# shanice-l/UNOPose

Measured on AMD Instinct MI355X. Metric: (query,ref) pairs/sec forward, higher is better.
Workload: dtype bf16; 1 GPU; UNOPose.forward, batch 32 pairs/GPU, 2048 query pts, 5000->2048 reference pts, 196 coarse pts, 518x518 crops, DINOv2 ViT-B/14 reg4, random-init (trained-like) weights

## Files before the change

### include/unopose_hip.h

```cpp
#ifndef UNOPOSE_HIP_H
#define UNOPOSE_HIP_H

#include <stdint.h>

#ifdef __cplusplus
extern "C" {
#endif

#define UNOPOSE_OK 0
#define UNOPOSE_EINVAL 1
#define UNOPOSE_ELAUNCH 2
#define UNOPOSE_ENOMEM 3

typedef void *unopose_stream_t;

int unopose_abi_version(void);
const char *unopose_last_error(void);


int unopose_furthest_point_sampling(const float *xyz, int B, int N, int M,
                                    int32_t *idx, unopose_stream_t stream);

int unopose_gather_points(const float *points, const int32_t *idx, int B, int C,
                          int N, int M, float *out, unopose_stream_t stream);
// ... 45 lines not shown
int unopose_pe_image_bytes(void);
int unopose_pe_pack_weights(const float *w1, const float *b1, const float *w2, const float *b2,
                            const float *w3, const float *b3, void *image, unopose_stream_t stream);

int unopose_pe_geometry(const float *xyz, int B, int N, float radius, int nsample, float radius2, int nsample2,
                        const int *cand_in, const int *cand_cnt_in, int cand_stride, void *lists, int *counts,
                        float *frames, int *cand_out, void *lists2, int *counts2, float *frames2,
                        unopose_stream_t stream);
int unopose_pe_mlp_max_packed(const float *xyz, int B, int N, float radius, int nsample, const void *image,
                              const void *lists, const int *counts, const float *frames, void *out, int out_ld,
                              int out_split, unopose_stream_t stream);

int unopose_geo_embedding(const float *points, int B, int n, const void *wd_hi,
                          const void *wd_lo, const void *wa_hi, const void *wa_lo,
                          const float *bias_sum, const float *div_term,
                          float sigma_d, float factor_a, int reduce_mean, int split,
                          int out_bf16, int32_t *knn_ws, void *out,
                          unopose_stream_t stream);

int unopose_geo_embedding_table(const float *points, int B, int n, const float *tab_d, int rows_d, const float *tab_a, int rows_a,
                                const float *bias_sum, const float *w_d, const float *div_term, int hinv, int npoint, float sigma_d,
                                float factor_a, int reduce_mean, int out_bf16, int32_t *knn_ws, void *out,
                                unopose_stream_t stream);

int unopose_geo_embedding_train_workgroups(int B, int n);
int unopose_geo_embedding_train_forward(const float *points, int B, int n, const float *tab_d, int rows_d, const float *tab_a, int rows_a,
                                        const float *bias_sum, const float *w_d, const float *div_term, int hinv, float sigma_d, float factor_a,
                                        int reduce_mean, int32_t *knn, float *out, void *amax, unopose_stream_t stream);
int unopose_geo_embedding_train_backward(const float *points, const int32_t *knn, int B, int n, int rows_d, int rows_a, int hinv, float sigma_d,
                                         float factor_a, int reduce_mean, const float *dE, const void *amax, float *ws, float *full_d,
                                         int *past_table, unopose_stream_t stream);

int unopose_pe_group_mlp_max(const float *xyz, int B, int N, float radius, int nsample,
                             const float *w1, const float *b1, const float *w2,
                             const float *b2, const float *w3, const float *b3,
                             int bf16x3, float *out, unopose_stream_t stream);

int unopose_softmax_stats(const float *x, int B, int R, int C, float *stats_ws, unopose_stream_t stream);
int unopose_infonce_grad(const float *x, int B, int R, int C, const float *stats_ws, const long long *label1,
                         const long long *label2, const float *g, float *grad, unopose_stream_t stream);

int unopose_bn_train_chunk(void);
int unopose_bn_relu_train_forward(const float *x, int B, int C, long L, const float *gamma, const float *beta, float eps, float momentum,
                                  float *running_mean, float *running_var, float *workspace, float *mean, float *rstd, float *y,
                                  unopose_stream_t stream);
int unopose_bn_relu_train_backward(const float *x, const float *dy, int B, int C, long L, const float *gamma, const float *beta,
                                   const float *mean, const float *rstd, float *workspace, float *dgamma, float *dbeta, float *dx,
                                   unopose_stream_t stream);

int unopose_bn_relu_maxpool_train_forward(const float *x, int B, int C, int N, int S, const float *gamma, const float *beta, float eps,
                                          float momentum, float *running_mean, float *running_var, float *workspace, float *mean, float *rstd,
                                          float *out, int32_t *idx, unopose_stream_t stream);
int unopose_bn_relu_maxpool_train_backward(const float *x, const float *g, const int32_t *idx, int B, int C, int N, int S, const float *gamma,
                                           const float *beta, const float *mean, const float *rstd, float *workspace, float *dgamma, float *dbeta,
                                           float *dx, unopose_stream_t stream);

int unopose_saliency_train_forward(const float *atten, const float *s1, const float *s2, int B, int n1, int n2, float *m1, float *m2, float *rmax,
                                   float *rsum, float *cmax, float *csum, unopose_stream_t stream);
int unopose_saliency_train_backward(const float *atten, const float *s1, const float *s2, const float *m1, const float *m2, const float *rmax,
                                    const float *rsum, const float *cmax, const float *csum, const float *g1, const float *g2, int B, int n1, int n2,
                                    float *d_atten, float *ds1, float *ds2, unopose_stream_t stream);

int unopose_nearest_partner(const float *a, const float *b, int B, int n, int m, int over_b, float thr, float *dmin, int32_t *arg,
                            uint8_t *any_close, unopose_stream_t stream);

int unopose_conv1x1_train_wgrad_blocks(void);
int unopose_conv1x1_train_forward(const float *x, int B, int cin, long L, const float *w, int cout, float *y, unopose_stream_t stream);
int unopose_conv1x1_train_wgrad(const float *dy, const float *x, int B, int cout, int cin, long L, float *workspace, float *dw,
                                unopose_stream_t stream);

int unopose_linear_wgrad_f32_splits(long rows, int N, int K);
int unopose_linear_wgrad_f32(const float *g, const float *x, long rows, int N, int K, float *workspace, float *dw, unopose_stream_t stream);
int unopose_assign_labels(const float *atten, int B, int R, int C, const float *score1,
                          const float *score2, float *stats_ws, float *w1, float *w2,
                          unopose_stream_t stream);

int unopose_fine_correspondences(const float *atten, int B, int R, int C, const float *score1,
                                 const float *score2, const float *stats_ws, const float *w1,
                                 const float *w2, const float *pts2, float *weight, float *pred,
                                 unopose_stream_t stream);

int unopose_upproj_plan(const long long *choose, int B2, int Np, int H, int W, int side, int tok_offset, int tok_stride,
                        int cap_rows, int *ws, int *row_list, int *cellmap, int *tile_info, unopose_stream_t stream);

int unopose_linear_bf16_ld(const void *A, int lda, const void *W, int ldw, const float *bias, void *C, int ldc, long M, int N, int K,
                           int epilogue, unopose_stream_t stream);

int unopose_linear_add_layernorm_bf16(const void *A, const void *W, const float *bias, const void *resid, const float *ln_w,
                                      const float *ln_b, float eps, void *C, long M, int K, unopose_stream_t stream);

int unopose_linear_bf16_kv_vt(const void *A, const void *W, const float *bias, void *C, void *vt, long M, int N, int K, int tokens, int key_pad,
                              unopose_stream_t stream);

int unopose_linear_bf16_gather(const void *A, long M, int K, const void *W, int N, const float *bias, const int *row_list,
                               const int *tile_info, int max_tiles, void *C, unopose_stream_t stream);

int unopose_bilinear_sample_compact(const void *Cc, const int *cellmap, const long long *choose, int B2, int side, int Np,
                                    int H, int W, void *out, int out_bf16, unopose_stream_t stream);

int unopose_fine_assign(const void *f1, const void *f2, int B, int R, int C, int D, float shift, const float *score1,
                        const float *score2, const float *pts2, float *ws, float *w1, float *w2, float *weight,
                        float *pred, unopose_stream_t stream);

int unopose_min_dist(const float *p, const float *q, int B, int N, int M, const float *R,
                     const float *t, int cand_per_b, float *out, unopose_stream_t stream);

int unopose_coarse_hypotheses(const float *atten, int B, int R, int C, const float *score1,
                              const float *score2, const float *stats_ws, const float *w1,
                              const float *w2, const float *rand, int nprop, const float *pts1,
                              const float *pts2, float *cdf_ws, float *Rout, float *tout,
                              float *dis, unopose_stream_t stream);

int unopose_coarse_scores(const float *pts1, const float *pts2, int B, int n1, int n2,
                          const float *Rall, const float *tall, int nprop, const int64_t *top,
                          int ncand, const float *w1, float *score, unopose_stream_t stream);

int unopose_topk_smallest(const float *x, int B, int n, int k, int64_t *idx, unopose_stream_t stream);
int unopose_coarse_pick(const float *score, const int64_t *top, int B, int ncand, const float *Rall, const float *tall, int nprop,
                        float *R, float *t, float *best_score, unopose_stream_t stream);

int unopose_token_attention(const void *q, int ldq, const void *k, int ldk, const void *vt,
                            const void *qp, int ldqp, const void *E, int B, int n, int m,
                            float scale, void *out, unopose_stream_t stream);
int unopose_token_attention_key_pad(void);

int unopose_token_attention_f32(const float *q, int ldq, const float *k, int ldk, const float *vt,
                                const float *qp, int ldqp, const float *E, int B, int n, int m,
                                float scale, float *out, unopose_stream_t stream);
int unopose_vit_attention_f32(const float *qkv, int B, int T, int H, float *out, unopose_stream_t stream);
int unopose_token_attention_f32_train(const float *q, int ldq, const float *k, int ldk, const float *vt,
                                      const float *qp, int ldqp, const float *E, int B, int n, int m,
                                      float scale, float *out, float *P, unopose_stream_t stream);
int unopose_token_attention_f32_backward(const float *dout, const float *q, int ldq, const float *v, int ldv,
                                         const float *kt, const float *qp, int ldqp, const float *E, const float *P,
                                         int B, int n, int m, float scale, float *dS, float *dq, float *dk, float *dv,
                                         float *dqp, float *dE, unopose_stream_t stream);
int unopose_vit_attention_f32_split(const float *qkv, int B, int T, int H, void *out_split, unopose_stream_t stream);
int unopose_vit_attention_f32_ss(const void *qkv_split, int B, int T, int H, void *out_split, unopose_stream_t stream);

int unopose_vit_attention(const void *qkv, int B, int T, int H, void *out, unopose_stream_t stream);
int unopose_vit_attention_route(int T, int H);

int unopose_add_layernorm(const void *a, int a_bf16, const void *b, int b_bf16, const float *w,
                          const float *bias, long rows, int C, float eps, void *out, int out_bf16,
                          unopose_stream_t stream);

int unopose_add_layernorm_strided(const void *a, int a_bf16, const void *b, int b_bf16, const float *w,
                                  const float *bias, long rows, int C, float eps, void *out, int out_bf16,
                                  long ld_out, unopose_stream_t stream);

int unopose_add_layernorm_train(const void *a, int a_bf16, const void *b, int b_bf16, const float *w,
                                const float *bias, long rows, int C, float eps, float *y, float *s, float *mean,
                                float *rstd, unopose_stream_t stream);
int unopose_add_layernorm_backward_slabs(long rows, int C);
int unopose_add_layernorm_backward(const float *dy, const float *s, const float *mean, const float *rstd,
                                   const float *w, long rows, int C, float *dx, float *dw, float *db,
                                   float *partials, int partial_slabs, unopose_stream_t stream);

int unopose_bilinear_sample(const void *z, int z_bf16, const long long *choose, int B, int side, int Np,
                            int H, int W, float *out, unopose_stream_t stream);

int unopose_bilinear_sample_tokens(const void *z, int z_bf16, const long long *choose, int B, int side, int Np,
                                   int H, int W, int tok_offset, int tok_stride, float *out,
                                   unopose_stream_t stream);

int unopose_scale_residual_layernorm(float *x, const void *y_bf16, const float *gamma, const float *w,
                                     const float *bias, long rows, int C, float eps, void *out_bf16,
                                     unopose_stream_t stream);
int unopose_scale_residual_layernorm_f32(float *x, const float *y, const float *gamma, const float *w, const float *bias, long rows,
                                         int C, float eps, void *out_split, long out_ld_bytes, unopose_stream_t stream);

int unopose_scale_residual(float *x, const void *y_bf16, const float *gamma, long rows, int C,
                           unopose_stream_t stream);

int unopose_linear_attention(const void *x, const float *inv_softplus_scale, const void *kvt,
                             const float *ksum, int B, int N, int focus, int mode, void *out,
                             unopose_stream_t stream);
int unopose_linear_attention_kv_state(const void *ykv, const float *inv_softplus_scale, int B, int J, int rows_per_pair,
                                      int first_row, int focus, void *kvt, float *ksum, unopose_stream_t stream);
int unopose_linear_attention_f32(const float *x, const float *inv_softplus_scale, const float *kvt,
                                 const float *ksum, int B, int N, int focus, int mode, float *out,
                                 unopose_stream_t stream);

int unopose_render_depth(const float *verts, int V, const int *faces, int F, const float *Rt, const float *K4, int P, int H, int W,
                         float *depth, unopose_stream_t stream);

int unopose_render_color(const float *verts, int V, const int *faces, int F, const float *colors, float surf_r, float surf_g, float surf_b,
                         float ambient, const float *Rt, const float *K4, int P, int H, int W, void *keys, float *depth, void *rgb,
                         unopose_stream_t stream);

int unopose_render_shaded(const float *verts, int V, const int *faces, int F, const float *normals, const float *colors, const float *uv,
                          const float *texture, int Ht, int Wt, float surf_r, float surf_g, float surf_b, float ambient, int phong, int ssaa,
                          const float *Rt, const float *K4, int P, int H, int W, void *keys, void *rgb, unopose_stream_t stream);

int unopose_vis_workspace_ints(void);
int unopose_vis_compose(const void *rgbs, const float *depths, int P, int H, int W, const void *photo, int resolve_visib, int *boxes,
                        void *ren_rgb, float *ren_depth, void *vis_rgb, unopose_stream_t stream);
int unopose_vis_depth_diff(const float *ren_depth, const float *depth, int H, int W, float delta, void *workspace, void *image, double *stats,
                           unopose_stream_t stream);

int unopose_patchify_bf16(const float *rgb_a, int na, const float *rgb_b, int nb, int S, int Kp, void *out,
                          unopose_stream_t stream);
int unopose_vit_tokens_layernorm(const void *patch, const float *pos, const float *prefix, int npre, int P, int nimg, int C,
                                 const float *ln_w, const float *ln_b, float eps, float *x, void *n1, float *row_mean, unopose_stream_t stream);
int unopose_patchify_split(const float *rgb_a, int na, const float *rgb_b, int nb, int S, int Kp, void *out, unopose_stream_t stream);
int unopose_vit_tokens_layernorm_f32(const float *patch, const float *pos, const float *prefix, int npre, int P, int nimg, int C,
                                     const float *ln_w, const float *ln_b, float eps, float *x, void *n1_split, unopose_stream_t stream);
int unopose_row_dot(const void *x, int x_bf16, const float *w, float b, long rows, int C, void *out, int out_bf16,
                    unopose_stream_t stream);
int unopose_normalize_rows_bf16(const void *x, int x_bf16, long rows, int C, float temp, void *out, int out_f32,
                                unopose_stream_t stream);
int unopose_gather_rows(const void *feats, int B, int N, int row_bytes, const void *idx, int idx_is_i64, int J, int off,
                        const void *alt, long alt_stride_bytes, int prepend, void *out, unopose_stream_t stream);
int unopose_transpose_pad_bf16(const void *v, long ld, int B, int m, int C, int pad, void *vt, unopose_stream_t stream);
int unopose_transpose_pad_f32(const float *v, long ld, int B, int m, int C, int pad, float *vt, unopose_stream_t stream);

int unopose_cloud_radius(const float *pts, int B, int N, float *radius, unopose_stream_t stream);
int unopose_scale_by_radius(const float *x, int B, int n, const float *radius, float eps, int multiply, float *out, unopose_stream_t stream);
int unopose_overlap_scores(const void *scores, int x_bf16, int B, int n_tot, int n1, int halves, float *out, unopose_stream_t stream);
int unopose_nan_to_num_multi(const void *ptrs_dev, const void *sizes_dev, int n_tensors, long max_size, float nan_value, float posinf_value,
                             float neginf_value, unopose_stream_t stream);
int unopose_copy_rows(const void *src, long src_stride_bytes, void *dst, long dst_stride_bytes, int rows, int row_bytes,
                      unopose_stream_t stream);
int unopose_rigid_rows_bf16(const float *p, int B, int N, const float *t, const float *R, void *out, unopose_stream_t stream);
int unopose_token_sum_bf16(const void *x, int B, int J, int C, float *out, unopose_stream_t stream);
int unopose_pose_score(const float *dis, const float *w, int B, int N, float thr, float *out, unopose_stream_t stream);

int unopose_linear_bf16(const void *A, const void *W, const float *bias, void *C, long M, int N, int K,
                        int epilogue, unopose_stream_t stream);
int unopose_gemm_bf16_tile(void);

int unopose_linear_bf16_residual(const void *A, const void *W, const float *bias, float *xres, void *xb, float *stats, const float *prev,
                                 int prev_nparts, long M, int N, int K, unopose_stream_t stream);
int unopose_linear_bf16_lnfold(const void *A, const void *W, const float *dvec, const float *cvec, const float *stats, int nparts, float eps,
                               void *C, long M, int N, int K, int gelu, unopose_stream_t stream);
int unopose_gemm_fold_stagger(int eighth_ticks_per_ktile);

int unopose_bmm_f32(const float *A, long sab, long sah, long sai, long sak, const float *Bm, long sbb, long sbh, long sbj, long sbk,
                    float *C, int bo, int bi, int n, int m, int K, float alpha, unopose_stream_t stream);

int unopose_split_bf16x2(const float *X, long M, int K, void *Xs, unopose_stream_t stream);
int unopose_linear_f32x3(const void *As, const void *Ws, const float *bias, float *C, void *Cs, long M, int N, int K,
                         int epilogue, unopose_stream_t stream);
int unopose_linear_f32x3_bf16(const void *As, const void *Ws, const float *bias, const void *resid, void *Cb, long M, int N, int K,
                              unopose_stream_t stream);

int unopose_prep_desc_ints(void);
int unopose_prep_crop_resize(const void *img, int H, int W, int C, const int *desc, const int *taps, const void *masks, const float *lut,
                             int D, int S, int bgr, int use_mask, float *out, unopose_stream_t stream);
int unopose_prep_compact_lift(const double *depth, int H, int W, const int *desc, const void *masks, const int *row_base, double fx,
                              double fy, double cx, double cy, int D, int max_h, int *pix, double *cloud, double *row_sums,
                              unopose_stream_t stream);
int unopose_prep_distances(const int *desc, const double *cloud, const double *row_sums, int D, int max_n, double *dist,
                           unopose_stream_t stream);
int unopose_prep_gather(const int *sel, const int *index, const int *pix, const double *cloud, int P, int n, int S, float *pts, void *choose,
                        unopose_stream_t stream);

int unopose_rle_desc_ints(void);
int unopose_rle_stats_ints(void);
int unopose_rle_parse(const void *bytes, const int *lists, const int *desc, int D, int H, int W, int *starts, int *stats,
                      unopose_stream_t stream);
int unopose_rle_fill(const int *desc, const int *starts, const double *depth, int D, int H, int W, void *masks, int *stats,
                     unopose_stream_t stream);
int unopose_rle_column_scan(const void *masks, int D, int H, int W, int *col_count, int *totals, unopose_stream_t stream);
int unopose_rle_compact(const void *masks, const int *col_count, const void *off, int D, int H, int W, int *pos, unopose_stream_t stream);
int unopose_rle_diff(const int *pos, const void *off, int D, int max_n, int H, int W, int *counts, unopose_stream_t stream);
int unopose_window_masks(const void *masks, const int *desc, int K, int max_h, int H, int W, void *packed, int *row_counts,
                         unopose_stream_t stream);

int unopose_vsd_count_ints(void);
int unopose_vsd_counts(const float *test, int n_test, const float *gt, int n_gt, const float *est, int n_est, const int *index,
                       const double *pairs, const double *taus, int T, int P, int H, int W, int *counts, unopose_stream_t stream);
int unopose_pose_errors(const double *pts, int n, const double *syms, int S, const double *est, const double *gt, const double *K, int P,
                        double *mssd, double *mspd, unopose_stream_t stream);

int unopose_adi_tile_points(void);
int unopose_adi_slab_points(void);
int unopose_pose_metrics(const double *pts, int n, const double *syms, int S, const double *est, const double *gt, const double *K, int P,
                         int proj_sym, double *out, unopose_stream_t stream);
int unopose_adi(const double *pts, int n, const double *est, const double *gt, int P, double *workspace, double *adi,
                unopose_stream_t stream);

int unopose_gt_visibility_ints(void);
int unopose_gt_visibility(const float *canvas, int n_canvas, const float *test, int n_test, const int *index, const double *params, int G,
                          int H, int W, int *out, void *mask, void *mask_visib, unopose_stream_t stream);

int unopose_pts_extent_tile_points(void);
int unopose_pts_extent_doubles(void);
int unopose_pts_extent(const double *pts, const long long *offsets, const long long *offsets_dev, int M, int prune, double *kept,
                       long long *kept_count, double *out, unopose_stream_t stream);

int unopose_ref_select_query_tile(void);
int unopose_ref_select_entry_tile(void);
int unopose_ref_select_slab(int Q, int C, int S);
int unopose_ref_select(const double *Rq, const long long *q_scene, const unsigned long long *q_key, int Q, const double *Rc,
                       const long long *c_scene, const unsigned long long *c_key, int C, const double *syms, int S, double trace_min,
                       unsigned long long seed, int cross_scene, int slab, long long *workspace, long long *out, unopose_stream_t stream);

int unopose_adam_table_ints(int what);
int unopose_adam_prepare(const void *grads_dev, const void *chunks_dev, long n_chunks, int n_tensors, double *partials, unopose_stream_t stream);
int unopose_adam_finalise(const double *partials, long n_chunks, int n_tensors, const void *state_dev, const void *finite, double max_norm, double lr,
                          double beta1, double beta2, float *block, unopose_stream_t stream);
int unopose_adam_update(const void *grads_dev, const void *state_dev, const void *chunks_dev, long n_chunks, int n_tensors, const float *block,
                        double beta1, double beta2, double eps, double weight_decay, unopose_stream_t stream);

int unopose_coloraug_ints(int what);
int unopose_coloraug_luma_sum(const void *src, int H, int W, const int *desc, const int *ops, int n_crops, int max_pixels, int pos, void *sums,
                              unopose_stream_t stream);
int unopose_coloraug_step(const void *src, void *dst, int H, int W, const int *desc, const int *ops, const void *grids, const float *noise,
                          const void *sums, int n_crops, int max_pixels, int pos, unopose_stream_t stream);
int unopose_coloraug_blur_lines(const void *src, void *dst, int H, int W, const int *desc, const int *ops, int n_crops, int max_across,
                                int max_line, int pos, int axis, unopose_stream_t stream);

#ifdef __cplusplus
}
#endif
#endif
```

### unopose_amd/_lib.py

```python
import ctypes
import os

import torch

_HERE = os.path.dirname(os.path.abspath(__file__))
SO_PATH = os.environ.get("UNOPOSE_LIB") or os.path.join(_HERE, "libunopose_hip.so")

_lib = None

_P = ctypes.c_void_p
_I = ctypes.c_int
_F = ctypes.c_float
_L = ctypes.c_long
_D = ctypes.c_double

SIGNATURES = {
    "unopose_furthest_point_sampling": [_P, _I, _I, _I, _P, _P],
    "unopose_gather_points": [_P, _P, _I, _I, _I, _I, _P, _P],
    "unopose_gather_points_grad": [_P, _P, _I, _I, _I, _I, _P, _P],
    "unopose_ball_query": [_P, _P, _I, _I, _I, _F, _I, _P, _P],
    "unopose_group_points": [_P, _P, _I, _I, _I, _I, _I, _P, _P],
    "unopose_group_points_grad": [_P, _P, _I, _I, _I, _I, _I, _P, _P],
    "unopose_three_nn": [_P, _P, _I, _I, _I, _P, _P, _P],
    "unopose_three_interpolate": [_P, _P, _P, _I, _I, _I, _I, _P, _P],
    "unopose_three_interpolate_grad": [_P, _P, _P, _I, _I, _I, _I, _P, _P],
    "unopose_lrf_global": [_P, _I, _I, _I, _P, _P],
    "unopose_query_lrf_group": [_P, _I, _I, _F, _I, _P, _P],
    "unopose_lrf_group_idx": [_P, _P, _P, _I, _I, _F, _I, _P, _P],
    "unopose_weighted_procrustes": [_P, _P, _P, _I, _I, _F, _F, _P, _P, _P],
    "unopose_assign_labels": [_P, _I, _I, _I, _P, _P, _P, _P, _P, _P],
    "unopose_linear_bf16_ld": [_P, _I, _P, _I, _P, _P, _I, ctypes.c_long, _I, _I, _I, _P],
    "unopose_scale_residual_layernorm_f32": [_P, _P, _P, _P, _P, ctypes.c_long, _I, _F, _P, _L, _P],
    "unopose_gather_rows": [_P, _I, _I, _I, _P, _I, _I, _I, _P, _L, _I, _P, _P],
    "unopose_softmax_stats": [_P, _I, _I, _I, _P, _P],
    "unopose_infonce_grad": [_P, _I, _I, _I, _P, _P, _P, _P, _P, _P],
    "unopose_fine_correspondences": [_P, _I, _I, _I, _P, _P, _P, _P, _P, _P, _P, _P, _P],
    "unopose_upproj_plan": [_P, _I, _I, _I, _I, _I, _I, _I, _I, _P, _P, _P, _P, _P],
    "unopose_linear_add_layernorm_bf16": [_P, _P, _P, _P, _P, _P, _F, _P, ctypes.c_long, _I, _P],
    "unopose_linear_bf16_kv_vt": [_P, _P, _P, _P, _P, ctypes.c_long, _I, _I, _I, _I, _P],
    "unopose_linear_bf16_gather": [_P, ctypes.c_long, _I, _P, _I, _P, _P, _P, _I, _P, _P],
    "unopose_bilinear_sample_compact": [_P, _P, _P, _I, _I, _I, _I, _I, _P, _I, _P],
    "unopose_fine_assign": [_P, _P, _I, _I, _I, _I, _F, _P, _P, _P, _P, _P, _P, _P, _P, _P],
    "unopose_min_dist": [_P, _P, _I, _I, _I, _P, _P, _I, _P, _P],
    "unopose_coarse_hypotheses": [_P, _I, _I, _I, _P, _P, _P, _P, _P, _P, _I, _P, _P, _P, _P, _P, _P, _P],
    "unopose_coarse_scores": [_P, _P, _I, _I, _I, _P, _P, _I, _P, _I, _P, _P, _P],
    "unopose_topk_smallest": [_P, _I, _I, _I, _P, _P],
    "unopose_coarse_pick": [_P, _P, _I, _I, _P, _P, _I, _P, _P, _P, _P],
    "unopose_token_attention": [_P, _I, _P, _I, _P, _P, _I, _P, _I, _I, _I, _F, _P, _P],
    "unopose_token_attention_key_pad": [],
    "unopose_token_attention_f32": [_P, _I, _P, _I, _P, _P, _I, _P, _I, _I, _I, _F, _P, _P],
    "unopose_token_attention_f32_train": [_P, _I, _P, _I, _P, _P, _I, _P, _I, _I, _I, _F, _P, _P, _P],
    "unopose_token_attention_f32_backward": [_P, _P, _I, _P, _I, _P, _P, _I, _P, _P, _I, _I, _I, _F, _P, _P, _P, _P, _P, _P, _P],
    "unopose_vit_attention_f32": [_P, _I, _I, _I, _P, _P],
    "unopose_vit_attention_f32_split": [_P, _I, _I, _I, _P, _P],
    "unopose_vit_attention_f32_ss": [_P, _I, _I, _I, _P, _P],
    "unopose_bn_train_chunk": [],
    "unopose_bn_relu_train_forward": [_P, _I, _I, ctypes.c_long, _P, _P, _F, _F, _P, _P, _P, _P, _P, _P, _P],
    "unopose_bn_relu_train_backward": [_P, _P, _I, _I, ctypes.c_long, _P, _P, _P, _P, _P, _P, _P, _P, _P],
    "unopose_bn_relu_maxpool_train_forward": [_P, _I, _I, _I, _I, _P, _P, _F, _F, _P, _P, _P, _P, _P, _P, _P, _P],
    "unopose_bn_relu_maxpool_train_backward": [_P, _P, _P, _I, _I, _I, _I, _P, _P, _P, _P, _P, _P, _P, _P, _P],
    "unopose_nearest_partner": [_P, _P, _I, _I, _I, _I, _F, _P, _P, _P, _P],
    "unopose_saliency_train_forward": [_P, _P, _P, _I, _I, _I, _P, _P, _P, _P, _P, _P, _P],
    "unopose_saliency_train_backward": [_P, _P, _P, _P, _P, _P, _P, _P, _P, _P, _P, _I, _I, _I, _P, _P, _P, _P],
    "unopose_conv1x1_train_wgrad_blocks": [],
    "unopose_conv1x1_train_forward": [_P, _I, _I, ctypes.c_long, _P, _I, _P, _P],
    "unopose_conv1x1_train_wgrad": [_P, _P, _I, _I, _I, ctypes.c_long, _P, _P, _P],
    "unopose_linear_wgrad_f32_splits": [ctypes.c_long, _I, _I],
    "unopose_linear_wgrad_f32": [_P, _P, ctypes.c_long, _I, _I, _P, _P, _P],
    "unopose_vit_attention": [_P, _I, _I, _I, _P, _P],
    "unopose_vit_attention_route": [_I, _I],
    "unopose_add_layernorm": [_P, _I, _P, _I, _P, _P, ctypes.c_long, _I, _F, _P, _I, _P],
    "unopose_add_layernorm_strided": [_P, _I, _P, _I, _P, _P, ctypes.c_long, _I, _F, _P, _I, ctypes.c_long, _P],
    "unopose_add_layernorm_train": [_P, _I, _P, _I, _P, _P, _L, _I, _F, _P, _P, _P, _P, _P],
    "unopose_add_layernorm_backward_slabs": [_L, _I],
    "unopose_add_layernorm_backward": [_P, _P, _P, _P, _P, _L, _I, _P, _P, _P, _P, _I, _P],
    "unopose_bilinear_sample": [_P, _I, _P, _I, _I, _I, _I, _I, _P, _P],
    "unopose_bilinear_sample_tokens": [_P, _I, _P, _I, _I, _I, _I, _I, _I, _I, _P, _P],
    "unopose_scale_residual_layernorm": [_P, _P, _P, _P, _P, ctypes.c_long, _I, _F, _P, _P],
    "unopose_scale_residual": [_P, _P, _P, ctypes.c_long, _I, _P],
    "unopose_linear_attention": [_P, _P, _P, _P, _I, _I, _I, _I, _P, _P],
    "unopose_linear_attention_f32": [_P, _P, _P, _P, _I, _I, _I, _I, _P, _P],
    "unopose_linear_attention_kv_state": [_P, _P, _I, _I, _I, _I, _I, _P, _P, _P],
    "unopose_linear_bf16": [_P, _P, _P, _P, ctypes.c_long, _I, _I, _I, _P],
    "unopose_gemm_bf16_tile": [],
    "unopose_gemm_fold_stagger": [_I],
    "unopose_linear_bf16_residual": [_P, _P, _P, _P, _P, _P, _P, _I, ctypes.c_long, _I, _I, _P],
    "unopose_linear_bf16_lnfold": [_P, _P, _P, _P, _P, _I, _F, _P, ctypes.c_long, _I, _I, _I, _P],
    "unopose_patchify_bf16": [_P, _I, _P, _I, _I, _I, _P, _P],
    "unopose_patchify_split": [_P, _I, _P, _I, _I, _I, _P, _P],
    "unopose_vit_tokens_layernorm": [_P, _P, _P, _I, _I, _I, _I, _P, _P, _F, _P, _P, _P, _P],
    "unopose_vit_tokens_layernorm_f32": [_P, _P, _P, _I, _I, _I, _I, _P, _P, _F, _P, _P, _P],
    "unopose_row_dot": [_P, _I, _P, _F, ctypes.c_long, _I, _P, _I, _P],
    "unopose_normalize_rows_bf16": [_P, _I, ctypes.c_long, _I, _F, _P, _I, _P],
    "unopose_transpose_pad_bf16": [_P, ctypes.c_long, _I, _I, _I, _I, _P, _P],
    "unopose_transpose_pad_f32": [_P, _L, _I, _I, _I, _I, _P, _P],
    "unopose_cloud_radius": [_P, _I, _I, _P, _P],
    "unopose_scale_by_radius": [_P, _I, _I, _P, _F, _I, _P, _P],
    "unopose_overlap_scores": [_P, _I, _I, _I, _I, _I, _P, _P],
    "unopose_copy_rows": [_P, _L, _P, _L, _I, _I, _P],
    "unopose_nan_to_num_multi": [_P, _P, _I, _L, _F, _F, _F, _P],
    "unopose_rigid_rows_bf16": [_P, _I, _I, _P, _P, _P, _P],
    "unopose_token_sum_bf16": [_P, _I, _I, _I, _P, _P],
    "unopose_pose_score": [_P, _P, _I, _I, _F, _P, _P],
    "unopose_render_depth": [_P, _I, _P, _I, _P, _P, _I, _I, _I, _P, _P],
    "unopose_render_color": [_P, _I, _P, _I, _P, _F, _F, _F, _F, _P, _P, _I, _I, _I, _P, _P, _P, _P],
    "unopose_render_shaded": [_P, _I, _P, _I, _P, _P, _P, _P, _I, _I, _F, _F, _F, _F, _I, _I, _P, _P, _I, _I, _I, _P, _P, _P],
    "unopose_vis_workspace_ints": [],
    "unopose_vis_compose": [_P, _P, _I, _I, _I, _P, _I, _P, _P, _P, _P, _P],
    "unopose_vis_depth_diff": [_P, _P, _I, _I, _F, _P, _P, _P, _P],
    "unopose_bmm_f32": [_P, ctypes.c_long, ctypes.c_long, ctypes.c_long, ctypes.c_long, _P, ctypes.c_long, ctypes.c_long, ctypes.c_long, ctypes.c_long, _P, _I, _I, _I, _I, _I, _F, _P],
    "unopose_split_bf16x2": [_P, ctypes.c_long, _I, _P, _P],
    "unopose_linear_f32x3": [_P, _P, _P, _P, _P, ctypes.c_long, _I, _I, _I, _P],
    "unopose_pe_image_bytes": [],
    "unopose_pe_pack_weights": [_P, _P, _P, _P, _P, _P, _P, _P],
    "unopose_pe_geometry": [_P, _I, _I, _F, _I, _F, _I, _P, _P, _I, _P, _P, _P, _P, _P, _P, _P, _P],
    "unopose_pe_mlp_max_packed": [_P, _I, _I, _F, _I, _P, _P, _P, _P, _P, _I, _I, _P],
    "unopose_linear_f32x3_bf16": [_P, _P, _P, _P, _P, ctypes.c_long, _I, _I, _P],
    "unopose_pe_group_mlp_max": [_P, _I, _I, _F, _I, _P, _P, _P, _P, _P, _P, _I, _P, _P],
    "unopose_geo_embedding": [_P, _I, _I, _P, _P, _P, _P, _P, _P, _F, _F, _I, _I, _I, _P, _P, _P],
    "unopose_geo_embedding_train_workgroups": [_I, _I],
    "unopose_geo_embedding_train_forward": [_P, _I, _I, _P, _I, _P, _I, _P, _P, _P, _I, _F, _F, _I, _P, _P, _P, _P],
    "unopose_geo_embedding_train_backward": [_P, _P, _I, _I, _I, _I, _I, _F, _F, _I, _P, _P, _P, _P, _P, _P],
    "unopose_geo_embedding_table": [_P, _I, _I, _P, _I, _P, _I, _P, _P, _P, _I, _I, _F, _F, _I, _I, _P, _P, _P],
    "unopose_prep_desc_ints": [],
    "unopose_prep_crop_resize": [_P, _I, _I, _I, _P, _P, _P, _P, _I, _I, _I, _I, _P, _P],
    "unopose_prep_compact_lift": [_P, _I, _I, _P, _P, _P, _D, _D, _D, _D, _I, _I, _P, _P, _P, _P],
    "unopose_prep_distances": [_P, _P, _P, _I, _I, _P, _P],
    "unopose_prep_gather": [_P, _P, _P, _P, _I, _I, _I, _P, _P, _P],
    "unopose_rle_desc_ints": [],
    "unopose_rle_stats_ints": [],
    "unopose_rle_parse": [_P, _P, _P, _I, _I, _I, _P, _P, _P],
    "unopose_rle_fill": [_P, _P, _P, _I, _I, _I, _P, _P, _P],
    "unopose_rle_column_scan": [_P, _I, _I, _I, _P, _P, _P],
    "unopose_rle_compact": [_P, _P, _P, _I, _I, _I, _P, _P],
    "unopose_rle_diff": [_P, _P, _I, _I, _I, _I, _P, _P],
    "unopose_window_masks": [_P, _P, _I, _I, _I, _I, _P, _P, _P],
    "unopose_vsd_count_ints": [],
    "unopose_vsd_counts": [_P, _I, _P, _I, _P, _I, _P, _P, _P, _I, _I, _I, _I, _P, _P],
    "unopose_pose_errors": [_P, _I, _P, _I, _P, _P, _P, _I, _P, _P, _P],
    "unopose_adi_tile_points": [],
    "unopose_adi_slab_points": [],
    "unopose_pose_metrics": [_P, _I, _P, _I, _P, _P, _P, _I, _I, _P, _P],
    "unopose_adi": [_P, _I, _P, _P, _I, _P, _P, _P],
    "unopose_gt_visibility_ints": [],
    "unopose_gt_visibility": [_P, _I, _P, _I, _P, _P, _I, _I, _I, _P, _P, _P, _P],
    "unopose_pts_extent_tile_points": [],
    "unopose_pts_extent_doubles": [],
    "unopose_pts_extent": [_P, _P, _P, _I, _I, _P, _P, _P, _P],
    "unopose_ref_select_query_tile": [],
    "unopose_ref_select_entry_tile": [],
    "unopose_ref_select_slab": [_I, _I, _I],
    "unopose_ref_select": [_P, _P, _P, _I, _P, _P, _P, _I, _P, _I, _D, ctypes.c_ulonglong, _I, _I, _P, _P, _P],
    "unopose_adam_table_ints": [_I],
    "unopose_adam_prepare": [_P, _P, _L, _I, _P, _P],
    "unopose_adam_finalise": [_P, _L, _I, _P, _P, _D, _D, _D, _D, _P, _P],
    "unopose_adam_update": [_P, _P, _P, _L, _I, _P, _D, _D, _D, _D, _P],
    "unopose_coloraug_ints": [_I],
    "unopose_coloraug_luma_sum": [_P, _I, _I, _P, _P, _I, _I, _I, _P, _P],
    "unopose_coloraug_step": [_P, _P, _I, _I, _P, _P, _P, _P, _P, _I, _I, _I, _P],
    "unopose_coloraug_blur_lines": [_P, _P, _I, _I, _P, _P, _I, _I, _I, _I, _I, _P],
}


def lib():
    global _lib
    if _lib is None:
        if not os.path.exists(SO_PATH):
            raise RuntimeError(
                f"{SO_PATH} is missing: the HIP extension has not been built "
                "(run `python -m unopose_amd.build`). There is no CPU fallback."
# ... 68 lines not shown
```

### unopose_amd/csrc/fused.hip

```cpp
#include <algorithm>

#include "common.h"

namespace unopose {

template <bool IN_BF16>
__device__ __forceinline__ float fu_load(const void *p, size_t i) {
  return IN_BF16 ? bf2f(reinterpret_cast<const u16 *>(p)[i]) : reinterpret_cast<const float *>(p)[i];
}

template <bool A_BF16, bool B_BF16, bool HAS_B, bool OUT_BF16>
__global__ __launch_bounds__(256) void add_layernorm_kernel(const void *__restrict__ a, const void *__restrict__ b,
                                                            const float *__restrict__ w,
                                                            const float *__restrict__ bias, long rows, int C,
                                                            float eps, void *__restrict__ out, long ldo) {
  const long r = (long)blockIdx.x * 4 + (threadIdx.x >> 6);
  if (r >= rows) return;
  const int lane = threadIdx.x & 63;
  float v[16];
  float s = 0.f;
#pragma unroll
  for (int i = 0; i < 16; ++i) {
    const int c = i * 64 + lane;
    float x = 0.f;
    if (c < C) {
      x = fu_load<A_BF16>(a, (size_t)r * C + c);
      if (HAS_B) x += fu_load<B_BF16>(b, (size_t)r * C + c);
    }
    v[i] = x;
    s += x;
  }
  const float mean = wave_sum_f32(s) / (float)C;
  float q = 0.f;
#pragma unroll
  for (int i = 0; i < 16; ++i) {
    const int c = i * 64 + lane;
    const float d = c < C ? v[i] - mean : 0.f;
    q += d * d;
  }
  const float rstd = rsqrtf(wave_sum_f32(q) / (float)C + eps);
#pragma unroll
  for (int i = 0; i < 16; ++i) {
    const int c = i * 64 + lane;
    if (c < C) {
      const float y = (v[i] - mean) * rstd * w[c] + bias[c];
      if (OUT_BF16)
        reinterpret_cast<u16 *>(out)[(size_t)r * ldo + c] = f2bf(y);
      else
        reinterpret_cast<float *>(out)[(size_t)r * ldo + c] = y;
    }
  }
}

template <bool BF>
__device__ __forceinline__ float4 fu_load4(const void *p, size_t i) {
  if (BF) {
    const uint2 r = *reinterpret_cast<const uint2 *>(reinterpret_cast<const u16 *>(p) + i);
    return make_float4(bf2f((u16)(r.x & 0xFFFF)), bf2f((u16)(r.x >> 16)), bf2f((u16)(r.y & 0xFFFF)), bf2f((u16)(r.y >> 16)));
  }
  return *reinterpret_cast<const float4 *>(reinterpret_cast<const float *>(p) + i);
}
template <bool A_BF16, bool B_BF16, bool HAS_B, bool OUT_BF16>
__global__ __launch_bounds__(256) void add_layernorm_vec4_kernel(const void *__restrict__ a, const void *__restrict__ b,
                                                                 const float *__restrict__ w, const float *__restrict__ bias, long rows,
                                                                 int C, float eps, void *__restrict__ out, long ldo) {
  const long r = (long)blockIdx.x * 4 + (threadIdx.x >> 6);
  if (r >= rows) return;
  const int lane = threadIdx.x & 63;
  float4 v[4];
  float s = 0.f;
#pragma unroll
  for (int i = 0; i < 4; ++i) {
    const int c = (i * 64 + lane) * 4;
    float4 x = make_float4(0.f, 0.f, 0.f, 0.f);
    if (c < C) {
      x = fu_load4<A_BF16>(a, (size_t)r * C + c);
      if (HAS_B) {
        const float4 y = fu_load4<B_BF16>(b, (size_t)r * C + c);
        x.x += y.x;
        x.y += y.y;
        x.z += y.z;
        x.w += y.w;
      }
    }
    v[i] = x;
    s += (x.x + x.y) + (x.z + x.w);
  }
  const float mean = wave_sum_f32(s) / (float)C;
  float q = 0.f;
#pragma unroll
  for (int i = 0; i < 4; ++i) {
    if ((i * 64 + lane) * 4 < C) {
      const float d0 = v[i].x - mean, d1 = v[i].y - mean, d2 = v[i].z - mean, d3 = v[i].w - mean;
      q += (d0 * d0 + d1 * d1) + (d2 * d2 + d3 * d3);
    }
  }
  const float rstd = rsqrtf(wave_sum_f32(q) / (float)C + eps);
#pragma unroll
  for (int i = 0; i < 4; ++i) {
    const int c = (i * 64 + lane) * 4;
    if (c < C) {
      const float4 wv = *reinterpret_cast<const float4 *>(w + c), bv = *reinterpret_cast<const float4 *>(bias + c);
      const float y0 = (v[i].x - mean) * rstd * wv.x + bv.x, y1 = (v[i].y - mean) * rstd * wv.y + bv.y;
      const float y2 = (v[i].z - mean) * rstd * wv.z + bv.z, y3 = (v[i].w - mean) * rstd * wv.w + bv.w;
      if (OUT_BF16) {
        uint2 o;
        o.x = (uint32_t)f2bf(y0) | ((uint32_t)f2bf(y1) << 16);
        o.y = (uint32_t)f2bf(y2) | ((uint32_t)f2bf(y3) << 16);
        *reinterpret_cast<uint2 *>(reinterpret_cast<u16 *>(out) + (size_t)r * ldo + c) = o;
      } else {
        *reinterpret_cast<float4 *>(reinterpret_cast<float *>(out) + (size_t)r * ldo + c) = make_float4(y0, y1, y2, y3);
      }
    }
  }
}

__global__ __launch_bounds__(256) void scale_residual_layernorm_kernel(float *__restrict__ x, const u16 *__restrict__ y,
                                                                       const float *__restrict__ gamma,
                                                                       const float *__restrict__ w,
                                                                       const float *__restrict__ bias, long rows,
                                                                       int C, float eps, u16 *__restrict__ out) {
  const long r = (long)blockIdx.x * 4 + (threadIdx.x >> 6);
  if (r >= rows) return;
  const int lane = threadIdx.x & 63;
  float v[16];
  float s = 0.f;
#pragma unroll
  for (int i = 0; i < 4; ++i) {
    const int c = (i * 64 + lane) * 4;
    float4 xv = make_float4(0.f, 0.f, 0.f, 0.f);
    if (c < C) {
      xv = *reinterpret_cast<const float4 *>(x + (size_t)r * C + c);
      const uint2 yv = *reinterpret_cast<const uint2 *>(y + (size_t)r * C + c);
      const float4 g = *reinterpret_cast<const float4 *>(gamma + c);
      xv.x += g.x * bf2f((u16)(yv.x & 0xFFFF));
      xv.y += g.y * bf2f((u16)(yv.x >> 16));
      xv.z += g.z * bf2f((u16)(yv.y & 0xFFFF));
      xv.w += g.w * bf2f((u16)(yv.y >> 16));
      *reinterpret_cast<float4 *>(x + (size_t)r * C + c) = xv;
    }
    v[i * 4 + 0] = xv.x; v[i * 4 + 1] = xv.y; v[i * 4 + 2] = xv.z; v[i * 4 + 3] = xv.w;
    s += (xv.x + xv.y) + (xv.z + xv.w);
  }
  const float mean = wave_sum_f32(s) / (float)C;
  float q = 0.f;
#pragma unroll
  for (int i = 0; i < 4; ++i) {
    const int c = (i * 64 + lane) * 4;
    if (c < C) {
#pragma unroll
      for (int e = 0; e < 4; ++e) {
        const float d = v[i * 4 + e] - mean;
        q += d * d;
      }
    }
  }
  const float rstd = rsqrtf(wave_sum_f32(q) / (float)C + eps);
#pragma unroll
  for (int i = 0; i < 4; ++i) {
    const int c = (i * 64 + lane) * 4;
    if (c < C) {
      const float4 wv = *reinterpret_cast<const float4 *>(w + c), bv = *reinterpret_cast<const float4 *>(bias + c);
      uint2 o;
      o.x = (uint32_t)f2bf((v[i * 4 + 0] - mean) * rstd * wv.x + bv.x) |
            ((uint32_t)f2bf((v[i * 4 + 1] - mean) * rstd * wv.y + bv.y) << 16);
      o.y = (uint32_t)f2bf((v[i * 4 + 2] - mean) * rstd * wv.z + bv.z) |
            ((uint32_t)f2bf((v[i * 4 + 3] - mean) * rstd * wv.w + bv.w) << 16);
      *reinterpret_cast<uint2 *>(out + (size_t)r * C + c) = o;
    }
  }
}

__global__ __launch_bounds__(256) void scale_residual_layernorm_f32_kernel(float *__restrict__ x, const float *__restrict__ y,
                                                                           const float *__restrict__ gamma, const float *__restrict__ w,
                                                                           const float *__restrict__ bias, long rows, int C, float eps,
                                                                           char *__restrict__ out, long out_ld) {
  const long r = (long)blockIdx.x * 4 + (threadIdx.x >> 6);
  if (r >= rows) return;
  const int lane = threadIdx.x & 63;
  float v[16];
  float s = 0.f;
#pragma unroll
  for (int i = 0; i < 4; ++i) {
    const int c = (i * 64 + lane) * 4;
    float4 xv = make_float4(0.f, 0.f, 0.f, 0.f);
    if (c < C) {
      xv = *reinterpret_cast<const float4 *>(x + (size_t)r * C + c);
      if (y) {
        const float4 yv = *reinterpret_cast<const float4 *>(y + (size_t)r * C + c);
        const float4 g = *reinterpret_cast<const float4 *>(gamma + c);
        xv.x += g.x * yv.x; xv.y += g.y * yv.y; xv.z += g.z * yv.z; xv.w += g.w * yv.w;
        *reinterpret_cast<float4 *>(x + (size_t)r * C + c) = xv;
      }
    }
    v[i * 4 + 0] = xv.x; v[i * 4 + 1] = xv.y; v[i * 4 + 2] = xv.z; v[i * 4 + 3] = xv.w;
    s += (xv.x + xv.y) + (xv.z + xv.w);
  }
// ... 54 lines not shown
  const int b = blockIdx.y, lane = threadIdx.x & 63;
  const int p = blockIdx.x * 4 + (threadIdx.x >> 6);
  if (p >= Np) return;
  const long long pix = choose[(size_t)b * Np + p];
  const int hw = 4 * side;
  const BilinearTap tp = bilinear_tap(pix, H, W, hw);
  const int y0 = tp.y0, x0 = tp.x0, y1 = tp.y1, x1 = tp.x1;
  const float ly = tp.ly, lx = tp.lx;
  auto at = [&](int Y, int X) -> size_t {
    return ((((size_t)b * tok_stride + tok_off + (size_t)(Y >> 2) * side + (X >> 2))) * 16 + (Y & 3) * 4 + (X & 3)) * 256;
  };
  const size_t o00 = at(y0, x0), o01 = at(y0, x1), o10 = at(y1, x0), o11 = at(y1, x1);
  float v[4][4];
  const size_t offs[4] = {o00, o01, o10, o11};
#pragma unroll
  for (int k = 0; k < 4; ++k) {
    if (IN_BF16) {
      const uint2 r = *reinterpret_cast<const uint2 *>(reinterpret_cast<const u16 *>(z) + offs[k] + lane * 4);
      v[k][0] = bf2f((u16)(r.x & 0xFFFF)); v[k][1] = bf2f((u16)(r.x >> 16));
      v[k][2] = bf2f((u16)(r.y & 0xFFFF)); v[k][3] = bf2f((u16)(r.y >> 16));
    } else {
      const float4 r = *reinterpret_cast<const float4 *>(reinterpret_cast<const float *>(z) + offs[k] + lane * 4);
      v[k][0] = r.x; v[k][1] = r.y; v[k][2] = r.z; v[k][3] = r.w;
    }
  }
  float4 res;
  float *rp = &res.x;
#pragma unroll
  for (int c = 0; c < 4; ++c) {
    const float top = (1.f - lx) * v[0][c] + lx * v[1][c];
    const float bot = (1.f - lx) * v[2][c] + lx * v[3][c];
    rp[c] = (1.f - ly) * top + ly * bot;
  }
  *reinterpret_cast<float4 *>(out + ((size_t)b * Np + p) * 256 + lane * 4) = res;
}

}

using namespace unopose;

extern "C" {

int unopose_add_layernorm(const void *a, int a_bf16, const void *b, int b_bf16, const float *w, const float *bias,
                          long rows, int C, float eps, void *out, int out_bf16, unopose_stream_t stream) {
  return unopose_add_layernorm_strided(a, a_bf16, b, b_bf16, w, bias, rows, C, eps, out, out_bf16, C, stream);
}

int unopose_add_layernorm_strided(const void *a, int a_bf16, const void *b, int b_bf16, const float *w,
                                  const float *bias, long rows, int C, float eps, void *out, int out_bf16, long ld_out,
                                  unopose_stream_t stream) {
  UNOPOSE_REQUIRE(a && w && bias && out, "add_layernorm: null pointer");
  UNOPOSE_REQUIRE(rows >= 0 && C >= 1 && C <= 1024 && ld_out >= C, "add_layernorm: C=%d unsupported (<= 1024, ld_out >= C)", C);
  if (rows == 0) return UNOPOSE_OK;
  dim3 grid((unsigned)((rows + 3) / 4));
  hipStream_t s = (hipStream_t)stream;
  const bool vec4 = C % 4 == 0 && ld_out % 4 == 0;
#define UNOPOSE_LN(AB, BB, HB, OB)                                                                                               \
  do {                                                                                                                           \
    if (vec4)                                                                                                                    \
      hipLaunchKernelGGL((add_layernorm_vec4_kernel<AB, BB, HB, OB>), grid, dim3(256), 0, s, a, b, w, bias, rows, C, eps, out, ld_out); \
    else                                                                                                                         \
      hipLaunchKernelGGL((add_layernorm_kernel<AB, BB, HB, OB>), grid, dim3(256), 0, s, a, b, w, bias, rows, C, eps, out, ld_out);      \
  } while (0)
  const int key = (a_bf16 ? 8 : 0) | (b ? (b_bf16 ? 4 : 0) | 2 : 0) | (out_bf16 ? 1 : 0);
  switch (key) {
    case 0: UNOPOSE_LN(false, false, false, false); break;
    case 1: UNOPOSE_LN(false, false, false, true); break;
    case 2: UNOPOSE_LN(false, false, true, false); break;
    case 3: UNOPOSE_LN(false, false, true, true); break;
    case 6: UNOPOSE_LN(false, true, true, false); break;
    case 7: UNOPOSE_LN(false, true, true, true); break;
    case 8: UNOPOSE_LN(true, false, false, false); break;
    case 9: UNOPOSE_LN(true, false, false, true); break;
    case 10: UNOPOSE_LN(true, false, true, false); break;
    case 11: UNOPOSE_LN(true, false, true, true); break;
    case 14: UNOPOSE_LN(true, true, true, false); break;
    case 15: UNOPOSE_LN(true, true, true, true); break;
    default: UNOPOSE_REQUIRE(false, "add_layernorm: bad dtype combination");
  }
#undef UNOPOSE_LN
  return check_launch("add_layernorm");
}

int unopose_bilinear_sample(const void *z, int z_bf16, const long long *choose, int B, int side, int Np, int H, int W,
                            float *out, unopose_stream_t stream) {
  return unopose_bilinear_sample_tokens(z, z_bf16, choose, B, side, Np, H, W, 0, side * side, out, stream);
}

int unopose_bilinear_sample_tokens(const void *z, int z_bf16, const long long *choose, int B, int side, int Np, int H,
                                   int W, int tok_offset, int tok_stride, float *out, unopose_stream_t stream) {
  UNOPOSE_REQUIRE(z && choose && out, "bilinear_sample: null pointer");
  UNOPOSE_REQUIRE(B >= 0 && side >= 1 && Np >= 0 && H >= 1 && W >= 1 && B <= 65535 && tok_offset >= 0 &&
                      tok_stride >= tok_offset + side * side,
                  "bilinear_sample: bad sizes");
  if (B == 0 || Np == 0) return UNOPOSE_OK;
  dim3 grid(cdiv(Np, 4), B);
  if (z_bf16)
    hipLaunchKernelGGL(bilinear_sample_kernel<true>, grid, dim3(256), 0, (hipStream_t)stream, z, choose, side, Np, H, W,
                       tok_offset, tok_stride, out);
  else
    hipLaunchKernelGGL(bilinear_sample_kernel<false>, grid, dim3(256), 0, (hipStream_t)stream, z, choose, side, Np, H,
                       W, tok_offset, tok_stride, out);
  return check_launch("bilinear_sample");
}

int unopose_scale_residual_layernorm(float *x, const void *y_bf16, const float *gamma, const float *w, const float *bias,
                                     long rows, int C, float eps, void *out_bf16, unopose_stream_t stream) {
  UNOPOSE_REQUIRE(x && y_bf16 && gamma && w && bias && out_bf16, "scale_residual_layernorm: null pointer");
  UNOPOSE_REQUIRE(rows >= 0 && C >= 4 && C % 4 == 0 && C <= 1024, "scale_residual_layernorm: C must be a multiple of 4, <= 1024");
  if (rows == 0) return UNOPOSE_OK;
  hipLaunchKernelGGL(scale_residual_layernorm_kernel, dim3((unsigned)((rows + 3) / 4)), dim3(256), 0,
                     (hipStream_t)stream, x, (const u16 *)y_bf16, gamma, w, bias, rows, C, eps, (u16 *)out_bf16);
  return check_launch("scale_residual_layernorm");
}

int unopose_scale_residual_layernorm_f32(float *x, const float *y, const float *gamma, const float *w, const float *bias, long rows, int C, float eps,
                                         void *out_split, long out_ld_bytes, unopose_stream_t stream) {
  UNOPOSE_REQUIRE(x && (y || out_split) && (!y || gamma) && (!out_split || (w && bias)), "scale_residual_layernorm_f32: null pointer");
  UNOPOSE_REQUIRE(rows >= 0 && C >= 32 && C % 32 == 0 && C <= 1024, "scale_residual_layernorm_f32: C must be a multiple of 32, <= 1024");
  UNOPOSE_REQUIRE(out_ld_bytes == 0 || (out_ld_bytes >= (long)C * 4 && out_ld_bytes % 128 == 0), "scale_residual_layernorm_f32: output rows must be >= 4 C bytes apart, whole 128-byte lines (got %ld)", out_ld_bytes);
  if (rows == 0) return UNOPOSE_OK;
  hipLaunchKernelGGL(scale_residual_layernorm_f32_kernel, dim3((unsigned)((rows + 3) / 4)), dim3(256), 0, (hipStream_t)stream, x, y, gamma, w,
                     bias, rows, C, eps, (char *)out_split, out_ld_bytes ? out_ld_bytes : (long)C * 4);
  return check_launch("scale_residual_layernorm_f32");
}

int unopose_scale_residual(float *x, const void *y_bf16, const float *gamma, long rows, int C,
                           unopose_stream_t stream) {
  UNOPOSE_REQUIRE(x && y_bf16 && gamma, "scale_residual: null pointer");
  UNOPOSE_REQUIRE(rows >= 0 && C >= 4 && C % 4 == 0, "scale_residual: C must be a multiple of 4");
  if (rows == 0) return UNOPOSE_OK;
  const long n4 = rows * C / 4;
  const unsigned blocks = (unsigned)std::min<long>((n4 + 255) / 256, 4096);
  hipLaunchKernelGGL(scale_residual_kernel, dim3(blocks), dim3(256), 0, (hipStream_t)stream, x, (const u16 *)y_bf16,
                     gamma, n4, C);
  return check_launch("scale_residual");
}

}
```

### unopose_amd/csrc/gemm.hip

```cpp
#include <mutex>

#include "gemm_kernel.h"

using namespace unopose;

static inline int use_nt_store(long M, int N) { return (size_t)M * N * 2 > (32u << 20) ? 1 : 0; }

namespace unopose {
int gemm_small_tiles_limit() {
  return gemm_cu_count() * 5 / 8;
}
}
static int small_tiles_limit() { return unopose::gemm_small_tiles_limit(); }

namespace unopose {
int *gemm_sched_slot(hipStream_t stream) {
  hipStreamCaptureStatus cap = hipStreamCaptureStatusNone;
  if (hipStreamIsCapturing(stream, &cap) != hipSuccess || cap != hipStreamCaptureStatusNone) return nullptr;
  static std::mutex mu;
  static int *ring[64] = {nullptr};
  static unsigned next_slot[64] = {0};
  int dev = 0;
  if (hipGetDevice(&dev) != hipSuccess || dev < 0 || dev >= 64) return nullptr;
  std::lock_guard<std::mutex> lock(mu);
// ... 30 lines not shown
}

extern "C" {

int unopose_gemm_bf16_tile(void) { return GEMM_BM; }

int unopose_linear_bf16(const void *A, const void *W, const float *bias, void *C, long M, int N, int K, int epilogue,
                        unopose_stream_t stream) {
  UNOPOSE_REQUIRE(A && W && bias && C, "linear_bf16: null pointer");
  UNOPOSE_REQUIRE(M >= 1 && M < (1L << 31) && N >= GEMM_BN && N % GEMM_BN == 0 && K >= GEMM_BK && K % GEMM_BK == 0,
                  "linear_bf16: needs N %% 256 == 0 and K %% 64 == 0 (got M=%ld N=%d K=%d)", M, N, K);
  UNOPOSE_REQUIRE((size_t)M * K * 2 < (1UL << 32) && (size_t)N * K * 2 < (1UL << 32) && (size_t)M * N * 2 < (1UL << 32), "linear_bf16: operand larger than 4 GiB");
  UNOPOSE_REQUIRE(epilogue >= 0 && epilogue <= 2, "linear_bf16: epilogue must be 0 (bias), 1 (bias + GELU) or 2 (bias + ReLU)");
  return linear_bf16_dispatch(A, K, W, K, bias, C, N, M, N, K, epilogue, (hipStream_t)stream, "linear_bf16");
}

int unopose_linear_bf16_ld(const void *A, int lda, const void *W, int ldw, const float *bias, void *C, int ldc, long M, int N, int K,
                           int epilogue, unopose_stream_t stream) {
  UNOPOSE_REQUIRE(A && W && bias && C, "linear_bf16_ld: null pointer");
  UNOPOSE_REQUIRE(M >= 1 && M < (1L << 31) && N >= GEMM_BN && N % GEMM_BN == 0 && K >= GEMM_BK && K % GEMM_BK == 0,
                  "linear_bf16_ld: needs N %% 256 == 0 and K %% 64 == 0 (got M=%ld N=%d K=%d)", M, N, K);
  UNOPOSE_REQUIRE(lda >= K && ldw >= K && ldc >= N && lda % 8 == 0 && ldw % 8 == 0 && ldc % 8 == 0,
                  "linear_bf16_ld: row strides must cover the rows and be multiples of 8 elements (lda=%d ldw=%d ldc=%d)", lda, ldw, ldc);
  UNOPOSE_REQUIRE((size_t)M * lda * 2 < (1UL << 32) && (size_t)N * ldw * 2 < (1UL << 32) && (size_t)M * ldc * 2 < (1UL << 32), "linear_bf16_ld: operand larger than 4 GiB");
  UNOPOSE_REQUIRE(epilogue >= 0 && epilogue <= 2, "linear_bf16_ld: epilogue must be 0 (bias), 1 (bias + GELU) or 2 (bias + ReLU)");
  return linear_bf16_dispatch(A, lda, W, ldw, bias, C, ldc, M, N, K, epilogue, (hipStream_t)stream, "linear_bf16_ld");
}

int unopose_linear_add_layernorm_bf16(const void *A, const void *W, const float *bias, const void *resid, const float *ln_w,
                                      const float *ln_b, float eps, void *C, long M, int K, unopose_stream_t stream) {
  UNOPOSE_REQUIRE(A && W && bias && resid && ln_w && ln_b && C, "linear_add_layernorm_bf16: null pointer");
  UNOPOSE_REQUIRE(M >= 1 && M < (1L << 31) && K >= GEMM_BK && K % GEMM_BK == 0, "linear_add_layernorm_bf16: needs K %% 64 == 0 (got M=%ld K=%d)", M, K);
  UNOPOSE_REQUIRE((size_t)M * K * 2 < (1UL << 32), "linear_add_layernorm_bf16: operand larger than 4 GiB");
  const int tiles = cdiv(M, GEMM_BM);
  if (tiles < small_tiles_limit()) return gemm_small_linear_ln(A, W, bias, resid, ln_w, ln_b, eps, C, M, K, (hipStream_t)stream);
  const int n_cu = gemm_cu_count();
  const int grid = tiles >= n_cu ? n_cu : ((tiles + 7) & ~7);
  hipLaunchKernelGGL((gemm256_kernel<3, false>), dim3(grid), dim3(512), 0, (hipStream_t)stream, (const u16 *)A, (const u16 *)W, bias,
                     (u16 *)C, (int)M, GEMM_BN, K, 1, tiles, use_nt_store(M, GEMM_BN), (const int *)nullptr, (const int *)nullptr,
                     (const u16 *)resid, ln_w, ln_b, eps);
  return check_launch("linear_add_layernorm_bf16");
}

int unopose_linear_bf16_kv_vt(const void *A, const void *W, const float *bias, void *C, void *vt, long M, int N, int K, int tokens, int key_pad,
                               unopose_stream_t stream) {
  UNOPOSE_REQUIRE(A && W && bias && C && vt, "linear_bf16_kv_vt: null pointer");
  UNOPOSE_REQUIRE(M >= 1 && M < (1L << 31) && N >= 256 && N % 128 == 0 && K >= GEMM_BK && K % GEMM_BK == 0,
                  "linear_bf16_kv_vt: needs N %% 128 == 0 (>= 256) and K %% 64 == 0 (got M=%ld N=%d K=%d)", M, N, K);
  UNOPOSE_REQUIRE(tokens >= 1 && key_pad >= tokens && M % tokens == 0 && key_pad - tokens <= 64, "linear_bf16_kv_vt: M must be whole clouds of `tokens` rows, key_pad in [tokens, tokens + 64] (got %ld, %d, %d)", M, tokens, key_pad);
  UNOPOSE_REQUIRE((size_t)M * K * 2 < (1UL << 32) && (size_t)N * K * 2 < (1UL << 32) && (size_t)M * N * 2 < (1UL << 32), "linear_bf16_kv_vt: operand larger than 4 GiB");
  return gemm_small_linear_vt(A, W, bias, C, vt, M, N, K, tokens, key_pad, (hipStream_t)stream);
}

int unopose_linear_bf16_gather(const void *A, long M, int K, const void *W, int N, const float *bias, const int *row_list,
                               const int *tile_info, int max_tiles, void *C, unopose_stream_t stream) {
  UNOPOSE_REQUIRE(A && W && bias && C && row_list && tile_info, "linear_bf16_gather: null pointer");
  UNOPOSE_REQUIRE(M >= 1 && M < (1L << 31) && N >= GEMM_BN && N % GEMM_BN == 0 && N / GEMM_BN <= 64 && K >= GEMM_BK && K % GEMM_BK == 0,
                  "linear_bf16_gather: needs N %% 256 == 0 and K %% 64 == 0 (got M=%ld N=%d K=%d)", M, N, K);
  UNOPOSE_REQUIRE((size_t)M * K * 2 < (1UL << 32) && (size_t)N * K * 2 < (1UL << 32), "linear_bf16_gather: operand larger than 4 GiB");
  UNOPOSE_REQUIRE(max_tiles >= 0, "linear_bf16_gather: bad tile capacity");
  if (max_tiles == 0) return UNOPOSE_OK;
  const int n_cu = gemm_cu_count();
  const int grid = max_tiles >= n_cu ? n_cu : ((max_tiles + 7) & ~7);
  hipLaunchKernelGGL((gemm256_kernel<0, true>), dim3(grid), dim3(512), 0, (hipStream_t)stream, (const u16 *)A, (const u16 *)W, bias,
                     (u16 *)C, (int)M, N, K, 1, 0, 0, row_list, tile_info);
  return check_launch("linear_bf16_gather");
}

static int fold_launch_shape(long M, int N, int *grid, int *tiles, int *tiles_n) {
  *tiles_n = N / GEMM_BN;
  *tiles = cdiv(M, GEMM_BM) * *tiles_n;
  const int n_cu = gemm_cu_count();
  *grid = *tiles >= n_cu ? n_cu : ((*tiles + 7) & ~7);
  return use_nt_store(M, N);
}

static int g_fold_stagger = 8 * 105;
int unopose_gemm_fold_stagger(int eighth_ticks_per_ktile) {
  const int was = g_fold_stagger;
  if (eighth_ticks_per_ktile >= 0) g_fold_stagger = eighth_ticks_per_ktile;
  return was;
}

int unopose_linear_bf16_residual(const void *A, const void *W, const float *bias, float *xres, void *xb, float *stats, const float *prev,
                                 int prev_nparts, long M, int N, int K, unopose_stream_t stream) {
  UNOPOSE_REQUIRE(A && W && bias && xres && xb && stats, "linear_bf16_residual: null pointer");
  UNOPOSE_REQUIRE(prev != stats && (prev_nparts == 0 || (prev && prev_nparts * GEMM_BN == N && prev_nparts <= GEMM_LNF_MAXPARTS)),
                  "linear_bf16_residual: prev must be another buffer with 0 or N / 256 <= %d partials per row (got prev_nparts=%d N=%d)",
                  GEMM_LNF_MAXPARTS, prev_nparts, N);
  UNOPOSE_REQUIRE(M >= 1 && M < (1L << 31) && N >= GEMM_BN && N % GEMM_BN == 0 && K >= GEMM_BK && K % GEMM_BK == 0,
                  "linear_bf16_residual: needs N %% 256 == 0 and K %% 64 == 0 (got M=%ld N=%d K=%d)", M, N, K);
  UNOPOSE_REQUIRE((size_t)M * K * 2 < (1UL << 32) && (size_t)N * K * 2 < (1UL << 32) && (size_t)M * N * 4 < (1UL << 31), "linear_bf16_residual: operand too large for 32-bit buffer offsets");
  int grid, tiles, tiles_n;
  const int nt = fold_launch_shape(M, N, &grid, &tiles, &tiles_n);
  hipStream_t s = (hipStream_t)stream;
  int *const sched = tiles > grid ? gemm_sched_slot(s) : nullptr;
  hipLaunchKernelGGL((gemm256_kernel<5>), dim3(grid), dim3(512), 0, s, (const u16 *)A, (const u16 *)W, bias, (u16 *)xb, (int)M, N, K, tiles_n, tiles, nt,
                     (const int *)nullptr, (const int *)nullptr, (const u16 *)nullptr, (const float *)nullptr, (const float *)nullptr, 0.f, 0, 0, 0, sched,
                     (void *)xres, (const float *)nullptr, (float2 *)stats, prev_nparts, tiles > grid ? g_fold_stagger * (K / GEMM_BK) / 8 : 0, prev);
  return check_launch("linear_bf16_residual");
}

int unopose_linear_bf16_lnfold(const void *A, const void *W, const float *dvec, const float *cvec, const float *stats, int nparts, float eps, void *C,
                               long M, int N, int K, int gelu, unopose_stream_t stream) {
  UNOPOSE_REQUIRE(A && W && dvec && cvec && stats && C, "linear_bf16_lnfold: null pointer");
  UNOPOSE_REQUIRE(M >= 1 && M < (1L << 31) && N >= GEMM_BN && N % GEMM_BN == 0 && K >= GEMM_BK && K % GEMM_BK == 0,
                  "linear_bf16_lnfold: needs N %% 256 == 0 and K %% 64 == 0 (got M=%ld N=%d K=%d)", M, N, K);
  UNOPOSE_REQUIRE(nparts >= 1 && nparts <= GEMM_LNF_MAXPARTS && nparts * GEMM_BN == K, "linear_bf16_lnfold: needs nparts = K / 256 <= %d (got nparts=%d K=%d)", GEMM_LNF_MAXPARTS, nparts, K);
  UNOPOSE_REQUIRE((size_t)M * K * 2 < (1UL << 32) && (size_t)N * K * 2 < (1UL << 32) && (size_t)M * N * 2 < (1UL << 32), "linear_bf16_lnfold: operand larger than 4 GiB");
  int grid, tiles, tiles_n;
  const int nt = fold_launch_shape(M, N, &grid, &tiles, &tiles_n);
  hipStream_t s = (hipStream_t)stream;
  int *const sched = tiles > grid ? gemm_sched_slot(s) : nullptr;
#define UNOPOSE_LNF_LAUNCH(E)                                                                                                                      \
  hipLaunchKernelGGL((gemm256_kernel<E>), dim3(grid), dim3(512), 0, s, (const u16 *)A, (const u16 *)W, dvec, (u16 *)C, (int)M, N, K, tiles_n, tiles, nt, \
                     (const int *)nullptr, (const int *)nullptr, (const u16 *)nullptr, (const float *)nullptr, (const float *)nullptr, eps, 0, 0, 0, sched, \
                     (void *)nullptr, cvec, (float2 *)stats, nparts)
  if (gelu)
    UNOPOSE_LNF_LAUNCH(7);
  else
    UNOPOSE_LNF_LAUNCH(6);
#undef UNOPOSE_LNF_LAUNCH
  return check_launch("linear_bf16_lnfold");
}

}
```

### unopose_amd/csrc/gemm_kernel.h

```cpp
#pragma once
#include "gemm_common.h"

namespace unopose {

constexpr int GEMM_XPOL = 2;
#define GEMM_BK 64
constexpr int GEMM_ROTX = 5, GEMM_ROTS = 3;

#define GEMM_WAIT_VM(n) asm volatile("s_waitcnt vmcnt(" #n ")" ::: "memory")
#define GEMM_WAIT_VM_(n) GEMM_WAIT_VM(n)

#define GEMM_LDS_BIAS (2 * GEMM_BUFBYTES)
#define GEMM_LDS_MBOX (GEMM_LDS_BIAS + 2048)
#define GEMM_LDS_LNW (GEMM_LDS_MBOX + 16)
#define GEMM_LDS_LNB (GEMM_LDS_LNW + 1024)
#define GEMM_LDS_LNPART (GEMM_LDS_LNB + 1024)
#define GEMM_LDS_STATS GEMM_LDS_LNPART
#define GEMM_LNF_MAXPARTS 4
#define GEMM_LDS_SHIFT (GEMM_LDS_LNPART + 8192)

struct AccTile {
  static constexpr int RB = 16;
  static constexpr int NRB = 128 / RB;
  static constexpr int NP = 64 / RB;
  static constexpr int NCG = 16 / NP;
  static constexpr int NKS = 8 / NP;
  typedef f32x4 frag;
  static __device__ __forceinline__ int row(int lane) { return lane & (RB - 1); }
  static __device__ __forceinline__ int part(int lane) { return (lane / RB) & (NP - 1); }
  static __device__ __forceinline__ int col0(int cg, int pt) { return cg * (4 * NP) + 4 * pt; }
  static __device__ __forceinline__ f32x4 get(const frag (&acc)[NCG][NRB], int rb, int cg) { return acc[cg][rb]; }
  static __device__ __forceinline__ void set(frag (&acc)[NCG][NRB], int rb, int cg, f32x4 v) { acc[cg][rb] = v; }
  static __device__ __forceinline__ uint32_t frag_off(int ks, int lane) {
    const int r = row(lane), c = NP * ks + part(lane);
    return (uint32_t)((r >> 3) * 1024 + (r & 7) * 128 + ((c ^ ((r >> 1) & 7)) << 4));
  }
  static __device__ __forceinline__ frag mfma(bf16x8 w, bf16x8 a, frag c) { return __builtin_amdgcn_mfma_f32_16x16x32_bf16(w, a, c, 0, 0, 0); }
};

template <int EPI, bool GATHER = false, bool F32 = false>
__global__ __launch_bounds__(512, 1) __attribute__((amdgpu_num_vgpr(127))) void gemm256_kernel(const void *__restrict__ Av, const void *__restrict__ Wv,
                                                           const float *__restrict__ bias, void *__restrict__ Cv, int M,
                                                           int N, int K, int tiles_n, int tiles_arg, int nt_store,
                                                           const int *__restrict__ row_list = nullptr,
                                                           const int *__restrict__ tile_info = nullptr,
                                                           const u16 *__restrict__ resid = nullptr, const float *__restrict__ ln_w = nullptr,
                                                           const float *__restrict__ ln_b = nullptr, float ln_eps = 0.f, int lda = 0,
                                                           int ldw = 0, int ldc = 0, int *__restrict__ sched = nullptr,
                                                           void *__restrict__ C2v = nullptr, const float *__restrict__ aux_vec = nullptr,
                                                           float2 *__restrict__ stats = nullptr, int nparts = 0, int stagger = 0,
                                                           const float *__restrict__ fold_prev = nullptr) {
  static_assert(!(F32 && (EPI == 3 || GATHER)), "the fp32-class form has no LayerNorm epilogue / gathered rows");
  static_assert(!((F32 || GATHER) && EPI >= 5), "the residual / LayerNorm-fold epilogues belong to the dense bf16 form");
  constexpr bool LNF = EPI == 6 || EPI == 7;
  static_assert(F32 || EPI != 4, "EPI 4 (bf16 + residual out of fp32-class operands) is an F32 epilogue");
  constexpr int ESZ = F32 ? 4 : 2;
  constexpr int KT = F32 ? 32 : 64;
  using T = AccTile;
  using frag = T::frag;
  const char *A = reinterpret_cast<const char *>(Av), *W = reinterpret_cast<const char *>(Wv);
  const int LDA = lda ? lda : K, LDW = ldw ? ldw : K, LDC = ldc ? ldc : N;
  const int tiles = GATHER ? __builtin_amdgcn_readfirstlane(tile_info[0]) : tiles_arg;
  __shared__ __attribute__((aligned(1024))) char smem[GEMM_LDS_BIAS + 2048 + 16 + (EPI == 3 ? 2048 + 8192 : EPI == 5 ? 2048 + 8192 + 4096 : LNF ? 2048 + 2 * 8192 : 0)];
  float *const lnw_lds = reinterpret_cast<float *>(smem + GEMM_LDS_LNW), *const lnb_lds = reinterpret_cast<float *>(smem + GEMM_LDS_LNB);
  float2 *const ln_part = reinterpret_cast<float2 *>(smem + GEMM_LDS_LNPART);
  if (EPI == 3 && threadIdx.x < GEMM_BN) {
    lnw_lds[threadIdx.x] = ln_w[threadIdx.x];
    lnb_lds[threadIdx.x] = ln_b[threadIdx.x];
  }
  const int tid = threadIdx.x, lane = tid & 63, wave = __builtin_amdgcn_readfirstlane(tid >> 6);
  const int wm = wave >> 2, wn = wave & 3;
  const int lane_ = lane;
  const int xcd = blockIdx.x & 7, slot = blockIdx.x >> 3, nslots = gridDim.x >> 3;
  const int tiles_m = tiles / tiles_n, per_group = GEMM_GM * tiles_n;
  int cw = (size_t)N * K * ESZ > (size_t)(4u << 20) ? (2400 * 1024) / (GEMM_BN * K * ESZ) : 0;
  if (cw < 3) cw = 0;
  const bool colwalk = cw > 0 && !GATHER && tiles_n > cw && ((tiles_m & 7) == 0 || tiles_m >= 512);
  const int rq = tiles_m >> 3, rr = tiles_m & 7;
  const int rows_x = rq + (xcd < rr ? 1 : 0), row_base = xcd < rr ? xcd * (rq + 1) : rr * (rq + 1) + (xcd - rr) * rq;
  const int cq = tiles >> 3, cr = tiles & 7;
  const int chunk_base = xcd < cr ? xcd * (cq + 1) : cr * (cq + 1) + (xcd - cr) * cq;
  const int chunk_len = colwalk ? rows_x * tiles_n : cq + (xcd < cr ? 1 : 0);
  const __amdgpu_buffer_rsrc_t a_rs = __builtin_amdgcn_make_buffer_rsrc((void *)A, 0, (int)((size_t)M * LDA * ESZ), 0x00020000);
  const __amdgpu_buffer_rsrc_t w_rs = __builtin_amdgcn_make_buffer_rsrc((void *)W, 0, (int)((size_t)N * LDW * ESZ), 0x00020000);
  const __amdgpu_buffer_rsrc_t c_rs = __builtin_amdgcn_make_buffer_rsrc(Cv, 0, GATHER ? 0x7fffffff : (int)((size_t)M * LDC * 2), 0x00020000);
  const __amdgpu_buffer_rsrc_t b_rs = __builtin_amdgcn_make_buffer_rsrc((void *)bias, 0, N * 4, 0x00020000);
  const int nk = K / KT;

  uint32_t fr_off[T::NKS];
#pragma unroll
  for (int ks = 0; ks < T::NKS; ++ks) fr_off[ks] = T::frag_off(ks, lane);
  constexpr int ABH = 64 / T::RB, BBH = 32 / T::RB, BLKB = T::RB * GEMM_ROWB;
  const uint32_t a_base = (uint32_t)(wm * 16384);
  const uint32_t w_base = (uint32_t)(GEMM_OPBYTES + wn * 8192);
  const uint32_t a_dst = (uint32_t)((wave >> 2) * 16384 + (wave & 3) * 2048);
  const uint32_t w_dst = (uint32_t)(GEMM_OPBYTES + (wave >> 1) * 8192 + (wave & 1) * 2048);

  struct TileP {
    int m0, n0, rot;
    uint32_t a_off[4], w_off[2];
  };
  auto tile_params = [&](int ti, int step, TileP &p) {
    const int t = chunk_base + ti;
    int tn, tm;
    if (GATHER) {
      tm = t;
      tn = 0;
      const int ng = N / GEMM_BN;
      for (int g = 1; g < ng; ++g) tn += t >= tile_info[1 + g] ? 1 : 0;
      tn = __builtin_amdgcn_readfirstlane(tn);
    } else if (colwalk) {
      const int per_block = rows_x * cw;
      const int cb = ti / per_block, v = ti - cb * per_block;
      const int cwb = min(cw, tiles_n - cb * cw);
      const int g = v / (GEMM_GM * cwb), w = v - g * GEMM_GM * cwb;
      const int gm = min(GEMM_GM, rows_x - g * GEMM_GM);
      const int tl = w / gm;
      tn = cb * cw + tl;
      tm = row_base + g * GEMM_GM + (w - tl * gm);
    } else {
      const int mg = t / per_group, rr = t - mg * per_group;
      const int gm = min(GEMM_GM, tiles_m - mg * GEMM_GM);
      tn = rr / gm;
      tm = mg * GEMM_GM + (rr - tn * gm);
    }
    p.m0 = __builtin_amdgcn_readfirstlane(tm * GEMM_BM);
    p.n0 = __builtin_amdgcn_readfirstlane(tn * GEMM_BN);
#pragma unroll
    for (int j = 0; j < 4; ++j) {
      const int row = (wave >> 2) * 128 + (j >> 1) * 64 + (wave & 3) * 16 + (j & 1) * 8 + (lane >> 3);
      const int c = (lane & 7) ^ ((row >> 1) & 7);
      int arow = p.m0 + row;
      if (GATHER) arow = max(row_list[p.m0 + row], 0);
      p.a_off[j] = (uint32_t)((size_t)arow * LDA * ESZ + c * 16);
    }
#pragma unroll
    for (int i = 0; i < 2; ++i) {
      const int row = (wave >> 1) * 64 + (wave & 1) * 16 + i * 8 + (lane >> 3);
      const int c = (lane & 7) ^ ((row >> 1) & 7);
      p.w_off[i] = (uint32_t)((size_t)(p.n0 + row) * LDW * ESZ + c * 16);
    }
    const int skew = ((tm & 3) + tn) % GEMM_SKEW;
    p.rot = __builtin_amdgcn_readfirstlane((xcd * GEMM_ROTX + step * GEMM_ROTS + skew) % nk);
  };
  const uint32_t lds0 = (uint32_t)(uintptr_t)(__attribute__((address_space(3))) char *)smem;
// ... 232 lines not shown
        for (int cg = 0; cg < T::NCG; ++cg) {
          const int nl = T::col0(cg, pt);
          const f32x4 bv = *reinterpret_cast<const f32x4 *>(bias_lds + wn * 64 + nl);
          const uint2 r = *reinterpret_cast<const uint2 *>(rp + nl);
          f32x4 v = T::get(acc, rb, cg);
          v[0] = v[0] + bv[0] + __uint_as_float(r.x << 16);
          v[1] = v[1] + bv[1] + __uint_as_float(r.x & 0xffff0000u);
          v[2] = v[2] + bv[2] + __uint_as_float(r.y << 16);
          v[3] = v[3] + bv[3] + __uint_as_float(r.y & 0xffff0000u);
          T::set(acc, rb, cg, v);
          a1 += (v[0] + v[1]) + (v[2] + v[3]);
          a2 += (v[0] * v[0] + v[1] * v[1]) + (v[2] * v[2] + v[3] * v[3]);
        }
#pragma unroll
        for (int d = T::RB; d < 64; d <<= 1) {
          a1 += __shfl_xor(a1, d);
          a2 += __shfl_xor(a2, d);
        }
        if (pt == 0) ln_part[(wm * 128 + rb * T::RB + row) * 4 + wn] = make_float2(a1, a2);
      }
      __syncthreads();
#pragma unroll
      for (int rb = 0; rb < T::NRB; ++rb) {
        const float2 *pp = ln_part + (wm * 128 + rb * T::RB + row) * 4;
        const float t1 = (pp[0].x + pp[1].x) + (pp[2].x + pp[3].x), t2 = (pp[0].y + pp[1].y) + (pp[2].y + pp[3].y);
        const float mean = t1 * (1.f / GEMM_BN);
        const float rstd = rsqrtf(fmaxf(t2 * (1.f / GEMM_BN) - mean * mean, 0.f) + ln_eps);
#pragma unroll
        for (int cg = 0; cg < T::NCG; ++cg) {
          const int nl = wn * 64 + T::col0(cg, pt);
          const f32x4 gw = *reinterpret_cast<const f32x4 *>(lnw_lds + nl), gb = *reinterpret_cast<const f32x4 *>(lnb_lds + nl);
          f32x4 v = T::get(acc, rb, cg);
#pragma unroll
          for (int e = 0; e < 4; ++e) v[e] = (v[e] - mean) * rstd * gw[e] + gb[e];
          T::set(acc, rb, cg, v);
        }
      }
    }
    if constexpr (LNF) {
      int lane = lane_;
      asm volatile("" : "+v"(lane));
      const int row = T::row(lane), pt = T::part(lane);
      const float *c_lds = reinterpret_cast<const float *>(smem + GEMM_LDS_LNW + bsel * 1024);
      const float inv_k = 1.f / (float)K;
      float rs[T::NRB], nm[T::NRB];
#pragma unroll
      for (int rb = 0; rb < T::NRB; ++rb) {
        const float2 *sp = reinterpret_cast<const float2 *>(smem + GEMM_LDS_STATS + bsel * 8192) + (wm * 128 + rb * T::RB + row) * nparts;
        float t1 = 0.f, t2 = 0.f;
#pragma unroll
        for (int i = 0; i < GEMM_LNF_MAXPARTS; ++i)
          if (i < nparts) {
            const float2 q = sp[i];
            t1 += q.x;
            t2 += q.y;
          }
        const float mean = t1 * inv_k;
        rs[rb] = rsqrtf(fmaxf(t2 * inv_k - mean * mean, 0.f) + ln_eps);
        nm[rb] = -mean * rs[rb];
      }
#pragma unroll
      for (int cg = 0; cg < T::NCG; ++cg) {
        const int nl = wn * 64 + T::col0(cg, pt);
        const f32x4 cv = *reinterpret_cast<const f32x4 *>(c_lds + nl), dv = *reinterpret_cast<const f32x4 *>(bias_lds + nl);
#pragma unroll
        for (int rb = 0; rb < T::NRB; ++rb) {
          f32x4 v = T::get(acc, rb, cg);
#pragma unroll
          for (int e = 0; e < 4; ++e) v[e] = fmaf(rs[rb], v[e], fmaf(nm[rb], cv[e], dv[e]));
          T::set(acc, rb, cg, v);
        }
      }
    }
    if constexpr (EPI == 5) {
      int lane = lane_;
      asm volatile("" : "+v"(lane));
      const int arow = T::row(lane), pt = T::part(lane);
      char *cw = smem + par + (wave < 4 ? 8192 + (wave & 1) * 4096 + (wave >> 1) * 16384 : GEMM_OPBYTES + 4096 + (wave - 4) * 8192);
      const __amdgpu_buffer_rsrc_t x_rs = __builtin_amdgcn_make_buffer_rsrc(C2v, 0, (int)((size_t)M * N * 4), 0x00020000);
      const int r4 = lane >> 4, q = lane & 15;
      const uint32_t x_v0 = (uint32_t)((((size_t)m0 + wm * 128 + r4) * N + n0 + wn * 64 + q * 4) * 4);
      const uint32_t c_v0 = (uint32_t)((((size_t)m0 + wm * 128 + r4) * LDC + n0 + wn * 64 + q * 4) * 2);
      const uint32_t x_rowb = (uint32_t)(N * 4), c_rowb = (uint32_t)(LDC * 2);
      const int rows_p = tiles_m * GEMM_BM;
      float sv[2] = {0.f, 0.f};
      if (fold_prev != nullptr) {
        float pv[2][GEMM_LNF_MAXPARTS + 1];
#pragma unroll
        for (int j = 0; j < 2; ++j) {
          const size_t m = (size_t)m0 + wm * 128 + j * 64 + lane, sh_at = (size_t)rows_p * 2 * nparts + m;
#pragma unroll
          for (int i = 0; i < GEMM_LNF_MAXPARTS; ++i) pv[j][i] = fold_prev[i < nparts ? m * 2 * nparts + 2 * i : sh_at];
          pv[j][GEMM_LNF_MAXPARTS] = fold_prev[sh_at];
        }
#pragma unroll
        for (int j = 0; j < 2; ++j) {
          float t = 0.f;
#pragma unroll
          for (int i = 0; i < GEMM_LNF_MAXPARTS; ++i) t += i < nparts ? pv[j][i] : 0.f;
          sv[j] = m0 + wm * 128 + j * 64 + lane < M ? pv[j][GEMM_LNF_MAXPARTS] + t * (1.f / (float)N) : 0.f;
        }
      }
      constexpr int PF = 3;
      f32x4 rv[PF][4];
      auto load_round = [&](int r, f32x4(&dst)[4]) {
#pragma unroll
        for (int it = 0; it < 4; ++it) {
          dst[it] = __builtin_bit_cast(f32x4, __builtin_amdgcn_raw_buffer_load_b128(x_rs, x_v0 + (uint32_t)(r * 16 + it * 4) * x_rowb, 0, GEMM_XPOL));
        }
      };
#pragma unroll
      for (int r = 0; r < PF; ++r) load_round(r, rv[r]);
      float *const sh_lds = reinterpret_cast<float *>(smem + GEMM_LDS_SHIFT + wave * 512);
#pragma unroll
      for (int r = 0; r < 8; ++r) {
        static_assert(T::RB == 16, "a staging round of the residual epilogue is one row block");
#pragma unroll
        for (int cg = 0; cg < T::NCG; ++cg) {
          const int s16 = (T::col0(cg, pt) >> 2) ^ arow;
          *reinterpret_cast<f32x4 *>(cw + arow * 256 + s16 * 16) = T::get(acc, r, cg);
        }
        if (r == 0) {
#pragma unroll
          for (int j = 0; j < 2; ++j) {
            sh_lds[j * 64 + lane] = sv[j];
            if (wn == 0) reinterpret_cast<float *>(stats)[(size_t)rows_p * 2 * tiles_n + m0 + wm * 128 + j * 64 + lane] = sv[j];
          }
        }
        __builtin_amdgcn_fence(__ATOMIC_RELEASE, "wavefront");
        __builtin_amdgcn_wave_barrier();
        __builtin_amdgcn_fence(__ATOMIC_ACQUIRE, "wavefront");
#pragma unroll
        for (int it = 0; it < 4; ++it) {
          const int row = it * 4 + r4;
          const f32x4 a = *reinterpret_cast<const f32x4 *>(cw + row * 256 + ((q ^ row) << 4));
          const f32x4 o = rv[r % PF][it];
          f32x4 v;
#pragma unroll
          for (int e = 0; e < 4; ++e) v[e] = a[e] + o[e];
          __builtin_amdgcn_raw_buffer_store_b128(__builtin_bit_cast(u32x4, v), x_rs, x_v0 + (uint32_t)(r * 16 + it * 4) * x_rowb, 0, GEMM_XPOL);
          const float s = sh_lds[row + r * 16];
#pragma unroll
          for (int e = 0; e < 4; ++e) v[e] = v[e] - s;
          typedef unsigned int u32x2 __attribute__((ext_vector_type(2)));
          const u32x2 pk = {cvt_pk_bf16_f32(v[0], v[1]), cvt_pk_bf16_f32(v[2], v[3])};
          if (nt_store)
            __builtin_amdgcn_raw_buffer_store_b64(pk, c_rs, c_v0 + (uint32_t)(r * 16 + it * 4) * c_rowb, 0, 2);
          else
            __builtin_amdgcn_raw_buffer_store_b64(pk, c_rs, c_v0 + (uint32_t)(r * 16 + it * 4) * c_rowb, 0, 0);
          float a1 = (v[0] + v[1]) + (v[2] + v[3]), a2 = (v[0] * v[0] + v[1] * v[1]) + (v[2] * v[2] + v[3] * v[3]);
          a1 += dpp_f32<0x111, 0xF>(a1, 0.f);
          a2 += dpp_f32<0x111, 0xF>(a2, 0.f);
          a1 += dpp_f32<0x112, 0xF>(a1, 0.f);
          a2 += dpp_f32<0x112, 0xF>(a2, 0.f);
          a1 += dpp_f32<0x114, 0xF>(a1, 0.f);
          a2 += dpp_f32<0x114, 0xF>(a2, 0.f);
          a1 += dpp_f32<0x118, 0xF>(a1, 0.f);
          a2 += dpp_f32<0x118, 0xF>(a2, 0.f);
          if (q == 15) ln_part[(wm * 128 + r * 16 + row) * 4 + wn] = make_float2(a1, a2);
        }
        __builtin_amdgcn_fence(__ATOMIC_RELEASE, "wavefront");
        __builtin_amdgcn_wave_barrier();
        __builtin_amdgcn_fence(__ATOMIC_ACQUIRE, "wavefront");
        if (r + PF < 8) load_round(r + PF, rv[r % PF]);
      }
      asm volatile("s_waitcnt lgkmcnt(0)" ::: "memory");
      __builtin_amdgcn_s_barrier();
// ... 214 lines not shown
```

### unopose_amd/csrc/upproj.hip

```cpp
#include <algorithm>

#include "common.h"

namespace unopose {

__global__ __launch_bounds__(256) void upproj_clear_kernel(int *__restrict__ flags, long nflags, int *__restrict__ row_list, long nrows) {
  const long n = nflags + nrows, step = (long)gridDim.x * 256;
  for (long i = (long)blockIdx.x * 256 + threadIdx.x; i < n; i += step) {
    if (i < nflags) flags[i] = 0;
    else row_list[i - nflags] = -1;
  }
}

__global__ __launch_bounds__(256) void upproj_mark_kernel(const long long *__restrict__ choose, int Np, int H, int W, int side,
                                                          int *__restrict__ flags) {
  const int b = blockIdx.y, p = blockIdx.x * 256 + threadIdx.x;
  if (p >= Np) return;
  const int hw = 4 * side;
  const BilinearTap t = bilinear_tap(choose[(size_t)b * Np + p], H, W, hw);
  int *f = flags + (size_t)b * hw * hw;
  f[t.y0 * hw + t.x0] = 1;
  f[t.y0 * hw + t.x1] = 1;
  f[t.y1 * hw + t.x0] = 1;
  f[t.y1 * hw + t.x1] = 1;
}

__device__ __forceinline__ int up_cell(int t, int s, int side) {
  const int ty = t / side, tx = t - ty * side;
  return (4 * ty + (s >> 2)) * (4 * side) + 4 * tx + (s & 3);
}

__global__ __launch_bounds__(256) void upproj_count_kernel(const int *__restrict__ flags, int side, int B2, int *__restrict__ counts) {
  __shared__ int cnt[16];
  const int b = blockIdx.x, hw = 4 * side;
  if (threadIdx.x < 16) cnt[threadIdx.x] = 0;
  __syncthreads();
  const int *f = flags + (size_t)b * hw * hw;
  int local[16];
#pragma unroll
  for (int s = 0; s < 16; ++s) local[s] = 0;
  for (int t = threadIdx.x; t < side * side; t += 256) {
#pragma unroll
    for (int s = 0; s < 16; ++s) local[s] += f[up_cell(t, s, side)];
  }
#pragma unroll
  for (int s = 0; s < 16; ++s) {
    const int v = (int)wave_sum_f32((float)local[s]);
    if ((threadIdx.x & 63) == 0) atomicAdd(&cnt[s], v);
  }
  __syncthreads();
  if (threadIdx.x < 16) counts[threadIdx.x * B2 + b] = cnt[threadIdx.x];
}

__global__ __launch_bounds__(64) void upproj_offsets_kernel(const int *__restrict__ counts, int B2, int *__restrict__ offsets,
                                                            int *__restrict__ tile_info) {
  __shared__ int total[16], start[17];
  const int s = threadIdx.x;
  if (s < 16) {
    int t = 0;
    for (int b = 0; b < B2; ++b) t += counts[s * B2 + b];
    total[s] = t;
  }
  __syncthreads();
  if (s == 0) {
    int run = 0;
    for (int g = 0; g < 16; ++g) {
      start[g] = run;
      run += (total[g] + 255) & ~255;
    }
    start[16] = run;
    tile_info[0] = run >> 8;
    for (int g = 0; g <= 16; ++g) tile_info[1 + g] = start[g] >> 8;
  }
  __syncthreads();
  if (s < 16) {
    int run = start[s];
    for (int b = 0; b < B2; ++b) {
      offsets[s * B2 + b] = run;
      run += counts[s * B2 + b];
    }
  }
}

__global__ __launch_bounds__(512) void upproj_fill_kernel(const int *__restrict__ flags, const int *__restrict__ offsets, int side, int B2, int tok_offset,
                                                          int tok_stride, int *__restrict__ row_list, int *__restrict__ cellmap) {
  const int b = blockIdx.x, lane = threadIdx.x & 63, wave = threadIdx.x >> 6, hw = 4 * side;
  const int *f = flags + (size_t)b * hw * hw;
  int *cm = cellmap + (size_t)b * hw * hw;
  for (int s = wave * 2; s < wave * 2 + 2; ++s) {
    int base = offsets[s * B2 + b];
    for (int t0 = 0; t0 < side * side; t0 += 64) {
      const int t = t0 + lane;
      const int cell = t < side * side ? up_cell(t, s, side) : 0;
      const bool on = t < side * side && f[cell] != 0;
      const unsigned long long m = __ballot(on);
      if (on) {
        const int r = base + __popcll(m & ((1ull << lane) - 1ull));
        row_list[r] = b * tok_stride + tok_offset + t;
        cm[cell] = r;
      }
      base += __popcll(m);
    }
  }
}

template <bool OUT_BF16>
__global__ __launch_bounds__(256) void bilinear_sample_compact_kernel(const u16 *__restrict__ Cc, const int *__restrict__ cellmap,
                                                                      const long long *__restrict__ choose, int side, int Np, int H,
                                                                      int W, void *__restrict__ outv) {
  const int b = blockIdx.y, lane = threadIdx.x & 63;
  const int p = blockIdx.x * 4 + (threadIdx.x >> 6);
  if (p >= Np) return;
  const int hw = 4 * side;
  const BilinearTap tp = bilinear_tap(choose[(size_t)b * Np + p], H, W, hw);
  const int *cm = cellmap + (size_t)b * hw * hw;
  const int rows[4] = {cm[tp.y0 * hw + tp.x0], cm[tp.y0 * hw + tp.x1], cm[tp.y1 * hw + tp.x0], cm[tp.y1 * hw + tp.x1]};
  float v[4][4];
#pragma unroll
  for (int k = 0; k < 4; ++k) {
    const uint2 r = *reinterpret_cast<const uint2 *>(Cc + (size_t)rows[k] * 256 + lane * 4);
    v[k][0] = bf2f((u16)(r.x & 0xFFFF));
    v[k][1] = bf2f((u16)(r.x >> 16));
    v[k][2] = bf2f((u16)(r.y & 0xFFFF));
    v[k][3] = bf2f((u16)(r.y >> 16));
  }
  const float ly = tp.ly, lx = tp.lx;
  float4 res;
  float *rp = &res.x;
#pragma unroll
  for (int c = 0; c < 4; ++c) {
    const float top = (1.f - lx) * v[0][c] + lx * v[1][c];
    const float bot = (1.f - lx) * v[2][c] + lx * v[3][c];
    rp[c] = (1.f - ly) * top + ly * bot;
  }
  if (OUT_BF16)
    *reinterpret_cast<uint2 *>(reinterpret_cast<u16 *>(outv) + ((size_t)b * Np + p) * 256 + lane * 4) =
        make_uint2(cvt_pk_bf16_f32(res.x, res.y), cvt_pk_bf16_f32(res.z, res.w));
  else
    *reinterpret_cast<float4 *>(reinterpret_cast<float *>(outv) + ((size_t)b * Np + p) * 256 + lane * 4) = res;
}

}

using namespace unopose;

extern "C" {

int unopose_upproj_plan(const long long *choose, int B2, int Np, int H, int W, int side, int tok_offset, int tok_stride, int cap_rows,
                        int *ws, int *row_list, int *cellmap, int *tile_info, unopose_stream_t stream) {
  UNOPOSE_REQUIRE(choose && ws && row_list && cellmap && tile_info, "upproj_plan: null pointer");
  UNOPOSE_REQUIRE(B2 >= 1 && B2 <= 65535 && Np >= 1 && H >= 1 && W >= 1 && side >= 1 && side <= 256 && tok_offset >= 0 &&
                      tok_stride >= tok_offset + side * side && cap_rows >= 0 && cap_rows % 256 == 0,
                  "upproj_plan: bad sizes");
  UNOPOSE_REQUIRE((long)B2 * tok_stride < (1L << 31), "upproj_plan: too many activation rows");
  {
    const long per_crop = std::min<long>(4L * Np, 16L * side * side);
    UNOPOSE_REQUIRE(cap_rows >= B2 * per_crop + 16 * 256, "upproj_plan: cap_rows %d below the worst case %ld (B2 * min(4 Np, cells) + 16 * 256)",
                    cap_rows, B2 * per_crop + 16 * 256);
  }
  hipStream_t s = (hipStream_t)stream;
  const size_t cells = (size_t)B2 * 16 * side * side;
  int *flags = ws, *counts = ws + cells, *offsets = counts + 16 * B2;
  hipLaunchKernelGGL(upproj_clear_kernel, dim3((unsigned)std::min<long>(((long)cells + cap_rows + 255) / 256, 2048)), dim3(256), 0, s, flags, (long)cells,
                     row_list, (long)cap_rows);
  hipLaunchKernelGGL(upproj_mark_kernel, dim3(cdiv(Np, 256), B2), dim3(256), 0, s, choose, Np, H, W, side, flags);
  hipLaunchKernelGGL(upproj_count_kernel, dim3(B2), dim3(256), 0, s, flags, side, B2, counts);
  hipLaunchKernelGGL(upproj_offsets_kernel, dim3(1), dim3(64), 0, s, counts, B2, offsets, tile_info);
  hipLaunchKernelGGL(upproj_fill_kernel, dim3(B2), dim3(512), 0, s, flags, offsets, side, B2, tok_offset, tok_stride, row_list,
                     cellmap);
  return check_launch("upproj_plan");
}

int unopose_bilinear_sample_compact(const void *Cc, const int *cellmap, const long long *choose, int B2, int side, int Np, int H, int W,
                                    void *out, int out_bf16, unopose_stream_t stream) {
  UNOPOSE_REQUIRE(Cc && cellmap && choose && out, "bilinear_sample_compact: null pointer");
  UNOPOSE_REQUIRE(B2 >= 0 && B2 <= 65535 && side >= 1 && Np >= 0 && H >= 1 && W >= 1, "bilinear_sample_compact: bad sizes");
  if (B2 == 0 || Np == 0) return UNOPOSE_OK;
  if (out_bf16)
    hipLaunchKernelGGL(bilinear_sample_compact_kernel<true>, dim3(cdiv(Np, 4), B2), dim3(256), 0, (hipStream_t)stream, (const u16 *)Cc, cellmap,
                       choose, side, Np, H, W, out);
  else
    hipLaunchKernelGGL(bilinear_sample_compact_kernel<false>, dim3(cdiv(Np, 4), B2), dim3(256), 0, (hipStream_t)stream, (const u16 *)Cc, cellmap,
                       choose, side, Np, H, W, out);
  return check_launch("bilinear_sample_compact");
}

}
```

### unopose_amd/csrc/vit_attn.hip

```cpp
#include "common.h"
#include "gemm_common.h"

namespace unopose {

typedef __bf16 bf16x4 __attribute__((ext_vector_type(4)));

constexpr int VA_CHUNK = 128;
constexpr int VA_LDK = 64 + 8;
constexpr int VA_VSUB = 128 * 16 + 64;
typedef short s16x4 __attribute__((ext_vector_type(4)));


constexpr float VA_DEFER = 8.f;
constexpr int VA_BUF = VA_CHUNK * VA_LDK + 4 * VA_VSUB;

template <int QB, int NBUF, int NW>
__global__ __launch_bounds__(NW * 64) __attribute__((amdgpu_waves_per_eu(QB == 1 ? 3 : 2, QB == 1 ? 4 : 2))) void vit_attn_kernel(const u16 *__restrict__ qkv, int T, int H, int BH, int nq,
                                                       float scale_log2e, u16 *__restrict__ out) {
  extern __shared__ __attribute__((aligned(16))) u16 smem[];
  u16 (*Ot)[32][72] = reinterpret_cast<u16 (*)[32][72]>(smem);
  static_assert(NW * 32 * 72 <= NBUF * VA_BUF, "output staging must fit the chunk buffers");
  constexpr int NT = NW * 64;
  const int xcd = blockIdx.x & 7, slot = blockIdx.x >> 3;
  const int bh = (slot / nq) * 8 + xcd, qblk = slot % nq;
// ... 134 lines not shown
      }
    }
  };

  auto chunk_compute = [&](int c0, const u16 *buf) {
    const int nk = min(VA_CHUNK, T - c0);
    int kt = 0;
    for (; kt + 32 <= nk; kt += 32) {
      f32x16 s[QB];
      qk_tile(buf, kt, s);
      softmax_pv_tile(buf, kt, s);
    }
    if (kt < nk) {
      f32x16 s[QB];
      qk_tile(buf, kt, s);
#pragma unroll
      for (int qb = 0; qb < QB; ++qb)
#pragma unroll
        for (int r = 0; r < 16; ++r)
          if (c0 + kt + (r & 3) + 8 * (r >> 2) + 4 * hb >= T) s[qb][r] = -3e38f;
      softmax_pv_tile(buf, kt, s);
    }
  };

  const int nchunks = (T + VA_CHUNK - 1) / VA_CHUNK;
  if (NBUF == 1) {
    chunk_load(0);
    for (int c = 0; c < nchunks; ++c) {
      __syncthreads();
      chunk_store(c * VA_CHUNK, smem);
      if (c + 1 < nchunks) chunk_load((c + 1) * VA_CHUNK);
      __syncthreads();
      if (active) chunk_compute(c * VA_CHUNK, smem);
    }
  } else {
    chunk_load(0);
    chunk_store(0, smem);
    if (nchunks > 1) chunk_load(VA_CHUNK);
    __syncthreads();
    for (int c = 0; c < nchunks; ++c) {
      if (active) chunk_compute(c * VA_CHUNK, smem + (c & 1) * VA_BUF);
      if (c + 1 < nchunks) {
        chunk_store((c + 1) * VA_CHUNK, smem + ((c + 1) & 1) * VA_BUF);
        if (c + 2 < nchunks) chunk_load((c + 2) * VA_CHUNK);
      }
      __syncthreads();
    }
  }
  __syncthreads();
  if (!active) return;
#pragma unroll
  for (int qb = 0; qb < QB; ++qb) {
    const float inv = 1.f / l_run[qb];
#pragma unroll
    for (int t = 0; t < 2; ++t)
#pragma unroll
      for (int r = 0; r < 16; ++r) {
        const int c = t * 32 + (r & 3) + 8 * (r >> 2) + 4 * hb;
        Ot[wave][col][c] = f2bf(o[qb][t][r] * inv);
      }
    __builtin_amdgcn_fence(__ATOMIC_RELEASE, "wavefront");
    __builtin_amdgcn_wave_barrier();
    __builtin_amdgcn_fence(__ATOMIC_ACQUIRE, "wavefront");
#pragma unroll
    for (int it = 0; it < 4; ++it) {
      const int row = it * 8 + (lane >> 3), seg = lane & 7;
      const int tq = q0 + qb * 32 + row;
      if (tq < T) {
        const uint4 v = *reinterpret_cast<const uint4 *>(&Ot[wave][row][seg * 8]);
        *reinterpret_cast<uint4 *>(out + ((size_t)b * T + tq) * (H * 64) + h * 64 + seg * 8) = v;
      }
    }
    __builtin_amdgcn_fence(__ATOMIC_RELEASE, "wavefront");
    __builtin_amdgcn_wave_barrier();
    __builtin_amdgcn_fence(__ATOMIC_ACQUIRE, "wavefront");
  }
}


constexpr int VD_KBYTES = VA_CHUNK * 128;
constexpr int VD_VSUBB = 128 * 32 + 128;
constexpr int VD_BUFB = VD_KBYTES + 4 * VD_VSUBB;

template <int NW>
__global__ __launch_bounds__(NW * 64, 2) void vit_attn_kernel_dma(const u16 *__restrict__ qkv, int T, int H, int BH, int nq, float scale_log2e,
                                                               u16 *__restrict__ out) {
  constexpr int QB = 2, NBUF = 2, NPC = 32 / NW;
  extern __shared__ __attribute__((aligned(1024))) char smemd[];
  u16 (*Ot)[32][72] = reinterpret_cast<u16 (*)[32][72]>(smemd);
  static_assert(NW * 32 * 72 * 2 <= NBUF * VD_BUFB, "output staging must fit the chunk buffers");
  const int xcd = blockIdx.x & 7, slot = blockIdx.x >> 3;
  const int bh = (slot / nq) * 8 + xcd, qblk = slot % nq;
  if (bh >= BH) return;
  const int b = bh / H, h = bh % H;
  const int tid = threadIdx.x, lane = tid & 63, wave = __builtin_amdgcn_readfirstlane(tid >> 6);
  const int q0 = (qblk * NW + wave) * (32 * QB);
  const bool active = q0 < T;
  const int col = lane & 31, hb = lane >> 5;
  const int C3 = 3 * H * 64;
  const u16 *base = qkv + (size_t)b * T * C3;
  const uint32_t lds0 = (uint32_t)(uintptr_t)(__attribute__((address_space(3))) char *)smemd;
  const __amdgpu_buffer_rsrc_t rs = __builtin_amdgcn_make_buffer_rsrc((void *)base, 0, (int)((size_t)T * C3 * 2), 0x00020000);
  uint32_t kvo[NPC / 2], vvo[NPC / 2], kdst[NPC / 2], vdst[NPC / 2];
#pragma unroll
  for (int i = 0; i < NPC / 2; ++i) {
    const int p = (NPC / 2) * wave + i;
    const int krow = 8 * p + (lane >> 3), gch = (lane & 7) ^ ((krow >> 1) & 7);
    kvo[i] = (uint32_t)(krow * C3 * 2 + (H * 64 + h * 64) * 2 + gch * 16);
    kdst[i] = (uint32_t)(p * 1024);
    const int sub = p >> 2, vkey = 32 * (p & 3) + (lane >> 1);
    vvo[i] = (uint32_t)(vkey * C3 * 2 + (2 * H * 64 + h * 64 + sub * 16 + (lane & 1) * 8) * 2);
    vdst[i] = (uint32_t)(VD_KBYTES + sub * VD_VSUBB + (p & 3) * 1024);
  }
  auto issue_chunk = [&](int c, int bslot) {
    const uint32_t b0 = lds0 + bslot * VD_BUFB, ro = (uint32_t)(c * VA_CHUNK) * (uint32_t)(C3 * 2);
#pragma unroll
    for (int i = 0; i < NPC / 2; ++i) gemm_dma16(b0 + kdst[i], kvo[i] + ro, rs, 0);
#pragma unroll
    for (int i = 0; i < NPC / 2; ++i) gemm_dma16(b0 + vdst[i], vvo[i] + ro, rs, 0);
  };
  const int nchunks = (T + VA_CHUNK - 1) / VA_CHUNK;
  issue_chunk(0, 0);

  bf16x8 qf[QB][4];
#pragma unroll
  for (int qb = 0; qb < QB; ++qb) {
    const int tq = min(q0 + qb * 32 + col, T - 1);
    const u16 *qp = base + (size_t)tq * C3 + h * 64 + hb * 8;
#pragma unroll
    for (int ks = 0; ks < 4; ++ks) qf[qb][ks] = *reinterpret_cast<const bf16x8 *>(qp + ks * 16);
  }
#pragma unroll
  for (int qb = 0; qb < QB; ++qb)
#pragma unroll
    for (int ks = 0; ks < 4; ++ks) asm volatile("" : "+v"(qf[qb][ks]));
  f32x16 o[QB][2];
  float m_run[QB], l_run[QB];
#pragma unroll
  for (int qb = 0; qb < QB; ++qb) {
    m_run[qb] = -3e38f;
    l_run[qb] = 0.f;
#pragma unroll
    for (int t = 0; t < 2; ++t)
#pragma unroll
      for (int r = 0; r < 16; ++r) o[qb][t][r] = 0.f;
  }
  uint32_t koff[4];
#pragma unroll
  for (int ks = 0; ks < 4; ++ks) koff[ks] = (uint32_t)(col * 128 + (((2 * ks + hb) ^ ((col >> 1) & 7)) << 4));
  const uint32_t vlane_off = (uint32_t)(VD_KBYTES + ((lane >> 4) & 1) * VD_VSUBB + (4 * hb + ((lane & 15) >> 2)) * 32 + (lane & 3) * 8);

  auto tile = [&](const char *buf, int c0, int kt, bool partial) {
    f32x16 s[QB];
#pragma unroll
    for (int qb = 0; qb < QB; ++qb)
#pragma unroll
      for (int r = 0; r < 16; ++r) s[qb][r] = 0.f;
#pragma unroll
    for (int ks = 0; ks < 4; ++ks) {
      const bf16x8 kf = *reinterpret_cast<const bf16x8 *>(buf + kt * 128 + koff[ks]);
#pragma unroll
      for (int qb = 0; qb < QB; ++qb) s[qb] = __builtin_amdgcn_mfma_f32_32x32x16_bf16(kf, qf[qb][ks], s[qb], 0, 0, 0);
    }
    if (partial) {
#pragma unroll
      for (int qb = 0; qb < QB; ++qb)
#pragma unroll
        for (int r = 0; r < 16; ++r)
          if (c0 + kt + (r & 3) + 8 * (r >> 2) + 4 * hb >= T) s[qb][r] = -3e38f;
    }
    const char *vlane = buf + vlane_off;
    union PF { bf16x8 v; uint32_t w[4]; } pf[QB][2];
    float alpha[QB];
    bool moved = false;
#pragma unroll
    for (int qb = 0; qb < QB; ++qb) {
      float mx = s[qb][0];
#pragma unroll
      for (int r = 1; r < 16; ++r) mx = fmaxf(mx, s[qb][r]);
      const auto sm = __builtin_amdgcn_permlane32_swap(__float_as_uint(mx), __float_as_uint(mx), false, false);
      mx = fmaxf(__uint_as_float(sm[0]), __uint_as_float(sm[1])) * scale_log2e;
      const bool grow = mx > m_run[qb] + VA_DEFER;
      const float m_use = grow ? mx : m_run[qb];
      alpha[qb] = __builtin_amdgcn_exp2f(m_run[qb] - m_use);
      m_run[qb] = m_use;
      moved |= grow;
      float ls = 0.f;
#pragma unroll
      for (int r = 0; r < 16; ++r) {
        s[qb][r] = __builtin_amdgcn_exp2f(fmaf(s[qb][r], scale_log2e, -m_use));
        ls += s[qb][r];
      }
      const auto sw = __builtin_amdgcn_permlane32_swap(__float_as_uint(ls), __float_as_uint(ls), false, false);
      l_run[qb] = fmaf(l_run[qb], alpha[qb], __uint_as_float(sw[0]) + __uint_as_float(sw[1]));
#pragma unroll
      for (int s2 = 0; s2 < 2; ++s2)
#pragma unroll
        for (int e = 0; e < 4; ++e) pf[qb][s2].w[e] = cvt_pk_bf16_f32(s[qb][s2 * 8 + 2 * e], s[qb][s2 * 8 + 2 * e + 1]);
    }
    auto v_frag = [&](int s2, int t) {
      const char *vp = vlane + t * 2 * VD_VSUBB + (kt + s2 * 16) * 32;
      union { bf16x8 v; s16x4 h4[2]; } vf;
      vf.h4[0] = __builtin_amdgcn_ds_read_tr16_b64_v4i16((s16x4 __attribute__((address_space(3))) *)(vp));
      vf.h4[1] = __builtin_amdgcn_ds_read_tr16_b64_v4i16((s16x4 __attribute__((address_space(3))) *)(vp + 8 * 32));
      return vf.v;
    };
#pragma unroll
    for (int s2 = 0; s2 < 2; ++s2)
#pragma unroll
      for (int t = 0; t < 2; ++t) {
        const bf16x8 vf = v_frag(s2, t);
#pragma unroll
        for (int qb = 0; qb < QB; ++qb) o[qb][t] = __builtin_amdgcn_mfma_f32_32x32x16_bf16(vf, pf[qb][s2].v, o[qb][t], 0, 0, 0);
      }
    if (__builtin_expect(__any(moved), 0)) {
#pragma unroll
      for (int t = 0; t < 2; ++t) {
        const bf16x8 v0 = v_frag(0, t), v1 = v_frag(1, t);
#pragma unroll
        for (int qb = 0; qb < QB; ++qb) {
          f32x16 d;
#pragma unroll
          for (int r = 0; r < 16; ++r) d[r] = 0.f;
          d = __builtin_amdgcn_mfma_f32_32x32x16_bf16(v0, pf[qb][0].v, d, 0, 0, 0);
          d = __builtin_amdgcn_mfma_f32_32x32x16_bf16(v1, pf[qb][1].v, d, 0, 0, 0);
#pragma unroll
          for (int r = 0; r < 16; ++r) o[qb][t][r] = fmaf(o[qb][t][r] - d[r], alpha[qb], d[r]);
        }
      }
    }
  };

  asm volatile("s_waitcnt vmcnt(0)" ::: "memory");
  __builtin_amdgcn_s_barrier();
  asm volatile("" ::: "memory");
  for (int c = 0; c < nchunks; ++c) {
    if (c + 1 < nchunks) issue_chunk(c + 1, (c + 1) & 1);
    if (active) {
      const int c0 = c * VA_CHUNK, nk = min(VA_CHUNK, T - c0);
      const char *buf = smemd + (c & 1) * VD_BUFB;
      int kt = 0;
      for (; kt + 32 <= nk; kt += 32) tile(buf, c0, kt, false);
      if (kt < nk) tile(buf, c0, kt, true);
    }
    asm volatile("s_waitcnt vmcnt(0) lgkmcnt(0)" ::: "memory");
    __builtin_amdgcn_s_barrier();
    asm volatile("" ::: "memory");
  }
  if (!active) return;
#pragma unroll
  for (int qb = 0; qb < QB; ++qb) {
    const float inv = 1.f / l_run[qb];
#pragma unroll
    for (int t = 0; t < 2; ++t)
#pragma unroll
      for (int r = 0; r < 16; ++r) Ot[wave][col][t * 32 + (r & 3) + 8 * (r >> 2) + 4 * hb] = f2bf(o[qb][t][r] * inv);
    __builtin_amdgcn_fence(__ATOMIC_RELEASE, "wavefront");
    __builtin_amdgcn_wave_barrier();
    __builtin_amdgcn_fence(__ATOMIC_ACQUIRE, "wavefront");
#pragma unroll
    for (int it = 0; it < 4; ++it) {
      const int row = it * 8 + (lane >> 3), seg = lane & 7;
      const int tq = q0 + qb * 32 + row;
      if (tq < T) {
        const uint4 v = *reinterpret_cast<const uint4 *>(&Ot[wave][row][seg * 8]);
        *reinterpret_cast<uint4 *>(out + ((size_t)b * T + tq) * (H * 64) + h * 64 + seg * 8) = v;
      }
    }
    __builtin_amdgcn_fence(__ATOMIC_RELEASE, "wavefront");
    __builtin_amdgcn_wave_barrier();
    __builtin_amdgcn_fence(__ATOMIC_ACQUIRE, "wavefront");
  }
}

}

using namespace unopose;

static int launch_vit_attn_dma(const void *qkv, int B, int T, int H, void *out, hipStream_t stream) {
  constexpr int NW = 4;
  static bool opt[64];
  const size_t lds = (size_t)2 * VD_BUFB;
  if (lds_optin(opt, reinterpret_cast<const void *>(&vit_attn_kernel_dma<NW>), lds, "vit_attention") != UNOPOSE_OK) return UNOPOSE_ELAUNCH;
  const int BH = B * H, nq = cdiv(T, 32 * NW * 2);
  const long blocks = (long)cdiv(BH, 8) * nq * 8;
  hipLaunchKernelGGL((vit_attn_kernel_dma<NW>), dim3((unsigned)blocks), dim3(NW * 64), lds, stream, (const u16 *)qkv, T, H, BH, nq,
                     0.125f * 1.4426950408889634f, (u16 *)out);
  return check_launch("vit_attention");
}

template <int QB, int NBUF, int NW>
static int launch_vit_attn(const void *qkv, int B, int T, int H, void *out, hipStream_t stream) {
  static bool opt[64];
  const size_t lds = (size_t)NBUF * VA_BUF * sizeof(u16);
  if (lds_optin(opt, reinterpret_cast<const void *>(&vit_attn_kernel<QB, NBUF, NW>), lds, "vit_attention") != UNOPOSE_OK) return UNOPOSE_ELAUNCH;
  const int BH = B * H, nq = cdiv(T, 32 * NW * QB);
  const float scale_log2e = 0.125f * 1.4426950408889634f;
  const long blocks = (long)cdiv(BH, 8) * nq * 8;
  hipLaunchKernelGGL((vit_attn_kernel<QB, NBUF, NW>), dim3((unsigned)blocks), dim3(NW * 64), lds, stream, (const u16 *)qkv, T,
                     H, BH, nq, scale_log2e, (u16 *)out);
  return check_launch("vit_attention");
}

static int vit_attn_route(int T, int H) {
  if (T >= 1024) return (size_t)T * 3 * H * 64 * 2 < (1UL << 31) ? 2 : 3;
  return T >= 512 ? 1 : 0;
}

extern "C" {

int unopose_vit_attention_route(int T, int H) { return vit_attn_route(T, H); }

int unopose_vit_attention(const void *qkv, int B, int T, int H, void *out, unopose_stream_t stream) {
  UNOPOSE_REQUIRE(qkv && out, "vit_attention: null pointer");
  UNOPOSE_REQUIRE(B >= 0 && T >= 1 && H >= 1 && (long)B * H * cdiv(T, 128) < (1L << 31), "vit_attention: bad sizes");
  if (B == 0) return UNOPOSE_OK;
  switch (vit_attn_route(T, H)) {
    case 3: return launch_vit_attn<2, 2, 8>(qkv, B, T, H, out, (hipStream_t)stream);
    case 2: return launch_vit_attn_dma(qkv, B, T, H, out, (hipStream_t)stream);
    case 1: return launch_vit_attn<2, 2, 4>(qkv, B, T, H, out, (hipStream_t)stream);
    default: return launch_vit_attn<1, 1, 4>(qkv, B, T, H, out, (hipStream_t)stream);
  }
}

}
```

### unopose_amd/model/modules.py

```python
import math

import torch
import torch.nn as nn
import torch.nn.functional as F

from .. import ops


class _Attention(nn.Module):
    def __init__(self, dim, heads):
        super().__init__()
        self.heads = heads
        self.qkv = nn.Linear(dim, 3 * dim)
        self.proj = nn.Linear(dim, dim)

    def forward(self, x):
        B, T, C = x.shape
        qkv = ops.linear(x, self.qkv)
        o = ops.vit_attention(qkv, self.heads)
        return ops.linear(o, self.proj)


class _LayerScale(nn.Module):
    def __init__(self, dim):
        super().__init__()
        self.gamma = nn.Parameter(torch.full((dim,), 1e-5))


class _Mlp(nn.Module):
    def __init__(self, dim, ratio=4):
        super().__init__()
        self.fc1 = nn.Linear(dim, ratio * dim)
        self.fc2 = nn.Linear(ratio * dim, dim)

    def forward(self, x):
        return ops.mlp(x, self.fc1, self.fc2)


class _Block(nn.Module):
    def __init__(self, dim, heads):
        super().__init__()
        self.norm1 = nn.LayerNorm(dim, eps=1e-6)
        self.attn = _Attention(dim, heads)
        self.ls1 = _LayerScale(dim)
        self.norm2 = nn.LayerNorm(dim, eps=1e-6)
        self.mlp = _Mlp(dim)
        self.ls2 = _LayerScale(dim)

    def forward_fused(self, x, n1, next_norm):
        y = self.attn(n1)
        n2 = ops.scale_residual_layernorm_(x, y, self.ls1.gamma, self.norm2)
        y = self.mlp(n2)
        if next_norm is None:
            ops.scale_residual_(x, y, self.ls2.gamma)
            return x, None
        return x, ops.scale_residual_layernorm_(x, y, self.ls2.gamma, next_norm)

    def forward_folded(self, x, n1, xb, stats):
        a = self.attn
        qkv = ops.linear(n1, a.qkv) if n1 is not None else ops.linear_lnfold(xb, stats, a.qkv, self.norm1)
        xb, stats = ops.linear_residual_(x, ops.vit_attention(qkv, a.heads), a.proj, self.ls1.gamma, stats)
        h = ops.linear_lnfold(xb, stats, self.mlp.fc1, self.norm2, gelu=True)
        return ops.linear_residual_(x, h, self.mlp.fc2, self.ls2.gamma, stats)

    def forward_fused_f32(self, x, n1s, next_norm):
        B, T, C = x.shape
        rows = B * T
        a, m = self.attn, self.mlp
        cq = ops._f32x3_weights(a.qkv)
        qkv_s = ops.linear_f32x3(n1s, cq[1], cq[2], rows, 3 * C, C, out="split")
        cp = ops._f32x3_weights(a.proj)
        y = ops.linear_f32x3(ops.vit_attention_f32_ss(qkv_s, B, T, a.heads), cp[1], cp[2], rows, C, C).reshape(B, T, C)
        n2s = ops.scale_residual_layernorm_f32_(x, y, self.ls1.gamma, self.norm2)
        c1, c2 = ops._f32x3_weights(m.fc1), ops._f32x3_weights(m.fc2)
        hs = ops.linear_f32x3(n2s, c1[1], c1[2], rows, 4 * C, C, gelu=True, out="split")
        y = ops.linear_f32x3(hs, c2[1], c2[2], rows, C, 4 * C).reshape(B, T, C)
        if next_norm is None:
            return ops.scale_residual_layernorm_f32_(x, y, self.ls2.gamma, None), None
        return x, ops.scale_residual_layernorm_f32_(x, y, self.ls2.gamma, next_norm)

    def forward(self, x):
        if torch.is_autocast_enabled() and x.dtype == torch.float32 and x.is_cuda and not ops.is_differentiable():
            x = x.contiguous()
            y = self.attn(ops.add_layernorm(x, None, self.norm1, torch.bfloat16))
            ops.scale_residual_(x, y, self.ls1.gamma)
            y = self.mlp(ops.add_layernorm(x, None, self.norm2, torch.bfloat16))
            return ops.scale_residual_(x, y, self.ls2.gamma)
        x = x + self.attn(self.norm1(x)) * self.ls1.gamma
        return x + self.mlp(self.norm2(x)) * self.ls2.gamma


class _PatchEmbed(nn.Module):
    def __init__(self, dim, patch):
        super().__init__()
        self.proj = nn.Conv2d(3, dim, patch, patch)


SPARSE_SINGLE_CROP = True
F32_PROLOGUE = True
F32_TAPS_SPLIT = True


class SplitTaps:

    def __init__(self, split, B, T, K):
        self.split, self.B, self.T, self.K = split, B, T, K


class ViT(nn.Module):

    def __init__(self, embed_dim=768, depth=12, num_heads=12, patch_size=14, img_size=224, reg_tokens=4):
        super().__init__()
        self.patch_size, self.depth = patch_size, depth
        self.patch_embed = _PatchEmbed(embed_dim, patch_size)
        self.cls_token = nn.Parameter(torch.zeros(1, 1, embed_dim))
        self.reg_token = nn.Parameter(torch.zeros(1, reg_tokens, embed_dim))
        self.pos_embed = nn.Parameter(torch.zeros(1, (img_size // patch_size) ** 2, embed_dim))
        self.blocks = nn.ModuleList([_Block(embed_dim, num_heads) for _ in range(depth)])
        self.norm = nn.LayerNorm(embed_dim, eps=1e-6)
        self.head = nn.Linear(embed_dim, 1000)

    def forward(self, x, taps_side_by_side=False):
        xa, xb = x if isinstance(x, (tuple, list)) else (x, None)
        if ops.vit_prologue_ok(xa, self) and (xb is None or xb.shape[1:] == xa.shape[1:]):
            x, n1, mean = ops.vit_prologue(xa, xb, self, self.blocks[0].norm1, row_mean=True)
            return self._fused_blocks(x, n1, taps_side_by_side, mean)
        if F32_PROLOGUE and ops.vit_prologue_f32_ok(xa, self) and (xb is None or xb.shape[1:] == xa.shape[1:]):
            x, ns = ops.vit_prologue_f32(xa, xb, self, self.blocks[0].norm1)
            return self._fused_blocks_f32(x, ns, taps_side_by_side)
        x = xa if xb is None else torch.cat([xa, xb], 0)
        B = x.shape[0]
        p = self.patch_size
        gh, gw = x.shape[2] // p, x.shape[3] // p
        patches = x.reshape(B, 3, gh, p, gw, p).permute(0, 2, 4, 1, 3, 5).reshape(B, gh * gw, 3 * p * p)
        x = ops.patch_embed(patches, self.patch_embed.proj)
        x = x + self.pos_embed
        x = torch.cat([self.cls_token.expand(B, -1, -1).to(x.dtype), self.reg_token.expand(B, -1, -1).to(x.dtype), x], 1)
        n = self.depth // 4
        taps = {self.depth - 1, self.depth - n - 1, self.depth - 2 * n - 1, self.depth - 3 * n - 1}
        outs = []
        if x.is_cuda and torch.is_autocast_enabled() and x.dtype == torch.float32 and x.shape[-1] % 4 == 0 \
                and not ops.is_differentiable():
            x = x.contiguous()
            return self._fused_blocks(x, ops.add_layernorm(x, None, self.blocks[0].norm1, torch.bfloat16), taps_side_by_side)
        if ops.vit_f32_fused_ok(x, self):
            x = x.contiguous()
            return self._fused_blocks_f32(x, ops.scale_residual_layernorm_f32_(x, None, None, self.blocks[0].norm1), taps_side_by_side)
        for i, blk in enumerate(self.blocks):
            x = blk(x)
            if i in taps:
                outs.append(ops.add_layernorm(x, None, self.norm)
                            if x.is_cuda and torch.is_autocast_enabled() and not ops.is_differentiable() else self.norm(x))
        return outs

    def _fused_blocks_f32(self, x, ns, taps_side_by_side):
        n = self.depth // 4
        taps = {self.depth - 1, self.depth - n - 1, self.depth - 2 * n - 1, self.depth - 3 * n - 1}
        outs = []
        wide = torch.empty(x.shape[0] * x.shape[1], 2 * 4 * x.shape[2], dtype=torch.bfloat16, device=x.device) if taps_side_by_side and F32_TAPS_SPLIT else None
        for i, blk in enumerate(self.blocks):
            x, ns = blk.forward_fused_f32(x, ns, self.blocks[i + 1].norm1 if i + 1 < len(self.blocks) else None)
            if i in taps:
                if wide is not None:
                    ops.scale_residual_layernorm_f32_(x, None, None, self.norm, wide=wide, block=len(outs))
                    outs.append(None)
                else:
                    outs.append(self.norm(x))
        return SplitTaps(wide, x.shape[0], x.shape[1], 4 * x.shape[2]) if wide is not None else outs


def _vit_fused_blocks(self, x, n1, taps_side_by_side, row_mean=None):
    n = self.depth // 4
    taps = {self.depth - 1, self.depth - n - 1, self.depth - 2 * n - 1, self.depth - 3 * n - 1}
    outs = []
    B, _, D = x.shape
    wide = torch.empty(B, x.shape[1], len(taps) * D, dtype=torch.bfloat16, device=x.device) if taps_side_by_side else None
    fold = ops.ln_fold_ok(B * x.shape[1], D, x.device)
    if fold and row_mean is None:
        row_mean = ops.fold_row_means(x)
    xb, stats = None, row_mean
    for i, blk in enumerate(self.blocks):
        nxt = self.blocks[i + 1].norm1 if i + 1 < len(self.blocks) else None
        if fold:
            xb, stats = blk.forward_folded(x, n1, xb, stats)
            n1 = None
        else:
            x, n1 = blk.forward_fused(x, n1, nxt)
        if i in taps:
            k = len(outs)
            outs.append(ops.add_layernorm(x, None, self.norm, out=None if wide is None else wide[:, :, k * D:(k + 1) * D]))
    return outs if wide is None else wide


ViT._fused_blocks = _vit_fused_blocks


def interpolate_pos_embed(pos_embed_ckpt, new_side):
    P0, C = pos_embed_ckpt.shape[-2:]
    s0 = int(P0 ** 0.5)
    if s0 == new_side:
        return pos_embed_ckpt
    t = pos_embed_ckpt.reshape(-1, s0, s0, C).permute(0, 3, 1, 2)
    t = F.interpolate(t, size=(new_side, new_side), mode="bicubic", align_corners=False)
    return t.permute(0, 2, 3, 1).flatten(1, 2)


class ViT_AE(nn.Module):

    def __init__(self, cfg):
        super().__init__()
        assert cfg.up_type == "linear" and cfg.use_pyramid_feat, "only the configured variant is built"
        assert "reg4" in cfg.vit_type and "patch14" in cfg.vit_type
        dims = {"vit_small": (384, 12, 6), "vit_base": (768, 12, 12), "vit_large": (1024, 24, 16)}
        D, depth, heads = dims[cfg.vit_type[:cfg.vit_type.index("_patch")]]
        assert D == cfg.embed_dim
        self.out_dim = cfg.out_dim
        self.img_size = cfg.get("img_size", 224)
        self.vit = ViT(D, depth, heads, 14, self.img_size)
        self.output_upscaling = nn.Linear(4 * D, 16 * cfg.out_dim, bias=True)
        if cfg.get("pretrained", False):
            self.load_dinov2(cfg.vit_ckpt)

    def load_dinov2(self, path):
        ck = torch.load(path, map_location="cpu")["model"]
        sd = self.vit.state_dict()
        for k in ("head.weight", "head.bias"):
            if k in ck and ck[k].shape != sd[k].shape:
                del ck[k]
        if "pos_embed" in ck:
            ck["pos_embed"] = interpolate_pos_embed(ck["pos_embed"], self.img_size // 14)
        self.vit.load_state_dict(ck, strict=False)

    def lowres_map(self, x):
        B, _, H, W = x.shape
        side = H // 14
        outs = self.vit(x)
        z = torch.cat([o[:, 5:, :] for o in outs], dim=2)
        z = ops.linear(z, self.output_upscaling).reshape(B, side, side, 4, 4, self.out_dim)
        return z.permute(0, 1, 3, 2, 4, 5).reshape(B, 4 * side, 4 * side, self.out_dim), (H, W)

    def upprojected(self, x):
        B, _, H, W = x.shape
        side = H // 14
        outs = self.vit(x)
        z = torch.cat([o[:, 5:, :] for o in outs], dim=2)
        return ops.linear(z, self.output_upscaling).reshape(B, side, side, 4, 4, self.out_dim), (H, W)

    def upprojected_tokens(self, x):
        B, _, H, W = x.shape
        return self.upproject(self.vit(x, taps_side_by_side=True), H, W)

    def upproject(self, outs, H, W):
        if isinstance(outs, SplitTaps):
            lin = self.output_upscaling
            c = ops._f32x3_weights(lin)
            z = ops.linear_f32x3(outs.split, c[1], c[2], outs.B * outs.T, lin.weight.shape[0], outs.K)
            return z.reshape(outs.B, outs.T, 4, 4, self.out_dim), (H, W), outs.T - (H // 14) * (W // 14)
        B = outs.shape[0] if torch.is_tensor(outs) else outs[0].shape[0]
        if torch.is_tensor(outs):
            z = ops.linear(outs, self.output_upscaling)
            return z.reshape(B, outs.shape[1], 4, 4, self.out_dim), (H, W), outs.shape[1] - (H // 14) * (W // 14)
        z = ops.linear(torch.cat([o[:, 5:, :] for o in outs], dim=2), self.output_upscaling)
        return z.reshape(B, -1, 4, 4, self.out_dim), (H, W), 0

    def pixel_features(self, x, choose):
        if x.is_cuda and self.out_dim == 256 and not ops.is_differentiable():
            if SPARSE_SINGLE_CROP and ops.sparse_upproj_ok(x) and x.shape[-1] == x.shape[-2] and x.shape[-1] % 14 == 0:
                sd = x.shape[-1] // 14
                npre = self.vit.cls_token.shape[1] + self.vit.reg_token.shape[1]
                plan = ops.upproj_plan(choose, x.shape[-2], x.shape[-1], sd, npre, npre + sd * sd)
                acts = self.vit(x, taps_side_by_side=True)
                if torch.is_tensor(acts) and acts.shape[1] == plan["tok_stride"]:
                    return ops.sparse_pixel_features(acts, self.output_upscaling, plan)
                z, (H, W), off = self.upproject(acts, x.shape[-2], x.shape[-1])
                return ops.bilinear_sample_native(z, choose, H, W, tok_offset=off)
            z, (H, W), off = self.upprojected_tokens(x)
            return ops.bilinear_sample_native(z, choose, H, W, tok_offset=off)
        low, (H, W) = self.lowres_map(x)
        return ops.bilinear_sample_pixels(low, choose, H, W)


class ViTEncoderOneRef(nn.Module):
    def __init__(self, cfg, npoint=None):
        super().__init__()
        self.npoint = npoint
        self.rgb_net = ViT_AE(cfg)


class SinusoidalPositionalEmbedding(nn.Module):
    def __init__(self, d_model):
        super().__init__()
        self.d_model = d_model
        div = torch.exp(torch.arange(0, d_model, 2).float() * (-math.log(10000.0) / d_model))
        self.register_buffer("div_term", div)


class GeometricStructureEmbedding(nn.Module):

    def __init__(self, cfg):
        super().__init__()
        self.sigma_d, self.sigma_a, self.angle_k = cfg.sigma_d, cfg.sigma_a, cfg.angle_k
        self.factor_a = 180.0 / (self.sigma_a * math.pi)
        self.embedding = SinusoidalPositionalEmbedding(cfg.hidden_dim)
        self.proj_d = nn.Linear(cfg.hidden_dim, cfg.hidden_dim)
        self.proj_a = nn.Linear(cfg.hidden_dim, cfg.hidden_dim)
        self.reduction_a = cfg.reduction_a
        if self.reduction_a not in ("max", "mean"):
            raise ValueError(f"Unsupported reduction mode: {self.reduction_a}.")

    def forward(self, points):
        return ops.geo_embedding(points, self)


class _MHA(nn.Module):
    def __init__(self, d, rpe):
        super().__init__()
        self.proj_q = nn.Linear(d, d)
        self.proj_k = nn.Linear(d, d)
        self.proj_v = nn.Linear(d, d)
        if rpe:
            self.proj_p = nn.Linear(d, d)


class _AttentionLayer(nn.Module):
    def __init__(self, d, rpe):
        super().__init__()
        self.attention = _MHA(d, rpe)
        self.linear = nn.Linear(d, d)
        self.norm = nn.LayerNorm(d)


class _AttentionOutput(nn.Module):
    def __init__(self, d):
        super().__init__()
        self.expand = nn.Linear(d, 2 * d)
        self.squeeze = nn.Linear(2 * d, d)
        self.norm = nn.LayerNorm(d)

    def forward(self, x, out=None):
        if x.is_cuda and not ops.is_differentiable():
            return ops.ffn_add_layernorm(x, self.expand, self.squeeze, self.norm, out=out)
        assert out is None
        return ops.add_layernorm_train(x, ops.linear(ops.linear(x, self.expand, relu=True), self.squeeze), self.norm)


class TransformerLayer(nn.Module):

    def __init__(self, d, rpe, heads=4):
        super().__init__()
        self.heads = heads
        self.attention = _AttentionLayer(d, rpe)
        self.output = _AttentionOutput(d)

    def forward(self, x, mem, embed=None, out=None):
# ... 226 lines not shown
```

### unopose_amd/model/unopose.py

```python

import torch
import torch.nn as nn
import torch.nn.functional as F

from .. import ops
from ..losses import aug_pose_noise, overlap_losses
from .config import to_cfg
from .modules import (GeometricStructureEmbedding, GeometricTransformer, PositionalEncoding,
                      SparseToDenseTransformer, ViTEncoderOneRef, _adjacent)


STACKED_FINE = True
PE_UNDER_COARSE = True
GEOM_UNDER_VIT = 1
LRF_UNDER_VIT = True
_SIDE_STREAMS = {}
COARSE_SLOT = True
TRAIN_PE_UNDER_COARSE = True


def _scores(scores, n1, halves=False):
    return ops.overlap_scores(scores, n1, halves=halves)


# ... 180 lines not shown
            scores = ops.score_head(torch.cat((f1, f2), dim=1), self.score_heads[self.nblock - 1])
            o1, o2 = ops.linear(f1, self.out_proj), ops.linear(f2, self.out_proj)
            if self.taps is None and ops.fine_pose_fused_ok(o1, o2):
                R, t, s = ops.fine_pose_from_features(o1, o2, self.cfg.temp, _scores(scores, n1), p1, p2)
                return self._finish(end_points, R, t, s, radius)
            atten = ops.feature_similarity(o1, o2, self.cfg.temp)
        score = _scores(scores, n1)
        if self.taps is not None:
            self.taps.update(f1=f1, f2=f2, atten=atten, score=score)
        R, t, s = ops.fine_pose(atten, score, p1, p2)
        return self._finish(end_points, R, t, s, radius)

    @staticmethod
    def _finish(end_points, R, t, s, radius):
        end_points["pred_R"] = R
        end_points["pred_t"] = ops.scale_by_radius(t, radius, multiply=True)
        end_points["pred_pose_score"] = s
        return end_points


class UNOPose(nn.Module):
    def __init__(self, cfg):
        super().__init__()
        cfg = to_cfg(cfg)
        self.cfg = cfg
        self.coarse_npoint = cfg.coarse_npoint
        self.fine_npoint = cfg.fine_npoint
        self.use_ref_rad = cfg.get("use_ref_rad", False)
        self.test_coarse_only = cfg.get("test_coarse_only", False)
        self.feature_extraction = ViTEncoderOneRef(cfg.feature_extraction, self.fine_npoint)
        self.geo_embedding = GeometricStructureEmbedding(cfg.geo_embedding)
        self.coarse_point_matching = CoarsePointMatchingOneRef(cfg.coarse_point_matching)
        self.fine_point_matching = FinePointMatchingOneRef(cfg.fine_point_matching)
        self.taps = None
        self.fixed_init = None
        self._zero_rows = {}
        self.internal_overlap = True

    def _features(self, end_points):
        rgb, choose = end_points["rgb"], end_points["rgb_choose"]
        assert choose.size(1) == self.fine_npoint
        net = self.feature_extraction.rgb_net
        dense_pm = end_points["pts"]
        if "dense_po" in end_points and "dense_fo" in end_points:
            dense_fm = net.pixel_features(rgb, choose)
            dense_po, dense_fo = end_points["dense_po"].clone(), end_points["dense_fo"].clone()
            radius = ops.cloud_radius(dense_po)
            dense_pm = ops.scale_by_radius(dense_pm, radius)
            dense_po = ops.scale_by_radius(dense_po, radius)
            return dense_pm, dense_fm, dense_po, dense_fo, radius, None
        if "ref_dense_po" in end_points:
            radius = end_points["ref_radius"]
            dense_pm = ops.scale_by_radius(dense_pm, radius)
            return dense_pm, net.pixel_features(rgb, choose), end_points["ref_dense_po"], end_points["ref_dense_fo"], radius, None
        tem_rgb, tem_choose, tem_pts = end_points["tem1_rgb"], end_points["tem1_choose"], end_points["tem1_pts"]
        radius = ops.cloud_radius(tem_pts)
        dense_pm = ops.scale_by_radius(dense_pm, radius)
        tem_n = ops.scale_by_radius(tem_pts, radius)
        main = torch.cuda.current_stream()
        side = self._side_stream(tem_n.device)
        side.wait_stream(main)
        with torch.cuda.stream(side):
            idx_o = ops.furthest_point_sample(tem_n, self.fine_npoint)
            dense_po = ops.gather_rows(tem_n, idx_o)
            sparse_up = (ops.sparse_upproj_ok(rgb) and idx_o.shape == choose.shape and net.out_dim == 256 and rgb.shape == tem_rgb.shape
                         and tem_choose.dtype == choose.dtype and tem_choose.is_contiguous())
            if sparse_up:
                both_choose = torch.empty(2 * choose.shape[0], choose.shape[1], dtype=choose.dtype, device=choose.device)
                both_choose[:choose.shape[0]].copy_(choose)
                sel_choose = ops.gather_rows(tem_choose.unsqueeze(-1), idx_o, out=both_choose[choose.shape[0]:].unsqueeze(-1)).squeeze(-1)
            else:
                sel_choose = torch.gather(tem_choose, 1, idx_o.long())
            for t in (idx_o, dense_po, sel_choose):
                t.record_stream(main)
            plan = None
            if sparse_up:
                sd = rgb.shape[-1] // 14
                npre = net.vit.cls_token.shape[1] + net.vit.reg_token.shape[1]
                both_choose.record_stream(main)
                plan = ops.upproj_plan(both_choose, rgb.shape[-2], rgb.shape[-1], sd, npre, npre + sd * sd)
                for t in plan.values():
                    if torch.is_tensor(t):
                        t.record_stream(main)
            pre = None
            if GEOM_UNDER_VIT and self.internal_overlap:
                pre = {}
                pre["idx_m"] = ops.furthest_point_sample(dense_pm, self.coarse_npoint)
                pre["idx_o"] = ops.furthest_point_sample(dense_po, self.coarse_npoint)
                pre["sparse_pm"] = ops.gather_rows(dense_pm.float(), pre["idx_m"])
                pre["sparse_po"] = ops.gather_rows(dense_po.float(), pre["idx_o"])
                if GEOM_UNDER_VIT > 1 or LRF_UNDER_VIT:
                    pre["sparse_pm_lrf"] = ops.gather_rows(ops.lrf_global(end_points["pts"], self.use_ref_rad), pre["idx_m"])
                    pre["sparse_po_lrf"] = ops.gather_rows(ops.lrf_global(tem_pts, self.use_ref_rad), pre["idx_o"])
                if GEOM_UNDER_VIT > 1:
                    bg_point = torch.ones(dense_pm.size(0), 1, 3, device=dense_pm.device)
                    pre["geo"] = self.geo_embedding(torch.cat([torch.cat([bg_point, pre["sparse_pm_lrf"]], dim=1),
                                                               torch.cat([bg_point, pre["sparse_po_lrf"]], dim=1)], dim=0))
                for t in pre.values():
                    t.record_stream(main)
        B = rgb.shape[0]
        if plan is not None:
            acts = net.vit((rgb, tem_rgb), taps_side_by_side=True)
            if torch.is_tensor(acts) and acts.shape[1] == plan["tok_stride"]:
                main.wait_stream(side)
                both = ops.sparse_pixel_features(acts, net.output_upscaling, plan)
                return dense_pm, both[:B], dense_po, both[B:], radius, pre
            z, (H, W), off = net.upproject(acts, rgb.shape[-2], rgb.shape[-1])
        else:
            z, (H, W), off = net.upproject(net.vit((rgb, tem_rgb), taps_side_by_side=True), rgb.shape[-2], rgb.shape[-1])
        both = torch.empty(2 * B, choose.shape[1], 256, dtype=torch.float32, device=z.device) \
            if sel_choose.shape == choose.shape else None
        dense_fm = ops.bilinear_sample_native(z[:B], choose, H, W, out=None if both is None else both[:B], tok_offset=off)
        main.wait_stream(side)
        dense_fo = ops.bilinear_sample_native(z[B:], sel_choose, H, W, out=None if both is None else both[B:], tok_offset=off)
        return dense_pm, dense_fm, dense_po, dense_fo, radius, pre

    @torch.no_grad()
    def encode_reference(self, tem1_rgb, tem1_choose, tem1_pts):
        radius = ops.cloud_radius(tem1_pts)
        tem_n = ops.scale_by_radius(tem1_pts, radius)
        idx_o = ops.furthest_point_sample(tem_n, self.fine_npoint)
        sel_choose = torch.gather(tem1_choose, 1, idx_o.long())
        net = self.feature_extraction.rgb_net
        return dict(ref_dense_po=ops.gather_rows(tem_n, idx_o), ref_dense_fo=net.pixel_features(tem1_rgb, sel_choose),
                    ref_radius=radius, ref_lrf=ops.lrf_global(tem1_pts, self.use_ref_rad))

    def _side_stream(self, device):
        cur = torch.cuda.current_stream(device)
        key = (torch.device(device).index if torch.device(device).index is not None else torch.cuda.current_device(), cur.cuda_stream)
        if key not in _SIDE_STREAMS:
            _SIDE_STREAMS[key] = torch.cuda.Stream(device=device)
        return _SIDE_STREAMS[key]

    def _sample_wlrf(self, pts, pts_lrf, feats, npoint):
        idx = ops.furthest_point_sample(pts, npoint)
        return ops.gather_rows(pts.float(), idx), ops.gather_rows(pts_lrf, idx), ops.gather_rows(feats, idx), idx

    def _lowres_train(self, rgb):
        net = self.feature_extraction.rgb_net
        frozen = not any(p.requires_grad for p in net.vit.parameters())
        if frozen:
            with torch.no_grad(), ops.differentiable(False):
                taps = net.vit(rgb)
        else:
            taps = net.vit(rgb)
        B, _, H, W = rgb.shape
        side = H // 14
        z = torch.cat([o[:, 5:, :] for o in taps], dim=2).float()
        z = ops.linear(z, net.output_upscaling).reshape(B, side, side, 4, 4, net.out_dim)
        return z.permute(0, 1, 3, 2, 4, 5).reshape(B, 4 * side, 4 * side, net.out_dim)

    def _pixel_features_train(self, rgb, choose):
        return ops.bilinear_sample_pixels(self._lowres_train(rgb), choose, rgb.shape[-2], rgb.shape[-1])

    def forward_train(self, end_points):
        tem_pts = end_points["tem1_pts"]
        radius = torch.norm(tem_pts - tem_pts.mean(1, keepdim=True), dim=2).max(1)[0]
        scale = radius.reshape(-1, 1, 1) + 1e-6
        dense_pm, tem_n = end_points["pts"] / scale, tem_pts / scale
        main = torch.cuda.current_stream() if dense_pm.is_cuda else None
        side = self._side_stream(dense_pm.device) if main is not None and self.internal_overlap else None
        geo = {}

        def geometry():
            with torch.no_grad():
                geo["idx_o"] = ops.furthest_point_sample(tem_n, self.fine_npoint)
                geo["dense_po"] = ops.gather_rows(tem_n, geo["idx_o"])
                geo["sel_choose"] = torch.gather(end_points["tem1_choose"], 1, geo["idx_o"].long())
                geo["pm_lrf"] = ops.lrf_global(end_points["pts"], self.use_ref_rad)
                geo["po_lrf"] = ops.lrf_global(tem_pts, self.use_ref_rad)
                geo["fps_m"] = ops.furthest_point_sample(dense_pm, self.coarse_npoint)
                geo["fps_o"] = ops.furthest_point_sample(geo["dense_po"], self.coarse_npoint)

        if side is not None:
            side.wait_stream(main)
            with torch.cuda.stream(side):
                geometry()
                for t in geo.values():
                    t.record_stream(main)
            low_m = self._lowres_train(end_points["rgb"])
            low_o = self._lowres_train(end_points["tem1_rgb"])
            main.wait_stream(side)
        else:
            geometry()
            low_m = self._lowres_train(end_points["rgb"])
# ... 146 lines not shown
```

### unopose_amd/ops/__init__.py

```python
import sys
import types

from . import _state
from .common import (
    _c, differentiable, is_differentiable, _fallbacks_seen, note_fallback, _params_key, _SPLIT_MEMO, _MUTATION_EPOCH, note_mutation,
    clear_split_memo, _aligned16, _no_autograd, _f32_path, _own_f32, _own_glue,
)
from .dense import (
    linear_backend, _bf16_weights, linear_bf16_hip, own_gemm_ok, bf16_linear_2d, f32x3_ok, split_f32, _f32x3_weights, linear_f32x3,
    linear_f32x3_bf16, linear_f32_raw, _transposed_weights, _LinearFn, _ZERO_BIAS, _zero_bias, linear_train, _lin, mlp, linear,
    ffn_add_layernorm, linear_add_layernorm, patch_embed, vit_prologue_ok, vit_prologue, vit_prologue_f32_ok, vit_prologue_f32, bmm_nt_f32, score_head, add_layernorm,
    _AddLayerNormFn, add_layernorm_train_ok, add_layernorm_train,
    scale_residual_, scale_residual_layernorm_f32_, vit_f32_fused_ok, scale_residual_layernorm_, ln_fold_ok, _fold_producer_weights,
    _fold_consumer_weights, linear_residual_, linear_lnfold, fold_shift, fold_row_means, _into,
)
from .attention import (
    vit_attention, vit_attention_f32_split, vit_attention_f32_ss, vit_attention_torch, _KEY_PAD, token_attention,
    _token_attention_hip_f32, _attn_weights, _token_attention_hip, token_attention_torch, _key_pad, _transpose_pad_f32, _TokenAttnFn,
    token_attention_train_ok, _token_attention_train, focused_linear_attention,
    _focused_linear_attention_hip_f32, _focused_linear_attention_hip, focused_linear_attention_torch,
)
from .geometry import (
    lrf_global, query_lrf_group, lrf_group_idx, weighted_procrustes, cloud_radius, scale_by_radius, gather_rows, pairwise_distance,
    _bf16_split, _mfma_fragment_order, _GEO_HINV, _GEO_D_RANGE, _GEO_TABLE_UNAVAILABLE, _geo_tables, geo_embedding, geo_embedding_torch,
    pe_group_mlp_max, pe_group_mlp_max_unfused, pe_geometry, pe_mlp_max, _pe_image, furthest_point_sample, _geo_grid, _GeoEmbedFn, geo_embedding_train_ok,
)
from .sampling import (
    bilinear_sample_native, sparse_upproj_ok, upproj_plan, sparse_pixel_features, bilinear_sample_pixels,
)
from .pose import (
    overlap_scores, set_first_rows_, pose_score, rigid_rows, feature_similarity, soft_assignment, coarse_pose_torch, fine_pose_torch, _assign_labels, _check_score_width,
    coarse_pose, fine_pose, fine_pose_fused_ok, normalize_rows_bf16, normalize_rows_f32, fine_pose_from_features,
)
from .prep import (
    PrepPlan, _desc_ints, _tap_table, prep_norm_table, _require, _result, prep_crop_resize, prep_lift, prep_gather,
)
from .augment import AugTables, color_augment, finish_crops
from .rle import pack_segs, rle_decode, rle_encode, window_masks
from .score import vsd_counts, pose_errors, pose_metrics, adi, gt_visibility, pts_extent, ref_select
from .vis import compose_poses
from .train import (
    _InfoNCEFn, infonce_two_way, _BNReLUTrain, bn_relu, _BNReLUMaxPoolTrain, bn_relu_maxpool, _SaliencyFn, saliency_pair,
    nearest_partner, _CONV_FWD_PAIRS, _CONV_WGRAD_PAIRS, _conv1x1_pair_ok, _conv1x1_wgrad_ok, _Conv1x1Fn, conv1x1,
)

_SWITCHES = frozenset(['FORBID_LIBRARY_BF16_GEMM', 'GEO_TABLE', 'GEO_TABLE_F32', 'HIP_GEMM_ALL', 'PIXEL_FEATS_BF16', 'TRAIN_FUSED_SALIENCY', 'TRAIN_OWN_ATTN', 'TRAIN_OWN_CONV', 'TRAIN_OWN_GEMM', 'TRAIN_OWN_GEMM_MIN_FLOP', 'TRAIN_OWN_GEO', 'TRAIN_OWN_LN', 'TRAIN_OWN_WGRAD', 'TRAIN_OWN_WGRAD_MIN_ROWS', 'USE_F32X3', 'USE_FUSED_BN_RELU', 'USE_FUSED_FINE', 'USE_FUSED_INFONCE', 'USE_FUSED_LINEAR_LN', 'USE_HIP_GEMM', 'USE_KV_VT', 'USE_LA_KV_STATE', 'USE_LN_FOLD', 'USE_OWN_TOPK', 'USE_SPARSE_UPPROJ', 'USE_STACKED_OUT', '_DIFF'])


class _OpsModule(types.ModuleType):

    def __getattr__(self, name):
        if name in _SWITCHES:
            return getattr(_state, name)
        raise AttributeError(f"module {self.__name__!r} has no attribute {name!r}")

    def __setattr__(self, name, value):
        if name in _SWITCHES:
            setattr(_state, name, value)
        else:
            super().__setattr__(name, value)

    def __delattr__(self, name):
        if name in _SWITCHES:
            raise AttributeError(f"{name} is a switch of ops._state and cannot be deleted")
        super().__delattr__(name)


sys.modules[__name__].__class__ = _OpsModule
```

### unopose_amd/ops/attention.py

```python
import ctypes

import torch
import torch.nn.functional as F

from .._lib import call, lib, on_device, ptr, stream_ptr
from . import _state as st
from .common import _c, _own_f32, _own_glue, _params_key, note_fallback
from .dense import _lin, bf16_linear_2d, bmm_nt_f32, linear, linear_f32_raw


def vit_attention(qkv, heads):
    if st._DIFF:
        return vit_attention_torch(qkv, heads)
    if qkv.dtype == torch.bfloat16 and qkv.shape[-1] == 3 * heads * 64:
        B, T, C3 = qkv.shape
        qkv = _c(qkv)
        out = torch.empty(B, T, C3 // 3, dtype=torch.bfloat16, device=qkv.device)
        with on_device(qkv.device):
            call("unopose_vit_attention", ptr(qkv), B, T, heads, ptr(out), stream_ptr())
        return out
    if qkv.dtype == torch.float32 and qkv.is_cuda and qkv.shape[-1] == 3 * heads * 64:
        B, T, C3 = qkv.shape
        qkv = _c(qkv)
        out = torch.empty(B, T, C3 // 3, dtype=torch.float32, device=qkv.device)
        with on_device(qkv.device):
            call("unopose_vit_attention_f32", ptr(qkv), B, T, heads, ptr(out), stream_ptr())
        return out
    note_fallback("vit_attention", f"head dim {qkv.shape[-1] // (3 * heads)} / dtype {qkv.dtype} (kernels: head dim 64, bf16 or fp32)")
    return vit_attention_torch(qkv, heads)


def vit_attention_f32_split(qkv, heads):
    B, T, C3 = qkv.shape
    assert qkv.dtype == torch.float32 and qkv.is_cuda and C3 == 3 * heads * 64
    qkv = _c(qkv)
    out = torch.empty(B * T, 2 * (C3 // 3), dtype=torch.bfloat16, device=qkv.device)
    with on_device(qkv.device):
        call("unopose_vit_attention_f32_split", ptr(qkv), B, T, heads, ptr(out), stream_ptr())
    return out


def vit_attention_f32_ss(qkv_split, B, T, heads):
    C3 = qkv_split.shape[-1] // 2
    assert qkv_split.dtype == torch.bfloat16 and qkv_split.is_cuda and qkv_split.is_contiguous() and C3 == 3 * heads * 64
    out = torch.empty(B * T, 2 * (C3 // 3), dtype=torch.bfloat16, device=qkv_split.device)
    with on_device(qkv_split.device):
        call("unopose_vit_attention_f32_ss", ptr(qkv_split), B, T, heads, ptr(out), stream_ptr())
    return out


def vit_attention_torch(qkv, heads):
    B, T, C3 = qkv.shape
    C = C3 // 3
    hd = C // heads
    q, k, v = qkv.reshape(B, T, 3, heads, hd).permute(2, 0, 3, 1, 4)
    sm = torch.float64 if qkv.dtype == torch.float64 else torch.float32
    a = torch.softmax((q * hd ** -0.5) @ k.transpose(-2, -1), dim=-1, dtype=sm).to(v.dtype) @ v
    return a.transpose(1, 2).reshape(B, T, C)


_KEY_PAD = None


def _key_pad():
    global _KEY_PAD
    if _KEY_PAD is None:
        _KEY_PAD = lib().unopose_token_attention_key_pad()
    return _KEY_PAD


def token_attention(x, mem, att, heads, embed=None):
    if st._DIFF and torch.is_grad_enabled() and token_attention_train_ok(x, mem, att, heads, embed):
        return _token_attention_train(x, mem, att, embed)
    if not st._DIFF and x.is_cuda and heads == 4 and x.shape[-1] == 256:
        if mem.shape[1] <= _key_pad():
            if torch.is_autocast_enabled():
                return _token_attention_hip(x, mem, att, embed)
            if x.dtype == torch.float32:
                return _token_attention_hip_f32(x, mem, att, embed)
    if not st._DIFF and x.is_cuda:
        note_fallback("token_attention", f"heads {heads} x width {x.shape[-1]}, {mem.shape[1]} keys, dtype {x.dtype} (kernels: 4 x 64, up to the padded key count)")
    return token_attention_torch(x, mem, att, heads, embed)


def _token_attention_hip_f32(x, mem, att, embed):

    B, n, C = x.shape
    m = mem.shape[1]
    rpe = embed is not None
    key = _params_key(att, rpe, "f32")
    cache = getattr(att, "_hip_cache_f32", None)
    if cache is None or cache[0] != key:
        with torch.no_grad():
            wq, bq = att.proj_q.weight.float(), att.proj_q.bias.float()
            pw, pb = [wq], [bq]
            if rpe:
                wp = att.proj_p.weight.float().reshape(4, 64, 256)
                pw.append(torch.einsum("hcd,hci->hdi", wp, wq.reshape(4, 64, 256)).reshape(1024, 256))
                pb.append(torch.einsum("hcd,hc->hd", wp, bq.reshape(4, 64)).reshape(1024))
            cache = (key, torch.cat(pw, 0).contiguous(), torch.cat(pb, 0).contiguous(),
                     torch.cat([att.proj_k.weight.float(), att.proj_v.weight.float()], 0).contiguous(),
                     torch.cat([att.proj_k.bias.float(), att.proj_v.bias.float()], 0).contiguous())
        att._hip_cache_f32 = cache
    _, w_q, b_q, w_kv, b_kv = cache
    yq = linear_f32_raw(x, w_q, b_q, att, "q")
    ykv = linear_f32_raw(mem, w_kv, b_kv, att, "kv")
    if ykv.is_contiguous() and C % 32 == 0 and m <= _KEY_PAD:
        vt = torch.empty(B, C, _KEY_PAD, dtype=torch.float32, device=x.device)
        with on_device(x.device):
            call("unopose_transpose_pad_f32", ctypes.c_void_p(ykv.data_ptr() + C * 4), ykv.stride(1), B, m, C, _KEY_PAD, ptr(vt), stream_ptr())
    else:
        vt = torch.zeros(B, C, _KEY_PAD, dtype=torch.float32, device=x.device)
# ... 278 lines not shown
```

### unopose_amd/ops/dense.py

```python
import ctypes

import torch
import torch.nn.functional as F

from .._lib import call, lib, on_device, ptr, stream_ptr
from . import _state as st
from .common import _MUTATION_EPOCH, _SPLIT_MEMO, _aligned16, _c, _f32_path, _no_autograd, _params_key, note_fallback, note_mutation


def linear_backend():
    if st.USE_HIP_GEMM and st.HIP_GEMM_ALL:
        return "csrc/gemm.hip (256x256x64 LDS-DMA tiles, persistent; bias / bias + erf-GELU epilogue) for every ViT linear"
    if st.USE_HIP_GEMM:
        return "hipBLASLt (through torch); fc1 + GELU: csrc/gemm.hip (256x256x64 LDS-DMA tiles, fused bias + erf-GELU epilogue)"
    return "hipBLASLt (through torch)"


def _bf16_weights(lin):
    key = _params_key(lin)
    cache = getattr(lin, "_bf16_cache", None)
    if cache is None or cache[0] != key:
        with torch.no_grad():
            b32 = torch.zeros(lin.weight.shape[0], device=lin.weight.device) if lin.bias is None else lin.bias.detach().float().contiguous()
            cache = (key, lin.weight.detach().to(torch.bfloat16).contiguous(),
# ... 544 lines not shown
    assert x.dtype == torch.float32 and x.is_contiguous() and y.dtype == torch.bfloat16
    y = _c(y)
    C = x.shape[-1]
    with on_device(x.device):
        call("unopose_scale_residual", ptr(x), ptr(y), ptr(gamma), x.numel() // C, C, stream_ptr())
    return x


def scale_residual_layernorm_f32_(x, y, gamma, norm, wide=None, block=0):
    note_mutation()
    assert x.dtype == torch.float32 and x.is_contiguous() and (y is None or y.dtype == torch.float32)
    C = x.shape[-1]
    rows = x.numel() // C
    ld, dst = 0, None
    if wide is not None:
        assert norm is not None and wide.dtype == torch.bfloat16 and wide.is_contiguous() and wide.shape[0] == rows and wide.shape[1] % (2 * C) == 0
        ld = wide.shape[1] * 2
        assert 0 <= block < wide.shape[1] // (2 * C)
        dst = ctypes.c_void_p(wide.data_ptr() + block * C * 4)
    out = None if (norm is None or wide is not None) else torch.empty(rows, 2 * C, dtype=torch.bfloat16, device=x.device)
    with on_device(x.device):
        call("unopose_scale_residual_layernorm_f32", ptr(x), None if y is None else ptr(_c(y)), None if y is None else ptr(gamma),
             None if norm is None else ptr(norm.weight), None if norm is None else ptr(norm.bias), rows, C,
             0.0 if norm is None else float(norm.eps), dst if wide is not None else (None if out is None else ptr(out)), ld, stream_ptr())
    return x if norm is None else (wide if wide is not None else out)


def vit_f32_fused_ok(x, vit):
    C = x.shape[-1]
    return (x.is_cuda and x.dtype == torch.float32 and not st._DIFF and _no_autograd() and not torch.is_autocast_enabled() and st.USE_F32X3 and C % 32 == 0
            and C <= 1024 and C % 64 == 0 and f32x3_ok(x.numel() // C, 3 * C, C) and f32x3_ok(x.numel() // C, C, 4 * C))


def scale_residual_layernorm_(x, y, gamma, norm):
    note_mutation()
    assert x.dtype == torch.float32 and x.is_contiguous() and y.dtype == torch.bfloat16
    y = _c(y)
    C = x.shape[-1]
    out = torch.empty(x.shape, dtype=torch.bfloat16, device=x.device)
    with on_device(x.device):
        call("unopose_scale_residual_layernorm", ptr(x), ptr(y), ptr(gamma), ptr(norm.weight), ptr(norm.bias),
             x.numel() // C, C, float(norm.eps), ptr(out), stream_ptr())
    return out


def ln_fold_ok(rows, C, device=None):
    if not (st.USE_LN_FOLD and st.USE_HIP_GEMM and st.HIP_GEMM_ALL) or C % 256 != 0 or C // 256 > 4 or rows * C * 4 >= 2 ** 31:
        return False
    n_cu = torch.cuda.get_device_properties(torch.cuda.current_device() if device is None else device).multi_processor_count & ~7
    return ((rows + 255) // 256) * (C // 256) >= n_cu * 5 // 8


def _fold_producer_weights(lin, gamma):
    key = (lin.weight._version, lin.weight.data_ptr(), lin.weight.device, None if lin.bias is None else lin.bias._version, gamma._version, gamma.data_ptr())
    cache = getattr(lin, "_fold_prod_cache", None)
    if cache is None or cache[0] != key:
        with torch.no_grad():
            g = gamma.detach().float()
            w = (lin.weight.detach().float() * g[:, None]).to(torch.bfloat16).contiguous()
            b = (torch.zeros_like(g) if lin.bias is None else lin.bias.detach().float() * g).contiguous()
        cache = (key, w, b)
        lin._fold_prod_cache = cache
    return cache


def _fold_consumer_weights(lin, norm):
    key = (lin.weight._version, lin.weight.data_ptr(), lin.weight.device, None if lin.bias is None else lin.bias._version,
           norm.weight._version, norm.weight.data_ptr(), norm.bias._version)
    cache = getattr(lin, "_fold_cons_cache", None)
    if cache is None or cache[0] != key:
        with torch.no_grad():
            w32 = lin.weight.detach().float()
            w = (w32 * norm.weight.detach().float()[None, :]).to(torch.bfloat16).contiguous()
            c = w.float().sum(1).contiguous()
            d = (w32.double() @ norm.bias.detach().double()).float()
            if lin.bias is not None:
                d = d + lin.bias.detach().float()
            d = d.contiguous()
        cache = (key, w, c, d)
        lin._fold_cons_cache = cache
    return cache


def linear_residual_(x, a, lin, gamma, prev=None):
    note_mutation()
    _, w, b = _fold_producer_weights(lin, gamma)
    C, K = w.shape
    rows = x.numel() // C
    rows_p = (rows + 255) // 256 * 256
    assert x.dtype == torch.float32 and x.is_contiguous() and a.dtype == torch.bfloat16 and a.numel() == rows * K
    prev_parts = 0
    if prev is not None:
        assert prev.dtype == torch.float32 and prev.device == x.device and prev.shape[0] == rows_p and prev.is_contiguous()
        if prev.dim() == 3:
            prev_parts = prev.shape[1]
            assert prev_parts == C // 256 and prev.untyped_storage().nbytes() >= (prev.storage_offset() + prev.numel() + rows_p) * 4
        else:
            assert prev.dim() == 1
    a = _c(a)
    xb = torch.empty(x.shape, dtype=torch.bfloat16, device=x.device)
    buf = torch.empty(rows_p * (2 * (C // 256) + 1), dtype=torch.float32, device=x.device)
    stats = buf[:rows_p * 2 * (C // 256)].view(rows_p, C // 256, 2)
    with on_device(x.device):
        call("unopose_linear_bf16_residual", ptr(a), ptr(w), ptr(b), ptr(x), ptr(xb), ptr(stats), None if prev is None else ptr(prev), prev_parts,
             rows, C, K, stream_ptr())
    return xb, stats


def fold_shift(stats):
    return torch.as_strided(stats, (stats.shape[0],), (1,), stats.storage_offset() + stats.numel())


def fold_row_means(x):
    C = x.shape[-1]
    rows = x.numel() // C
    mean = torch.zeros((rows + 255) // 256 * 256, dtype=torch.float32, device=x.device)
    with torch.autocast(x.device.type, enabled=False):
        torch.mean(x.reshape(rows, C), 1, out=mean[:rows])
    return mean


def linear_lnfold(xb, stats, lin, norm, gelu=False):
    _, w, c, d = _fold_consumer_weights(lin, norm)
    N, K = w.shape
    rows = xb.numel() // K
    out = torch.empty(*xb.shape[:-1], N, dtype=torch.bfloat16, device=xb.device)
    with on_device(xb.device):
        call("unopose_linear_bf16_lnfold", ptr(xb), ptr(w), ptr(d), ptr(c), ptr(stats), K // 256, float(norm.eps), ptr(out), rows, N, K, int(gelu), stream_ptr())
    return out
```

### unopose_amd/ops/sampling.py

```python
import torch

from .._lib import call, on_device, ptr, stream_ptr
from . import _state as st
from .common import _c, note_mutation
from .dense import _bf16_weights


def bilinear_sample_native(z, choose, H, W, out=None, tok_offset=0):
    z = _c(z)
    assert z.shape[-1] == 256 and z.shape[-2] == 4 and z.shape[-3] == 4 and z.dtype in (torch.float32, torch.bfloat16)
    if out is not None:
        note_mutation()
    B = z.shape[0]
    if z.dim() == 5:
        tok_stride = z.shape[1]
        side = int(round((tok_stride - tok_offset) ** 0.5))
        assert side * side + tok_offset == tok_stride
    else:
        assert z.dim() == 6 and tok_offset == 0
        side = z.shape[1]
        tok_stride = side * side
    choose = _c(choose.long())
    Np = choose.shape[1]
    if out is None:
        out = torch.empty(B, Np, 256, dtype=torch.float32, device=z.device)
    assert out.shape == (B, Np, 256) and out.dtype == torch.float32 and out.is_contiguous()
    with on_device(z.device):
        call("unopose_bilinear_sample_tokens", ptr(z), int(z.dtype == torch.bfloat16), ptr(choose), B, side, Np, int(H),
             int(W), int(tok_offset), int(tok_stride), ptr(out), stream_ptr())
    return out


def sparse_upproj_ok(x):
    return st.USE_SPARSE_UPPROJ and x.is_cuda and torch.is_autocast_enabled() and not st._DIFF


def upproj_plan(choose, H, W, side, tok_offset, tok_stride):
    choose = _c(choose.long())
    B2, Np = choose.shape
    cells = 16 * side * side
    cap_rows = (B2 * min(4 * Np, cells) + 16 * 256 + 255) // 256 * 256
    dev = choose.device
    i32 = dict(dtype=torch.int32, device=dev)
    plan = dict(choose=choose, H=int(H), W=int(W), side=int(side), tok_offset=int(tok_offset), tok_stride=int(tok_stride),
                cap_rows=cap_rows, ws=torch.empty(B2 * (cells + 32), **i32), row_list=torch.empty(cap_rows, **i32),
                cellmap=torch.empty(B2 * cells, **i32), tile_info=torch.empty(18, **i32))
    with on_device(dev):
        call("unopose_upproj_plan", ptr(choose), B2, Np, int(H), int(W), int(side), int(tok_offset), int(tok_stride), cap_rows,
             ptr(plan["ws"]), ptr(plan["row_list"]), ptr(plan["cellmap"]), ptr(plan["tile_info"]), stream_ptr())
    return plan


def sparse_pixel_features(acts, lin, plan, out=None):
    acts = _c(acts)
    if out is not None:
        note_mutation()
    B2, ts, K = acts.shape
    assert acts.dtype == torch.bfloat16 and ts == plan["tok_stride"] and B2 == plan["choose"].shape[0]
    cache = _bf16_weights(lin)
    w, bias = cache[1], cache[3]
    N = w.shape[0]
    assert N == 16 * 256 and w.shape[1] == K
    Np = plan["choose"].shape[1]
    dev = acts.device
    if out is None:
        out = torch.empty(B2, Np, 256, dtype=torch.bfloat16 if st.PIXEL_FEATS_BF16 else torch.float32, device=dev)
    assert out.shape == (B2, Np, 256) and out.dtype in (torch.float32, torch.bfloat16) and out.is_contiguous()
    with on_device(dev):
        cells = torch.empty(plan["cap_rows"], 256, dtype=torch.bfloat16, device=dev)
        call("unopose_linear_bf16_gather", ptr(acts), B2 * ts, K, ptr(w), N, ptr(bias), ptr(plan["row_list"]),
             ptr(plan["tile_info"]), plan["cap_rows"] // 256, ptr(cells), stream_ptr())
        call("unopose_bilinear_sample_compact", ptr(cells), ptr(plan["cellmap"]), ptr(plan["choose"]), B2, plan["side"], Np,
             plan["H"], plan["W"], ptr(out), int(out.dtype == torch.bfloat16), stream_ptr())
    return out


def bilinear_sample_pixels(low, choose, H, W):
    B, h, w, C = low.shape
    ys = torch.div(choose, W, rounding_mode="floor")
    xs = choose - ys * W

    def src(dst, n_in, n_out):
        s = (dst.float() + 0.5) * (n_in / n_out) - 0.5
        s = s.clamp(min=0.0)
        i0 = s.floor().long().clamp(max=n_in - 1)
        i1 = torch.where(i0 < n_in - 1, i0 + 1, i0)
        l1 = s - i0.float()
        return i0, i1, l1

    y0, y1, ly = src(ys, h, H)
    x0, x1, lx = src(xs, w, W)
    flat = low.reshape(B, h * w, C)

    def g(yy, xx):
        return torch.gather(flat, 1, (yy * w + xx).unsqueeze(2).expand(-1, -1, C)).float()

    lx, ly = lx.unsqueeze(2), ly.unsqueeze(2)
    top = (1 - lx) * g(y0, x0) + lx * g(y0, x1)
    bot = (1 - lx) * g(y1, x0) + lx * g(y1, x1)
    return (1 - ly) * top + ly * bot
```

Baseline: 1134 pairs/s.

## Compute last ViT block only on patch tokens needed by sparse up-projection

Adds a live-row plan built from the up-projection cell flags, so that only patch tokens feeding sampled pixels are kept. The final transformer layer's attention output, residual GEMM, LN-folded MLP GEMMs and final layernorm are restricted to these rows. A device-side row count bounds the GEMMs, and a scatter layernorm writes live rows back and zeroes dead ones. This targets dense last-layer work on tokens whose features are never sampled, at the cost of extra gather/scatter kernels and more GEMM template variants.

```diff
diff --git a/include/unopose_hip.h b/include/unopose_hip.h
--- a/include/unopose_hip.h
+++ b/include/unopose_hip.h
@@ -151,6 +151,14 @@
 
 int unopose_upproj_plan(const long long *choose, int B2, int Np, int H, int W, int side, int tok_offset, int tok_stride,
                         int cap_rows, int *ws, int *row_list, int *cellmap, int *tile_info, unopose_stream_t stream);
+int unopose_upproj_live_rows(const int *flags, int B2, int side, int tok_offset, int tok_stride, int *ws, int *live_rows, int *dead_rows,
+                             int *img_info, int *m_live, unopose_stream_t stream);
+int unopose_vit_attention_rows(const void *qkv, int B, int T, int H, const int *row_list, const int *img_info, int out_rows, void *out,
+                               unopose_stream_t stream);
+int unopose_gather_rows_stats(const float *x, const float *stats, long rows, int nparts, const int *row_list, long rows_c, int C, float *xc,
+                              float *stats_c, unopose_stream_t stream);
+int unopose_layernorm_scatter(const float *a, const float *w, const float *bias, long rows, int C, float eps, void *out, long ld_out, long nout,
+                              const int *out_rows, const int *zero_rows, long nzero, unopose_stream_t stream);
 
 int unopose_linear_bf16_ld(const void *A, int lda, const void *W, int ldw, const float *bias, void *C, int ldc, long M, int N, int K,
                            int epilogue, unopose_stream_t stream);
@@ -303,6 +311,10 @@
                                  int prev_nparts, long M, int N, int K, unopose_stream_t stream);
 int unopose_linear_bf16_lnfold(const void *A, const void *W, const float *dvec, const float *cvec, const float *stats, int nparts, float eps,
                                void *C, long M, int N, int K, int gelu, unopose_stream_t stream);
+int unopose_linear_bf16_residual_rows(const void *A, const void *W, const float *bias, float *xres, void *xb, float *stats, const float *prev,
+                                      int prev_nparts, long M, int N, int K, const int *m_dev, unopose_stream_t stream);
+int unopose_linear_bf16_lnfold_rows(const void *A, const void *W, const float *dvec, const float *cvec, const float *stats, int nparts, float eps,
+                                    void *C, long M, int N, int K, int gelu, const int *m_dev, unopose_stream_t stream);
 int unopose_gemm_fold_stagger(int eighth_ticks_per_ktile);
 
 int unopose_bmm_f32(const float *A, long sab, long sah, long sai, long sak, const float *Bm, long sbb, long sbh, long sbj, long sbk,
diff --git a/unopose_amd/_lib.py b/unopose_amd/_lib.py
--- a/unopose_amd/_lib.py
+++ b/unopose_amd/_lib.py
@@ -86,6 +86,12 @@
     "unopose_gemm_fold_stagger": [_I],
     "unopose_linear_bf16_residual": [_P, _P, _P, _P, _P, _P, _P, _I, ctypes.c_long, _I, _I, _P],
     "unopose_linear_bf16_lnfold": [_P, _P, _P, _P, _P, _I, _F, _P, ctypes.c_long, _I, _I, _I, _P],
+    "unopose_linear_bf16_residual_rows": [_P, _P, _P, _P, _P, _P, _P, _I, ctypes.c_long, _I, _I, _P, _P],
+    "unopose_linear_bf16_lnfold_rows": [_P, _P, _P, _P, _P, _I, _F, _P, ctypes.c_long, _I, _I, _I, _P, _P],
+    "unopose_upproj_live_rows": [_P, _I, _I, _I, _I, _P, _P, _P, _P, _P, _P],
+    "unopose_vit_attention_rows": [_P, _I, _I, _I, _P, _P, _I, _P, _P],
+    "unopose_gather_rows_stats": [_P, _P, ctypes.c_long, _I, _P, ctypes.c_long, _I, _P, _P, _P],
+    "unopose_layernorm_scatter": [_P, _P, _P, ctypes.c_long, _I, _F, _P, ctypes.c_long, ctypes.c_long, _P, _P, ctypes.c_long, _P],
     "unopose_patchify_bf16": [_P, _I, _P, _I, _I, _I, _P, _P],
     "unopose_patchify_split": [_P, _I, _P, _I, _I, _I, _P, _P],
     "unopose_vit_tokens_layernorm": [_P, _P, _P, _I, _I, _I, _I, _P, _P, _F, _P, _P, _P, _P],
diff --git a/unopose_amd/csrc/fused.hip b/unopose_amd/csrc/fused.hip
--- a/unopose_amd/csrc/fused.hip
+++ b/unopose_amd/csrc/fused.hip
@@ -60,13 +60,27 @@
   }
   return *reinterpret_cast<const float4 *>(reinterpret_cast<const float *>(p) + i);
 }
-template <bool A_BF16, bool B_BF16, bool HAS_B, bool OUT_BF16>
+template <bool A_BF16, bool B_BF16, bool HAS_B, bool OUT_BF16, bool SCATTER = false>
 __global__ __launch_bounds__(256) void add_layernorm_vec4_kernel(const void *__restrict__ a, const void *__restrict__ b,
                                                                  const float *__restrict__ w, const float *__restrict__ bias, long rows,
-                                                                 int C, float eps, void *__restrict__ out, long ldo) {
+                                                                 int C, float eps, void *__restrict__ out, long ldo,
+                                                                 const int *__restrict__ out_rows = nullptr,
+                                                                 const int *__restrict__ zero_rows = nullptr, long nzero = 0, long nout = 0) {
   const long r = (long)blockIdx.x * 4 + (threadIdx.x >> 6);
+  const int lane = threadIdx.x & 63;
+  long ro = r;
+  if (SCATTER) {
+    static_assert(!SCATTER || OUT_BF16, "the scattered form writes bf16");
+    if (r < nzero) {
+      const int z = zero_rows[r];
+      if (z >= 0 && z < nout)
+        for (int c = lane * 4; c < C; c += 256) *reinterpret_cast<uint2 *>(reinterpret_cast<u16 *>(out) + (size_t)z * ldo + c) = make_uint2(0u, 0u);
+    }
+    if (r >= rows) return;
+    ro = out_rows[r];
+    if (ro < 0 || ro >= nout) return;
+  }
   if (r >= rows) return;
-  const int lane = threadIdx.x & 63;
   float4 v[4];
   float s = 0.f;
 #pragma unroll
@@ -107,12 +121,26 @@
         uint2 o;
         o.x = (uint32_t)f2bf(y0) | ((uint32_t)f2bf(y1) << 16);
         o.y = (uint32_t)f2bf(y2) | ((uint32_t)f2bf(y3) << 16);
-        *reinterpret_cast<uint2 *>(reinterpret_cast<u16 *>(out) + (size_t)r * ldo + c) = o;
+        *reinterpret_cast<uint2 *>(reinterpret_cast<u16 *>(out) + (size_t)ro * ldo + c) = o;
       } else {
-        *reinterpret_cast<float4 *>(reinterpret_cast<float *>(out) + (size_t)r * ldo + c) = make_float4(y0, y1, y2, y3);
+        *reinterpret_cast<float4 *>(reinterpret_cast<float *>(out) + (size_t)ro * ldo + c) = make_float4(y0, y1, y2, y3);
       }
     }
   }
+}
+
+__global__ __launch_bounds__(256) void gather_rows_stats_kernel(const float *__restrict__ x, const float *__restrict__ stats, long rows, long rows_p, int nparts,
+                                                                const int *__restrict__ row_list, long rows_c, long rows_c_p, int C,
+                                                                float *__restrict__ xc, float *__restrict__ stats_c) {
+  const long c = (long)blockIdx.x * 4 + (threadIdx.x >> 6);
+  if (c >= rows_c) return;
+  const long r = row_list[c];
+  if (r < 0 || r >= rows) return;
+  const int lane = threadIdx.x & 63;
+  for (int k = lane * 4; k < C; k += 256)
+    *reinterpret_cast<float4 *>(xc + (size_t)c * C + k) = *reinterpret_cast<const float4 *>(x + (size_t)r * C + k);
+  if (lane < 2 * nparts) stats_c[(size_t)c * 2 * nparts + lane] = stats[(size_t)r * 2 * nparts + lane];
+  if (lane == 2 * nparts) stats_c[(size_t)rows_c_p * 2 * nparts + c] = stats[(size_t)rows_p * 2 * nparts + r];
 }
 
 __global__ __launch_bounds__(256) void scale_residual_layernorm_kernel(float *__restrict__ x, const u16 *__restrict__ y,
@@ -333,6 +361,29 @@
   return check_launch("add_layernorm");
 }
 
+int unopose_layernorm_scatter(const float *a, const float *w, const float *bias, long rows, int C, float eps, void *out, long ld_out, long nout,
+                              const int *out_rows, const int *zero_rows, long nzero, unopose_stream_t stream) {
+  UNOPOSE_REQUIRE(a && w && bias && out && out_rows && (zero_rows || nzero == 0), "layernorm_scatter: null pointer");
+  UNOPOSE_REQUIRE(rows >= 0 && nzero >= 0 && nout >= 0 && C >= 4 && C <= 1024 && C % 4 == 0 && ld_out >= C && ld_out % 4 == 0,
+                  "layernorm_scatter: needs C %% 4 == 0 (<= 1024) and ld_out %% 4 == 0, ld_out >= C (got C=%d)", C);
+  const long n = std::max(rows, nzero);
+  if (n == 0) return UNOPOSE_OK;
+  hipLaunchKernelGGL((add_layernorm_vec4_kernel<false, false, false, true, true>), dim3((unsigned)((n + 3) / 4)), dim3(256), 0, (hipStream_t)stream,
+                     (const void *)a, (const void *)nullptr, w, bias, rows, C, eps, out, ld_out, out_rows, zero_rows, nzero, nout);
+  return check_launch("layernorm_scatter");
+}
+
+int unopose_gather_rows_stats(const float *x, const float *stats, long rows, int nparts, const int *row_list, long rows_c, int C, float *xc,
+                              float *stats_c, unopose_stream_t stream) {
+  UNOPOSE_REQUIRE(x && stats && row_list && xc && stats_c, "gather_rows_stats: null pointer");
+  UNOPOSE_REQUIRE(rows >= 1 && rows_c >= 0 && C >= 4 && C % 4 == 0 && nparts >= 1 && nparts <= 16, "gather_rows_stats: bad sizes");
+  if (rows_c == 0) return UNOPOSE_OK;
+  const long rows_p = (rows + 255) / 256 * 256, rows_c_p = (rows_c + 255) / 256 * 256;
+  hipLaunchKernelGGL(gather_rows_stats_kernel, dim3((unsigned)((rows_c + 3) / 4)), dim3(256), 0, (hipStream_t)stream, x, stats, rows, rows_p, nparts,
+                     row_list, rows_c, rows_c_p, C, xc, stats_c);
+  return check_launch("gather_rows_stats");
+}
+
 int unopose_bilinear_sample(const void *z, int z_bf16, const long long *choose, int B, int side, int Np, int H, int W,
                             float *out, unopose_stream_t stream) {
   return unopose_bilinear_sample_tokens(z, z_bf16, choose, B, side, Np, H, W, 0, side * side, out, stream);
diff --git a/unopose_amd/csrc/gemm.hip b/unopose_amd/csrc/gemm.hip
--- a/unopose_amd/csrc/gemm.hip
+++ b/unopose_amd/csrc/gemm.hip
@@ -136,8 +136,8 @@
   return was;
 }
 
-int unopose_linear_bf16_residual(const void *A, const void *W, const float *bias, float *xres, void *xb, float *stats, const float *prev,
-                                 int prev_nparts, long M, int N, int K, unopose_stream_t stream) {
+static int linear_bf16_residual_impl(const void *A, const void *W, const float *bias, float *xres, void *xb, float *stats, const float *prev,
+                                     int prev_nparts, long M, int N, int K, const int *m_dev, unopose_stream_t stream) {
   UNOPOSE_REQUIRE(A && W && bias && xres && xb && stats, "linear_bf16_residual: null pointer");
   UNOPOSE_REQUIRE(prev != stats && (prev_nparts == 0 || (prev && prev_nparts * GEMM_BN == N && prev_nparts <= GEMM_LNF_MAXPARTS)),
                   "linear_bf16_residual: prev must be another buffer with 0 or N / 256 <= %d partials per row (got prev_nparts=%d N=%d)",
@@ -149,14 +149,32 @@
   const int nt = fold_launch_shape(M, N, &grid, &tiles, &tiles_n);
   hipStream_t s = (hipStream_t)stream;
   int *const sched = tiles > grid ? gemm_sched_slot(s) : nullptr;
-  hipLaunchKernelGGL((gemm256_kernel<5>), dim3(grid), dim3(512), 0, s, (const u16 *)A, (const u16 *)W, bias, (u16 *)xb, (int)M, N, K, tiles_n, tiles, nt,
-                     (const int *)nullptr, (const int *)nullptr, (const u16 *)nullptr, (const float *)nullptr, (const float *)nullptr, 0.f, 0, 0, 0, sched,
-                     (void *)xres, (const float *)nullptr, (float2 *)stats, prev_nparts, tiles > grid ? g_fold_stagger * (K / GEMM_BK) / 8 : 0, prev);
+#define UNOPOSE_RES_LAUNCH(MDEV)                                                                                                                        \
+  hipLaunchKernelGGL((gemm256_kernel<5, false, false, MDEV>), dim3(grid), dim3(512), 0, s, (const u16 *)A, (const u16 *)W, bias, (u16 *)xb, (int)M, N, K, \
+                     tiles_n, tiles, nt, (const int *)nullptr, m_dev, (const u16 *)nullptr, (const float *)nullptr, (const float *)nullptr, 0.f, 0, 0,  \
+                     0, sched, (void *)xres, (const float *)nullptr, (float2 *)stats, prev_nparts,                                                      \
+                     tiles > grid ? g_fold_stagger * (K / GEMM_BK) / 8 : 0, prev)
+  if (m_dev)
+    UNOPOSE_RES_LAUNCH(true);
+  else
+    UNOPOSE_RES_LAUNCH(false);
+#undef UNOPOSE_RES_LAUNCH
   return check_launch("linear_bf16_residual");
 }
 
-int unopose_linear_bf16_lnfold(const void *A, const void *W, const float *dvec, const float *cvec, const float *stats, int nparts, float eps, void *C,
-                               long M, int N, int K, int gelu, unopose_stream_t stream) {
+int unopose_linear_bf16_residual(const void *A, const void *W, const float *bias, float *xres, void *xb, float *stats, const float *prev,
+                                 int prev_nparts, long M, int N, int K, unopose_stream_t stream) {
+  return linear_bf16_residual_impl(A, W, bias, xres, xb, stats, prev, prev_nparts, M, N, K, nullptr, stream);
+}
+
+int unopose_linear_bf16_residual_rows(const void *A, const void *W, const float *bias, float *xres, void *xb, float *stats, const float *prev,
+                                      int prev_nparts, long M, int N, int K, const int *m_dev, unopose_stream_t stream) {
+  UNOPOSE_REQUIRE(m_dev, "linear_bf16_residual_rows: null row count");
+  return linear_bf16_residual_impl(A, W, bias, xres, xb, stats, prev, prev_nparts, M, N, K, m_dev, stream);
+}
+
+static int linear_bf16_lnfold_impl(const void *A, const void *W, const float *dvec, const float *cvec, const float *stats, int nparts, float eps, void *C,
+                                   long M, int N, int K, int gelu, const int *m_dev, unopose_stream_t stream) {
   UNOPOSE_REQUIRE(A && W && dvec && cvec && stats && C, "linear_bf16_lnfold: null pointer");
   UNOPOSE_REQUIRE(M >= 1 && M < (1L << 31) && N >= GEMM_BN && N % GEMM_BN == 0 && K >= GEMM_BK && K % GEMM_BK == 0,
                   "linear_bf16_lnfold: needs N %% 256 == 0 and K %% 64 == 0 (got M=%ld N=%d K=%d)", M, N, K);
@@ -166,16 +184,32 @@
   const int nt = fold_launch_shape(M, N, &grid, &tiles, &tiles_n);
   hipStream_t s = (hipStream_t)stream;
   int *const sched = tiles > grid ? gemm_sched_slot(s) : nullptr;
-#define UNOPOSE_LNF_LAUNCH(E)                                                                                                                      \
-  hipLaunchKernelGGL((gemm256_kernel<E>), dim3(grid), dim3(512), 0, s, (const u16 *)A, (const u16 *)W, dvec, (u16 *)C, (int)M, N, K, tiles_n, tiles, nt, \
-                     (const int *)nullptr, (const int *)nullptr, (const u16 *)nullptr, (const float *)nullptr, (const float *)nullptr, eps, 0, 0, 0, sched, \
-                     (void *)nullptr, cvec, (float2 *)stats, nparts)
-  if (gelu)
-    UNOPOSE_LNF_LAUNCH(7);
+#define UNOPOSE_LNF_LAUNCH(E, MDEV)                                                                                                                \
+  hipLaunchKernelGGL((gemm256_kernel<E, false, false, MDEV>), dim3(grid), dim3(512), 0, s, (const u16 *)A, (const u16 *)W, dvec, (u16 *)C, (int)M, N, K, \
+                     tiles_n, tiles, nt, (const int *)nullptr, m_dev, (const u16 *)nullptr, (const float *)nullptr, (const float *)nullptr, eps, 0, 0, \
+                     0, sched, (void *)nullptr, cvec, (float2 *)stats, nparts)
+  if (m_dev) {
+    if (gelu)
+      UNOPOSE_LNF_LAUNCH(7, true);
+    else
+      UNOPOSE_LNF_LAUNCH(6, true);
+  } else if (gelu)
+    UNOPOSE_LNF_LAUNCH(7, false);
   else
-    UNOPOSE_LNF_LAUNCH(6);
+    UNOPOSE_LNF_LAUNCH(6, false);
 #undef UNOPOSE_LNF_LAUNCH
   return check_launch("linear_bf16_lnfold");
 }
 
-}
+int unopose_linear_bf16_lnfold(const void *A, const void *W, const float *dvec, const float *cvec, const float *stats, int nparts, float eps, void *C,
+                               long M, int N, int K, int gelu, unopose_stream_t stream) {
+  return linear_bf16_lnfold_impl(A, W, dvec, cvec, stats, nparts, eps, C, M, N, K, gelu, nullptr, stream);
+}
+
+int unopose_linear_bf16_lnfold_rows(const void *A, const void *W, const float *dvec, const float *cvec, const float *stats, int nparts, float eps,
+                                    void *C, long M, int N, int K, int gelu, const int *m_dev, unopose_stream_t stream) {
+  UNOPOSE_REQUIRE(m_dev, "linear_bf16_lnfold_rows: null row count");
+  return linear_bf16_lnfold_impl(A, W, dvec, cvec, stats, nparts, eps, C, M, N, K, gelu, m_dev, stream);
+}
+
+}
diff --git a/unopose_amd/csrc/gemm_kernel.h b/unopose_amd/csrc/gemm_kernel.h
--- a/unopose_amd/csrc/gemm_kernel.h
+++ b/unopose_amd/csrc/gemm_kernel.h
@@ -38,7 +38,7 @@
   static __device__ __forceinline__ frag mfma(bf16x8 w, bf16x8 a, frag c) { return __builtin_amdgcn_mfma_f32_16x16x32_bf16(w, a, c, 0, 0, 0); }
 };
 
-template <int EPI, bool GATHER = false, bool F32 = false>
+template <int EPI, bool GATHER = false, bool F32 = false, bool MDEV = false>
 __global__ __launch_bounds__(512, 1) __attribute__((amdgpu_num_vgpr(127))) void gemm256_kernel(const void *__restrict__ Av, const void *__restrict__ Wv,
                                                            const float *__restrict__ bias, void *__restrict__ Cv, int M,
                                                            int N, int K, int tiles_n, int tiles_arg, int nt_store,
@@ -52,6 +52,7 @@
                                                            const float *__restrict__ fold_prev = nullptr) {
   static_assert(!(F32 && (EPI == 3 || GATHER)), "the fp32-class form has no LayerNorm epilogue / gathered rows");
   static_assert(!((F32 || GATHER) && EPI >= 5), "the residual / LayerNorm-fold epilogues belong to the dense bf16 form");
+  static_assert(!MDEV || EPI >= 5, "a device-side row count belongs to the residual / LayerNorm-fold epilogues");
   constexpr bool LNF = EPI == 6 || EPI == 7;
   static_assert(F32 || EPI != 4, "EPI 4 (bf16 + residual out of fp32-class operands) is an F32 epilogue");
   constexpr int ESZ = F32 ? 4 : 2;
@@ -60,7 +61,9 @@
   using frag = T::frag;
   const char *A = reinterpret_cast<const char *>(Av), *W = reinterpret_cast<const char *>(Wv);
   const int LDA = lda ? lda : K, LDW = ldw ? ldw : K, LDC = ldc ? ldc : N;
-  const int tiles = GATHER ? __builtin_amdgcn_readfirstlane(tile_info[0]) : tiles_arg;
+  const int tiles = GATHER ? __builtin_amdgcn_readfirstlane(tile_info[0])
+                    : MDEV ? __builtin_amdgcn_readfirstlane((min(max(tile_info[0], 0), M) + GEMM_BM - 1) / GEMM_BM * tiles_n)
+                           : tiles_arg;
   __shared__ __attribute__((aligned(1024))) char smem[GEMM_LDS_BIAS + 2048 + 16 + (EPI == 3 ? 2048 + 8192 : EPI == 5 ? 2048 + 8192 + 4096 : LNF ? 2048 + 2 * 8192 : 0)];
   float *const lnw_lds = reinterpret_cast<float *>(smem + GEMM_LDS_LNW), *const lnb_lds = reinterpret_cast<float *>(smem + GEMM_LDS_LNB);
   float2 *const ln_part = reinterpret_cast<float2 *>(smem + GEMM_LDS_LNPART);
@@ -459,7 +462,7 @@
       const uint32_t x_v0 = (uint32_t)((((size_t)m0 + wm * 128 + r4) * N + n0 + wn * 64 + q * 4) * 4);
       const uint32_t c_v0 = (uint32_t)((((size_t)m0 + wm * 128 + r4) * LDC + n0 + wn * 64 + q * 4) * 2);
       const uint32_t x_rowb = (uint32_t)(N * 4), c_rowb = (uint32_t)(LDC * 2);
-      const int rows_p = tiles_m * GEMM_BM;
+      const int rows_p = MDEV ? (M + GEMM_BM - 1) / GEMM_BM * GEMM_BM : tiles_m * GEMM_BM;
       float sv[2] = {0.f, 0.f};
       if (fold_prev != nullptr) {
         float pv[2][GEMM_LNF_MAXPARTS + 1];
diff --git a/unopose_amd/csrc/upproj.hip b/unopose_amd/csrc/upproj.hip
--- a/unopose_amd/csrc/upproj.hip
+++ b/unopose_amd/csrc/upproj.hip
@@ -104,6 +104,80 @@
   }
 }
 
+__global__ __launch_bounds__(256) void upproj_live_count_kernel(const int *__restrict__ flags, int side, int *__restrict__ tok_live,
+                                                                int *__restrict__ counts) {
+  __shared__ int cnt[4];
+  const int b = blockIdx.x, hw = 4 * side, ntok = side * side;
+  const int *f = flags + (size_t)b * hw * hw;
+  int local = 0;
+  for (int t = threadIdx.x; t < ntok; t += 256) {
+    int on = 0;
+#pragma unroll
+    for (int s = 0; s < 16; ++s) on |= f[up_cell(t, s, side)];
+    on = on != 0;
+    tok_live[(size_t)b * ntok + t] = on;
+    local += on;
+  }
+  const int v = (int)wave_sum_f32((float)local);
+  if ((threadIdx.x & 63) == 0) cnt[threadIdx.x >> 6] = v;
+  __syncthreads();
+  if (threadIdx.x == 0) counts[b] = (cnt[0] + cnt[1]) + (cnt[2] + cnt[3]);
+}
+
+__global__ __launch_bounds__(512) void upproj_live_fill_kernel(const int *__restrict__ tok_live, const int *__restrict__ counts, int side, int B2,
+                                                               int tok_offset, int tok_stride, int *__restrict__ live_rows,
+                                                               int *__restrict__ dead_rows, int2 *__restrict__ img_info, int *__restrict__ m_live) {
+  __shared__ int red[8], wcnt[8];
+  const int b = blockIdx.x, tid = threadIdx.x, lane = tid & 63, wave = tid >> 6, ntok = side * side;
+  int before = 0, all = 0;
+  for (int i = tid; i < B2; i += 512) {
+    const int c = counts[i];
+    all += c;
+    before += i < b ? c : 0;
+  }
+  before = (int)wave_sum_f32((float)before);
+  all = (int)wave_sum_f32((float)all);
+  if (lane == 0) red[wave] = before, wcnt[wave] = all;
+  __syncthreads();
+  int first = 0, total = 0;
+#pragma unroll
+  for (int w = 0; w < 8; ++w) first += red[w], total += wcnt[w];
+  __syncthreads();
+  const int nlive = counts[b];
+  if (tid == 0) {
+    img_info[b] = make_int2(first, nlive);
+    if (b == 0) m_live[0] = total;
+  }
+  const int dfirst = b * tok_stride - first;
+  const int npre = tok_stride - ntok;
+  for (int i = tid; i < npre; i += 512) dead_rows[dfirst + i] = b * tok_stride + (i < tok_offset ? i : ntok + i);
+  const int *tl = tok_live + (size_t)b * ntok;
+  int lbase = first, dbase = dfirst + npre;
+  for (int t0 = 0; t0 < ntok; t0 += 512) {
+    const int t = t0 + tid;
+    const bool in = t < ntok, on = in && tl[t] != 0;
+    const unsigned long long ml = __ballot(on), md = __ballot(in && !on);
+    if (lane == 0) red[wave] = __popcll(ml), wcnt[wave] = __popcll(md);
+    __syncthreads();
+    int lo = 0, dlo = 0, lsum = 0, dsum = 0;
+#pragma unroll
+    for (int w = 0; w < 8; ++w) {
+      lo += w < wave ? red[w] : 0;
+      dlo += w < wave ? wcnt[w] : 0;
+      lsum += red[w];
+      dsum += wcnt[w];
+    }
+    const unsigned long long below = (1ull << lane) - 1ull;
+    if (on) live_rows[lbase + lo + __popcll(ml & below)] = b * tok_stride + tok_offset + t;
+    else if (in) dead_rows[dbase + dlo + __popcll(md & below)] = b * tok_stride + tok_offset + t;
+    lbase += lsum;
+    dbase += dsum;
+    __syncthreads();
+  }
+  for (long j = (long)total + (long)b * 512 + tid; j < (long)B2 * ntok; j += (long)B2 * 512) live_rows[j] = -1;
+  for (long j = (long)B2 * tok_stride - total + (long)b * 512 + tid; j < (long)B2 * tok_stride; j += (long)B2 * 512) dead_rows[j] = -1;
+}
+
 template <bool OUT_BF16>
 __global__ __launch_bounds__(256) void bilinear_sample_compact_kernel(const u16 *__restrict__ Cc, const int *__restrict__ cellmap,
                                                                       const long long *__restrict__ choose, int side, int Np, int H,
@@ -171,6 +245,21 @@
   return check_launch("upproj_plan");
 }
 
+int unopose_upproj_live_rows(const int *flags, int B2, int side, int tok_offset, int tok_stride, int *ws, int *live_rows, int *dead_rows,
+                             int *img_info, int *m_live, unopose_stream_t stream) {
+  UNOPOSE_REQUIRE(flags && ws && live_rows && dead_rows && img_info && m_live, "upproj_live_rows: null pointer");
+  UNOPOSE_REQUIRE(B2 >= 1 && B2 <= 65535 && side >= 1 && side <= 256 && tok_offset >= 0 && tok_stride >= tok_offset + side * side,
+                  "upproj_live_rows: bad sizes");
+  UNOPOSE_REQUIRE((long)B2 * tok_stride < (1L << 24), "upproj_live_rows: too many activation rows");
+  UNOPOSE_REQUIRE(((uintptr_t)img_info & 7) == 0, "upproj_live_rows: img_info must be 8-byte aligned");
+  hipStream_t s = (hipStream_t)stream;
+  int *tok_live = ws, *counts = ws + (size_t)B2 * side * side;
+  hipLaunchKernelGGL(upproj_live_count_kernel, dim3(B2), dim3(256), 0, s, flags, side, tok_live, counts);
+  hipLaunchKernelGGL(upproj_live_fill_kernel, dim3(B2), dim3(512), 0, s, tok_live, counts, side, B2, tok_offset, tok_stride, live_rows, dead_rows,
+                     (int2 *)img_info, m_live);
+  return check_launch("upproj_live_rows");
+}
+
 int unopose_bilinear_sample_compact(const void *Cc, const int *cellmap, const long long *choose, int B2, int side, int Np, int H, int W,
                                     void *out, int out_bf16, unopose_stream_t stream) {
   UNOPOSE_REQUIRE(Cc && cellmap && choose && out, "bilinear_sample_compact: null pointer");
diff --git a/unopose_amd/csrc/vit_attn.hip b/unopose_amd/csrc/vit_attn.hip
--- a/unopose_amd/csrc/vit_attn.hip
+++ b/unopose_amd/csrc/vit_attn.hip
@@ -240,9 +240,10 @@
 constexpr int VD_VSUBB = 128 * 32 + 128;
 constexpr int VD_BUFB = VD_KBYTES + 4 * VD_VSUBB;
 
-template <int NW>
+template <int NW, bool LIST = false>
 __global__ __launch_bounds__(NW * 64, 2) void vit_attn_kernel_dma(const u16 *__restrict__ qkv, int T, int H, int BH, int nq, float scale_log2e,
-                                                               u16 *__restrict__ out) {
+                                                               u16 *__restrict__ out, const int *__restrict__ row_list = nullptr,
+                                                               const int2 *__restrict__ img_info = nullptr, int out_rows = 0) {
   constexpr int QB = 2, NBUF = 2, NPC = 32 / NW;
   extern __shared__ __attribute__((aligned(1024))) char smemd[];
   u16 (*Ot)[32][72] = reinterpret_cast<u16 (*)[32][72]>(smemd);
@@ -252,8 +253,15 @@
   if (bh >= BH) return;
   const int b = bh / H, h = bh % H;
   const int tid = threadIdx.x, lane = tid & 63, wave = __builtin_amdgcn_readfirstlane(tid >> 6);
+  int first = 0, nquery = T;
+  if (LIST) {
+    const int2 info = img_info[b];
+    first = __builtin_amdgcn_readfirstlane(info.x);
+    nquery = __builtin_amdgcn_readfirstlane(min(info.y, T));
+    if (qblk * NW * (32 * QB) >= nquery) return;
+  }
   const int q0 = (qblk * NW + wave) * (32 * QB);
-  const bool active = q0 < T;
+  const bool active = q0 < nquery;
   const int col = lane & 31, hb = lane >> 5;
   const int C3 = 3 * H * 64;
   const u16 *base = qkv + (size_t)b * T * C3;
@@ -283,7 +291,9 @@
   bf16x8 qf[QB][4];
 #pragma unroll
   for (int qb = 0; qb < QB; ++qb) {
-    const int tq = min(q0 + qb * 32 + col, T - 1);
+    int tq = min(q0 + qb * 32 + col, nquery - 1);
+    if (LIST)
+      tq = active ? min(max(row_list[min(first + tq, out_rows - 1)] - b * T, 0), T - 1) : 0;
     const u16 *qp = base + (size_t)tq * C3 + h * 64 + hb * 8;
 #pragma unroll
     for (int ks = 0; ks < 4; ++ks) qf[qb][ks] = *reinterpret_cast<const bf16x8 *>(qp + ks * 16);
@@ -383,7 +393,7 @@
           d = __builtin_amdgcn_mfma_f32_32x32x16_bf16(v0, pf[qb][0].v, d, 0, 0, 0);
           d = __builtin_amdgcn_mfma_f32_32x32x16_bf16(v1, pf[qb][1].v, d, 0, 0, 0);
 #pragma unroll
-          for (int r = 0; r < 16; ++r) o[qb][t][r] = fmaf(o[qb][t][r] - d[r], alpha[qb], d[r]);
+          for (int r = 0; r < 16; ++r) o[qb][t][r] = alpha[qb] < 1.f ? fmaf(o[qb][t][r] - d[r], alpha[qb], d[r]) : o[qb][t][r];
         }
       }
     }
@@ -420,9 +430,9 @@
     for (int it = 0; it < 4; ++it) {
       const int row = it * 8 + (lane >> 3), seg = lane & 7;
       const int tq = q0 + qb * 32 + row;
-      if (tq < T) {
+      if (tq < nquery && (!LIST || first + tq < out_rows)) {
         const uint4 v = *reinterpret_cast<const uint4 *>(&Ot[wave][row][seg * 8]);
-        *reinterpret_cast<uint4 *>(out + ((size_t)b * T + tq) * (H * 64) + h * 64 + seg * 8) = v;
+        *reinterpret_cast<uint4 *>(out + (LIST ? (size_t)(first + tq) : (size_t)b * T + tq) * (H * 64) + h * 64 + seg * 8) = v;
       }
     }
     __builtin_amdgcn_fence(__ATOMIC_RELEASE, "wavefront");
@@ -445,6 +455,19 @@
   hipLaunchKernelGGL((vit_attn_kernel_dma<NW>), dim3((unsigned)blocks), dim3(NW * 64), lds, stream, (const u16 *)qkv, T, H, BH, nq,
                      0.125f * 1.4426950408889634f, (u16 *)out);
   return check_launch("vit_attention");
+}
+
+static int launch_vit_attn_dma_rows(const void *qkv, int B, int T, int H, const int *row_list, const int *img_info, int out_rows, void *out,
+                                    hipStream_t stream) {
+  constexpr int NW = 4;
+  static bool opt[64];
+  const size_t lds = (size_t)2 * VD_BUFB;
+  if (lds_optin(opt, reinterpret_cast<const void *>(&vit_attn_kernel_dma<NW, true>), lds, "vit_attention_rows") != UNOPOSE_OK) return UNOPOSE_ELAUNCH;
+  const int BH = B * H, nq = cdiv(T, 32 * NW * 2);
+  const long blocks = (long)cdiv(BH, 8) * nq * 8;
+  hipLaunchKernelGGL((vit_attn_kernel_dma<NW, true>), dim3((unsigned)blocks), dim3(NW * 64), lds, stream, (const u16 *)qkv, T, H, BH, nq,
+                     0.125f * 1.4426950408889634f, (u16 *)out, row_list, (const int2 *)img_info, out_rows);
+  return check_launch("vit_attention_rows");
 }
 
 template <int QB, int NBUF, int NW>
@@ -481,4 +504,15 @@
   }
 }
 
-}
+int unopose_vit_attention_rows(const void *qkv, int B, int T, int H, const int *row_list, const int *img_info, int out_rows, void *out,
+                               unopose_stream_t stream) {
+  UNOPOSE_REQUIRE(qkv && out && row_list && img_info, "vit_attention_rows: null pointer");
+  UNOPOSE_REQUIRE(B >= 0 && T >= 1 && H >= 1 && (long)B * H * cdiv(T, 128) < (1L << 31) && (long)B * T < (1L << 31) && out_rows >= 0,
+                  "vit_attention_rows: bad sizes");
+  UNOPOSE_REQUIRE(vit_attn_route(T, H) == 2, "vit_attention_rows: only the LDS-DMA route (T >= 1024) has a row-list form (got T=%d H=%d)", T, H);
+  UNOPOSE_REQUIRE(((uintptr_t)img_info & 7) == 0, "vit_attention_rows: img_info must be 8-byte aligned");
+  if (B == 0 || out_rows == 0) return UNOPOSE_OK;
+  return launch_vit_attn_dma_rows(qkv, B, T, H, row_list, img_info, out_rows, out, (hipStream_t)stream);
+}
+
+}
diff --git a/unopose_amd/model/modules.py b/unopose_amd/model/modules.py
--- a/unopose_amd/model/modules.py
+++ b/unopose_amd/model/modules.py
@@ -62,6 +62,19 @@
         xb, stats = ops.linear_residual_(x, ops.vit_attention(qkv, a.heads), a.proj, self.ls1.gamma, stats)
         h = ops.linear_lnfold(xb, stats, self.mlp.fc1, self.norm2, gelu=True)
         return ops.linear_residual_(x, h, self.mlp.fc2, self.ls2.gamma, stats)
+
+    def forward_folded_rows(self, x, n1, xb, stats, live):
+        a = self.attn
+        qkv = ops.linear(n1, a.qkv) if n1 is not None else ops.linear_lnfold(xb, stats, a.qkv, self.norm1)
+        if live.get("event") is not None:
+            torch.cuda.current_stream().wait_event(live["event"])
+        o = ops.vit_attention_rows(qkv, a.heads, live)
+        xc, sc = ops.gather_rows_stats(x.reshape(-1, x.shape[-1]), stats, live["rows"])
+        m = live["m_live"]
+        xbc, sc = ops.linear_residual_(xc, o, a.proj, self.ls1.gamma, sc, m_dev=m)
+        h = ops.linear_lnfold(xbc, sc, self.mlp.fc1, self.norm2, gelu=True, m_dev=m)
+        ops.linear_residual_(xc, h, self.mlp.fc2, self.ls2.gamma, sc, m_dev=m)
+        return xc
 
     def forward_fused_f32(self, x, n1s, next_norm):
         B, T, C = x.shape
@@ -97,6 +110,7 @@
 
 
 SPARSE_SINGLE_CROP = True
+LAST_BLOCK_LIVE = True
 F32_PROLOGUE = True
 F32_TAPS_SPLIT = True
 
@@ -120,11 +134,11 @@
         self.norm = nn.LayerNorm(embed_dim, eps=1e-6)
         self.head = nn.Linear(embed_dim, 1000)
 
-    def forward(self, x, taps_side_by_side=False):
+    def forward(self, x, taps_side_by_side=False, live=None):
         xa, xb = x if isinstance(x, (tuple, list)) else (x, None)
         if ops.vit_prologue_ok(xa, self) and (xb is None or xb.shape[1:] == xa.shape[1:]):
             x, n1, mean = ops.vit_prologue(xa, xb, self, self.blocks[0].norm1, row_mean=True)
-            return self._fused_blocks(x, n1, taps_side_by_side, mean)
+            return self._fused_blocks(x, n1, taps_side_by_side, mean, live)
         if F32_PROLOGUE and ops.vit_prologue_f32_ok(xa, self) and (xb is None or xb.shape[1:] == xa.shape[1:]):
             x, ns = ops.vit_prologue_f32(xa, xb, self, self.blocks[0].norm1)
             return self._fused_blocks_f32(x, ns, taps_side_by_side)
@@ -153,6 +167,10 @@
                             if x.is_cuda and torch.is_autocast_enabled() and not ops.is_differentiable() else self.norm(x))
         return outs
 
+    def last_block_rows_ok(self, T):
+        a = self.blocks[-1].attn
+        return LAST_BLOCK_LIVE and a.qkv.weight.shape[1] == 64 * a.heads and ops.vit_attention_rows_ok(T, a.heads)
+
     def _fused_blocks_f32(self, x, ns, taps_side_by_side):
         n = self.depth // 4
         taps = {self.depth - 1, self.depth - n - 1, self.depth - 2 * n - 1, self.depth - 3 * n - 1}
@@ -169,7 +187,7 @@
         return SplitTaps(wide, x.shape[0], x.shape[1], 4 * x.shape[2]) if wide is not None else outs
 
 
-def _vit_fused_blocks(self, x, n1, taps_side_by_side, row_mean=None):
+def _vit_fused_blocks(self, x, n1, taps_side_by_side, row_mean=None, live=None):
     n = self.depth // 4
     taps = {self.depth - 1, self.depth - n - 1, self.depth - 2 * n - 1, self.depth - 3 * n - 1}
     outs = []
@@ -179,8 +197,16 @@
     if fold and row_mean is None:
         row_mean = ops.fold_row_means(x)
     xb, stats = None, row_mean
+    last = len(self.blocks) - 1
+    T = x.shape[1]
+    rows_route = (live is not None and fold and wide is not None and last in taps and last > 0 and live["images"] == B
+                  and live["tok_stride"] == T and self.last_block_rows_ok(T))
     for i, blk in enumerate(self.blocks):
         nxt = self.blocks[i + 1].norm1 if i + 1 < len(self.blocks) else None
+        if fold and rows_route and i == last and stats.dim() == 3:
+            xc = blk.forward_folded_rows(x, n1, xb, stats, live)
+            ops.layernorm_scatter(xc, self.norm, wide[:, :, len(outs) * D:(len(outs) + 1) * D], live["rows"], live["dead"])
+            return wide
         if fold:
             xb, stats = blk.forward_folded(x, n1, xb, stats)
             n1 = None
@@ -269,7 +295,7 @@
                 sd = x.shape[-1] // 14
                 npre = self.vit.cls_token.shape[1] + self.vit.reg_token.shape[1]
                 plan = ops.upproj_plan(choose, x.shape[-2], x.shape[-1], sd, npre, npre + sd * sd)
-                acts = self.vit(x, taps_side_by_side=True)
+                acts = self.vit(x, taps_side_by_side=True, live=ops.upproj_live_rows(plan) if self.vit.last_block_rows_ok(npre + sd * sd) else None)
                 if torch.is_tensor(acts) and acts.shape[1] == plan["tok_stride"]:
                     return ops.sparse_pixel_features(acts, self.output_upscaling, plan)
                 z, (H, W), off = self.upproject(acts, x.shape[-2], x.shape[-1])
diff --git a/unopose_amd/model/unopose.py b/unopose_amd/model/unopose.py
--- a/unopose_amd/model/unopose.py
+++ b/unopose_amd/model/unopose.py
@@ -286,6 +286,13 @@
                 for t in plan.values():
                     if torch.is_tensor(t):
                         t.record_stream(main)
+                if net.vit.last_block_rows_ok(npre + sd * sd):
+                    live = ops.upproj_live_rows(plan)
+                    for t in live.values():
+                        if torch.is_tensor(t):
+                            t.record_stream(main)
+                    live["event"] = torch.cuda.Event()
+                    live["event"].record(side)
             pre = None
             if GEOM_UNDER_VIT and self.internal_overlap:
                 pre = {}
@@ -304,7 +311,7 @@
                     t.record_stream(main)
         B = rgb.shape[0]
         if plan is not None:
-            acts = net.vit((rgb, tem_rgb), taps_side_by_side=True)
+            acts = net.vit((rgb, tem_rgb), taps_side_by_side=True, live=plan.get("live"))
             if torch.is_tensor(acts) and acts.shape[1] == plan["tok_stride"]:
                 main.wait_stream(side)
                 both = ops.sparse_pixel_features(acts, net.output_upscaling, plan)
diff --git a/unopose_amd/ops/__init__.py b/unopose_amd/ops/__init__.py
--- a/unopose_amd/ops/__init__.py
+++ b/unopose_amd/ops/__init__.py
@@ -12,10 +12,10 @@
     ffn_add_layernorm, linear_add_layernorm, patch_embed, vit_prologue_ok, vit_prologue, vit_prologue_f32_ok, vit_prologue_f32, bmm_nt_f32, score_head, add_layernorm,
     _AddLayerNormFn, add_layernorm_train_ok, add_layernorm_train,
     scale_residual_, scale_residual_layernorm_f32_, vit_f32_fused_ok, scale_residual_layernorm_, ln_fold_ok, _fold_producer_weights,
-    _fold_consumer_weights, linear_residual_, linear_lnfold, fold_shift, fold_row_means, _into,
+    _fold_consumer_weights, linear_residual_, linear_lnfold, fold_shift, fold_row_means, _into, gather_rows_stats, layernorm_scatter,
 )
 from .attention import (
-    vit_attention, vit_attention_f32_split, vit_attention_f32_ss, vit_attention_torch, _KEY_PAD, token_attention,
+    vit_attention, vit_attention_rows, vit_attention_rows_ok, vit_attention_f32_split, vit_attention_f32_ss, vit_attention_torch, _KEY_PAD, token_attention,
     _token_attention_hip_f32, _attn_weights, _token_attention_hip, token_attention_torch, _key_pad, _transpose_pad_f32, _TokenAttnFn,
     token_attention_train_ok, _token_attention_train, focused_linear_attention,
     _focused_linear_attention_hip_f32, _focused_linear_attention_hip, focused_linear_attention_torch,
@@ -26,7 +26,7 @@
     pe_group_mlp_max, pe_group_mlp_max_unfused, pe_geometry, pe_mlp_max, _pe_image, furthest_point_sample, _geo_grid, _GeoEmbedFn, geo_embedding_train_ok,
 )
 from .sampling import (
-    bilinear_sample_native, sparse_upproj_ok, upproj_plan, sparse_pixel_features, bilinear_sample_pixels,
+    bilinear_sample_native, sparse_upproj_ok, upproj_plan, upproj_live_rows, sparse_pixel_features, bilinear_sample_pixels,
 )
 from .pose import (
     overlap_scores, set_first_rows_, pose_score, rigid_rows, feature_similarity, soft_assignment, coarse_pose_torch, fine_pose_torch, _assign_labels, _check_score_width,
diff --git a/unopose_amd/ops/attention.py b/unopose_amd/ops/attention.py
--- a/unopose_amd/ops/attention.py
+++ b/unopose_amd/ops/attention.py
@@ -28,6 +28,23 @@
         return out
     note_fallback("vit_attention", f"head dim {qkv.shape[-1] // (3 * heads)} / dtype {qkv.dtype} (kernels: head dim 64, bf16 or fp32)")
     return vit_attention_torch(qkv, heads)
+
+
+def vit_attention_rows_ok(T, heads):
+    return not st._DIFF and lib().unopose_vit_attention_route(int(T), int(heads)) == 2
+
+
+def vit_attention_rows(qkv, heads, live, out=None):
+    B, T, C3 = qkv.shape
+    assert qkv.is_cuda and qkv.dtype == torch.bfloat16 and C3 == 3 * heads * 64 and vit_attention_rows_ok(T, heads)
+    assert live["images"] == B and live["tok_stride"] == T
+    qkv = _c(qkv)
+    if out is None:
+        out = torch.empty(live["cap"], C3 // 3, dtype=torch.bfloat16, device=qkv.device)
+    assert out.shape == (live["cap"], C3 // 3) and out.dtype == torch.bfloat16 and out.is_contiguous()
+    with on_device(qkv.device):
+        call("unopose_vit_attention_rows", ptr(qkv), B, T, heads, ptr(live["rows"]), ptr(live["info"]), live["cap"], ptr(out), stream_ptr())
+    return out
 
 
 def vit_attention_f32_split(qkv, heads):
diff --git a/unopose_amd/ops/dense.py b/unopose_amd/ops/dense.py
--- a/unopose_amd/ops/dense.py
+++ b/unopose_amd/ops/dense.py
@@ -650,7 +650,7 @@
     return cache
 
 
-def linear_residual_(x, a, lin, gamma, prev=None):
+def linear_residual_(x, a, lin, gamma, prev=None, m_dev=None):
     note_mutation()
     _, w, b = _fold_producer_weights(lin, gamma)
     C, K = w.shape
@@ -670,8 +670,13 @@
     buf = torch.empty(rows_p * (2 * (C // 256) + 1), dtype=torch.float32, device=x.device)
     stats = buf[:rows_p * 2 * (C // 256)].view(rows_p, C // 256, 2)
     with on_device(x.device):
-        call("unopose_linear_bf16_residual", ptr(a), ptr(w), ptr(b), ptr(x), ptr(xb), ptr(stats), None if prev is None else ptr(prev), prev_parts,
-             rows, C, K, stream_ptr())
+        if m_dev is None:
+            call("unopose_linear_bf16_residual", ptr(a), ptr(w), ptr(b), ptr(x), ptr(xb), ptr(stats), None if prev is None else ptr(prev), prev_parts,
+                 rows, C, K, stream_ptr())
+        else:
+            assert m_dev.dtype == torch.int32 and m_dev.device == x.device and m_dev.numel() == 1
+            call("unopose_linear_bf16_residual_rows", ptr(a), ptr(w), ptr(b), ptr(x), ptr(xb), ptr(stats), None if prev is None else ptr(prev),
+                 prev_parts, rows, C, K, ptr(m_dev), stream_ptr())
     return xb, stats
 
 
@@ -688,11 +693,52 @@
     return mean
 
 
-def linear_lnfold(xb, stats, lin, norm, gelu=False):
+def linear_lnfold(xb, stats, lin, norm, gelu=False, m_dev=None):
     _, w, c, d = _fold_consumer_weights(lin, norm)
     N, K = w.shape
     rows = xb.numel() // K
     out = torch.empty(*xb.shape[:-1], N, dtype=torch.bfloat16, device=xb.device)
     with on_device(xb.device):
-        call("unopose_linear_bf16_lnfold", ptr(xb), ptr(w), ptr(d), ptr(c), ptr(stats), K // 256, float(norm.eps), ptr(out), rows, N, K, int(gelu), stream_ptr())
+        if m_dev is None:
+            call("unopose_linear_bf16_lnfold", ptr(xb), ptr(w), ptr(d), ptr(c), ptr(stats), K // 256, float(norm.eps), ptr(out), rows, N, K, int(gelu), stream_ptr())
+        else:
+            assert m_dev.dtype == torch.int32 and m_dev.device == xb.device and m_dev.numel() == 1
+            call("unopose_linear_bf16_lnfold_rows", ptr(xb), ptr(w), ptr(d), ptr(c), ptr(stats), K // 256, float(norm.eps), ptr(out), rows, N, K, int(gelu),
+                 ptr(m_dev), stream_ptr())
     return out
+
+
+def gather_rows_stats(x, stats, row_list):
+    C = x.shape[-1]
+    rows = x.numel() // C
+    n = row_list.numel()
+    nparts = stats.shape[1]
+    assert x.dtype == torch.float32 and x.is_contiguous() and stats.dtype == torch.float32 and stats.dim() == 3 and stats.is_contiguous()
+    assert stats.shape[0] == (rows + 255) // 256 * 256 and stats.untyped_storage().nbytes() >= (stats.storage_offset() + stats.numel() + stats.shape[0]) * 4
+    assert row_list.dtype == torch.int32 and row_list.is_contiguous() and row_list.device == x.device
+    n_p = (n + 255) // 256 * 256
+    xc = torch.empty(n, C, dtype=torch.float32, device=x.device)
+    buf = torch.empty(n_p * (2 * nparts + 1), dtype=torch.float32, device=x.device)
+    stats_c = buf[:n_p * 2 * nparts].view(n_p, nparts, 2)
+    with on_device(x.device):
+        call("unopose_gather_rows_stats", ptr(x), ptr(stats), rows, nparts, ptr(row_list), n, C, ptr(xc), ptr(stats_c), stream_ptr())
+    return xc, stats_c
+
+
+def layernorm_scatter(a, norm, out, out_rows, zero_rows=None):
+    note_mutation()
+    C = a.shape[-1]
+    n = a.numel() // C
+    assert a.dtype == torch.float32 and a.is_contiguous() and out.dtype == torch.bfloat16 and out.shape[-1] == C and out.stride(-1) == 1
+    ld = out.stride(-2)
+    exp = ld
+    for d in range(out.dim() - 2, -1, -1):
+        assert out.stride(d) == exp or out.shape[d] == 1, "out rows must be uniformly strided"
+        exp *= out.shape[d]
+    nout = out.numel() // C
+    assert out_rows.dtype == torch.int32 and out_rows.numel() == n and out_rows.is_contiguous()
+    assert zero_rows is None or (zero_rows.dtype == torch.int32 and zero_rows.is_contiguous())
+    with on_device(a.device):
+        call("unopose_layernorm_scatter", ptr(a), ptr(norm.weight), ptr(norm.bias), n, C, float(norm.eps), ptr(out), int(ld), nout, ptr(out_rows),
+             None if zero_rows is None else ptr(zero_rows), 0 if zero_rows is None else zero_rows.numel(), stream_ptr())
+    return out
diff --git a/unopose_amd/ops/sampling.py b/unopose_amd/ops/sampling.py
--- a/unopose_amd/ops/sampling.py
+++ b/unopose_amd/ops/sampling.py
@@ -51,6 +51,20 @@
     return plan
 
 
+def upproj_live_rows(plan):
+    B2, side, ts = plan["choose"].shape[0], plan["side"], plan["tok_stride"]
+    dev = plan["ws"].device
+    i32 = dict(dtype=torch.int32, device=dev)
+    cap = B2 * side * side
+    live = dict(rows=torch.empty(cap, **i32), dead=torch.empty(B2 * ts, **i32), info=torch.empty(B2, 2, **i32), m_live=torch.empty(1, **i32),
+                ws=torch.empty(cap + B2, **i32), cap=cap, images=B2, tok_stride=ts)
+    with on_device(dev):
+        call("unopose_upproj_live_rows", ptr(plan["ws"]), B2, side, plan["tok_offset"], ts, ptr(live["ws"]), ptr(live["rows"]), ptr(live["dead"]),
+             ptr(live["info"]), ptr(live["m_live"]), stream_ptr())
+    plan["live"] = live
+    return live
+
+
 def sparse_pixel_features(acts, lin, plan, out=None):
     acts = _c(acts)
     if out is not None:
```

Measured after the change: 1145 pairs/s (median of 6 runs). 1.0% higher.
